# 2bitoperations/rtldavis

Hardware: AMD Instinct MI355X
Metric: complex MSamples/s demodulated (uint8 IQ -> packed bits -> preamble matches -> packets) (higher is better)
Workload: dtype f32 (FIR: f16 x f16 -> f32 on the matrix pipe, exact integer accumulation); 1 GPU; 4096 streams x 33 blocks x 8192 samples uint8 IQ per GPU (BASELINE configs[3]/[4]: 64 unique synthetic streams tiled, 2.21 GB resident in HBM), 14 samples/symbol, 19.2 kbit/s; streams_per_gpu=4096, parallelism=streams/1

## Files before the change

### include/rtldavis_hip.h

```cpp
#ifndef RTLDAVIS_HIP_H
#define RTLDAVIS_HIP_H

#include <stddef.h>
#include <stdint.h>

#ifdef __cplusplus
extern "C" {
#endif

#define RD_MAX_PREAMBLE 64
#define RD_MAX_PKT_BYTES 32

typedef enum rd_status {
    RD_OK = 0,
    RD_ERR_ARG = -1,
    RD_ERR_DEVICE = -2,
    RD_ERR_CAPACITY = -3,
    RD_ERR_STATE = -4
} rd_status;

typedef struct rd_config {
    int32_t bit_rate;
    int32_t symbol_length;
    int32_t preamble_symbols;
    int32_t packet_symbols;
    int32_t block_size;
    uint8_t preamble[RD_MAX_PREAMBLE];
} rd_config;

typedef struct rd_packet {
    int32_t stream;
    int32_t call;
    int32_t index;
    int32_t nbytes;
    uint8_t data[RD_MAX_PKT_BYTES];
    double rssi;
    double snr;
} rd_packet;

typedef struct rd_parsed {
    int32_t stream;
    int32_t call;
    int32_t index;
    int32_t freq_err;
    int32_t id;
    int32_t nbytes;
    uint8_t data[RD_MAX_PKT_BYTES];
    double rssi;
    double snr;
} rd_parsed;

typedef struct rd_timing {
    float demod_ms;
    float fixup_ms;
    float search_ms;
    float slice_ms;
    float total_ms;
    int32_t runs;
} rd_timing;

const char *rd_last_error(void);
int rd_device_count(void);
int rd_set_device(int device);
int rd_set_wait_timeout_ms(int ms);

typedef struct rd_demod rd_demod;

int rd_create(const rd_config *cfg, rd_demod **out);
void rd_destroy(rd_demod *h);
int rd_reset(rd_demod *h);
int rd_demod_block(rd_demod *h, const void *samples, size_t count, int is_complex, rd_packet *out, int cap, int *n);
int rd_create_multi(const rd_config *cfg, int n_streams, rd_demod **out);
int rd_demod_blocks(rd_demod *h, const uint8_t *iq, size_t nbytes, rd_packet *out, int cap, int *n);
int rd_demod_submit(rd_demod *h, const void *samples, size_t count, int is_complex);
int rd_set_input_push(int mode);
int rd_demod_input_mode(rd_demod *h);
int rd_demod_register_input(rd_demod *h, void *host, size_t nbytes);
int rd_demod_submit_from(rd_demod *h, size_t offset, size_t count, int is_complex);
int rd_demod_fetch(rd_demod *h, rd_packet *out, int cap, int *n);
int rd_demod_inflight(rd_demod *h);
int rd_demod_refetch(rd_demod *h, rd_packet *out, int cap, int *n);
int rd_copy_discriminated_stream(rd_demod *h, int stream, double *out, size_t n);
int rd_copy_discriminated(rd_demod *h, double *out, size_t n);
int rd_copy_filtered(rd_demod *h, double *out_interleaved, size_t n_complex);
int rd_copy_quantized(rd_demod *h, uint8_t *out, size_t n);

typedef struct rd_batch rd_batch;

int rd_batch_create(const rd_config *cfg, int n_streams, int n_blocks, rd_batch **out);
void rd_batch_destroy(rd_batch *b);
int rd_batch_input_ptr(rd_batch *b, void **dev_ptr, size_t *nbytes);
int rd_batch_upload(rd_batch *b, const uint8_t *iq_host, size_t nbytes);
int rd_batch_upload_async(rd_batch *b, const uint8_t *iq_host, size_t nbytes, void *hip_stream);
int rd_batch_run(rd_batch *b, void *hip_stream);
int rd_batch_results(rd_batch *b, rd_packet *out, int cap, int *n);
int rd_batch_copy_bits(rd_batch *b, int stream, uint8_t *out, size_t nbytes);
int rd_batch_copy_discriminated(rd_batch *b, int stream, size_t t0, double *out, size_t n);
int rd_batch_set_parse(rd_batch *b, int enabled);
int rd_batch_parsed(rd_batch *b, rd_parsed *out, int cap, int *n);
int rd_batch_set_timing(rd_batch *b, int enabled);
int rd_batch_get_timing(rd_batch *b, rd_timing *out);
int rd_batch_set_pipelined(rd_batch *b, int enabled);
#define RD_FORM_ORDERED_TAIL 1u
#define RD_FORM_SECOND_PASS 8u
#define RD_FORM_ONE_LAUNCH_TAIL 16u
int rd_batch_last_run_forms(rd_batch *b, uint32_t *forms);
int rd_batch_get_counters(rd_batch *b, uint64_t *fixup_runs, uint64_t *matches);

int rd_lut_execute(const uint8_t *in_bytes, size_t n_bytes, double *out_cplx, size_t n_cplx);
int rd_rotate_fs4(const double *in_cplx, double *out_cplx, size_t n_cplx);
int rd_fir9(const double *in_cplx, size_t n_in, double *out_cplx, size_t n_out);
int rd_discriminate(const double *in_cplx, size_t n_in, double *out, size_t n_out);
int rd_quantize(const double *in, uint8_t *out, size_t n);
int rd_search(const rd_config *cfg, const uint8_t *quantized, size_t n, int32_t *indices, int cap, int *count);

typedef struct rd_chan_config {
    int32_t out_rate;
    int32_t decim;
    int32_t n_taps;
    int32_t n_channels;
    double gain;
} rd_chan_config;
typedef struct rd_chan rd_chan;

#define RD_IQ_U8 0
#define RD_IQ_S8 1
#define RD_IQ_S16 2

int rd_chan_create(const rd_chan_config *cfg, const double *taps, const int64_t *shift_hz, rd_chan **out);
int rd_chan_create_fmt(const rd_chan_config *cfg, int sample_format, const double *taps, const int64_t *shift_hz,
                       rd_chan **out);
void rd_chan_destroy(rd_chan *h);
int rd_chan_upload(rd_chan *h, const void *wide_iq, size_t nbytes);
int rd_chan_input_ptr(rd_chan *h, size_t n_wide_samples, void **dev_ptr);
int rd_chan_run(rd_chan *h, size_t n_out, void *dst_dev, size_t dst_stream_stride, void *hip_stream);
int rd_chan_run_host(rd_chan *h, size_t n_out, uint8_t *out_host, size_t nbytes);

typedef struct rd_wideband rd_wideband;
int rd_wideband_create(const rd_config *cfg, const rd_chan_config *ccfg, const double *taps,
                       const int64_t *shift_hz, rd_wideband **out);
int rd_wb_create_fmt(const rd_config *cfg, const rd_chan_config *ccfg, int sample_format, const double *taps,
                     const int64_t *shift_hz, rd_wideband **out);
void rd_wideband_destroy(rd_wideband *w);
int rd_wideband_reset(rd_wideband *w);
int rd_wideband_submit(rd_wideband *w, const void *wide_iq, size_t nbytes);
int rd_wideband_fetch(rd_wideband *w, rd_packet *out, int cap, int *n);
int rd_wideband_refetch(rd_wideband *w, rd_packet *out, int cap, int *n);
int rd_wideband_inflight(rd_wideband *w);
int rd_wideband_copy_channelized(rd_wideband *w, uint8_t *out, size_t nbytes);
int rd_wideband_copy_discriminated(rd_wideband *w, int channel, double *out, size_t n);
int rd_wideband_debug_advance_clock(rd_wideband *w, uint64_t n_out);

void rd_debug_mfma_taps(uint16_t *out);
void rd_debug_mfma_taps8(uint16_t *out);
void rd_debug_mfma_taps8s(uint16_t *vals, uint32_t *idx);
int rd_debug_demod_mfma(const uint8_t *iq_host, int n_streams, uint32_t n_samples, int hist_mode,
                        uint32_t hist_bytes, float *g_out, uint32_t *bits_out, uint32_t *fix_out,
                        uint32_t fix_cap, uint32_t *n_fix);

#ifdef __cplusplus
}
#endif
#endif
```

### rtldavis_amd/_lib.py

```python
from __future__ import annotations

import ctypes as C
import os

import numpy as np

HERE = os.path.dirname(os.path.abspath(__file__))
LIB_PATH = os.environ.get("RTLDAVIS_HIP_LIB") or os.path.join(HERE, "librtldavis_hip.so")

RD_MAX_PREAMBLE = 64
RD_MAX_PKT_BYTES = 32
RD_OK, RD_ERR_ARG, RD_ERR_DEVICE, RD_ERR_CAPACITY, RD_ERR_STATE = 0, -1, -2, -3, -4


class HipError(RuntimeError):
    """A HIP/device failure reported by librtldavis_hip (never swallowed, never retried on CPU)."""


class RdConfig(C.Structure):
    _fields_ = [("bit_rate", C.c_int32), ("symbol_length", C.c_int32), ("preamble_symbols", C.c_int32),
                ("packet_symbols", C.c_int32), ("block_size", C.c_int32), ("preamble", C.c_uint8 * RD_MAX_PREAMBLE)]


class RdPacket(C.Structure):
    _fields_ = [("stream", C.c_int32), ("call", C.c_int32), ("index", C.c_int32), ("nbytes", C.c_int32),
                ("data", C.c_uint8 * RD_MAX_PKT_BYTES), ("rssi", C.c_double), ("snr", C.c_double)]


class RdParsed(C.Structure):
    _fields_ = [("stream", C.c_int32), ("call", C.c_int32), ("index", C.c_int32), ("freq_err", C.c_int32),
                ("id", C.c_int32), ("nbytes", C.c_int32), ("data", C.c_uint8 * RD_MAX_PKT_BYTES),
                ("rssi", C.c_double), ("snr", C.c_double)]


class RdTiming(C.Structure):
    _fields_ = [("demod_ms", C.c_float), ("fixup_ms", C.c_float), ("search_ms", C.c_float),
                ("slice_ms", C.c_float), ("total_ms", C.c_float), ("runs", C.c_int32)]


class RdChanConfig(C.Structure):
    _fields_ = [("out_rate", C.c_int32), ("decim", C.c_int32), ("n_taps", C.c_int32), ("n_channels", C.c_int32),
                ("gain", C.c_double)]


RD_IQ_U8, RD_IQ_S8, RD_IQ_S16 = 0, 1, 2
SAMPLE_FORMATS = {"u8": (RD_IQ_U8, np.uint8), "s8": (RD_IQ_S8, np.int8), "s16": (RD_IQ_S16, np.int16)}


def sample_format(name):
    try:
        return SAMPLE_FORMATS[name]
    except (KeyError, TypeError):
        raise ValueError(f"unknown sample format {name!r}: one of {sorted(SAMPLE_FORMATS)}") from None


def iq_array(a, dtype):
    if np.dtype(dtype) == np.uint8:
        return np.ascontiguousarray(a, dtype=np.uint8).reshape(-1)
    a = np.asarray(a)
    if a.dtype != dtype:
        info = np.iinfo(dtype)
        if a.dtype.kind not in "iu" or (a.size and (a.min() < info.min or a.max() > info.max)):
            raise ValueError(f"a {a.dtype} array is not a capture of {np.dtype(dtype).name} samples")
        a = a.astype(dtype)
    return np.ascontiguousarray(a).reshape(-1)


_P = C.c_void_p
SIGNATURES = {
    "rd_last_error": (C.c_char_p, []),
    "rd_device_count": (C.c_int, []),
    "rd_set_device": (C.c_int, [C.c_int]),
    "rd_set_wait_timeout_ms": (C.c_int, [C.c_int]),
    "rd_set_input_push": (C.c_int, [C.c_int]),
    "rd_demod_input_mode": (C.c_int, [C.c_void_p]),
    "rd_create": (C.c_int, [C.POINTER(RdConfig), C.POINTER(_P)]),
    "rd_create_multi": (C.c_int, [C.POINTER(RdConfig), C.c_int, C.POINTER(_P)]),
    "rd_demod_blocks": (C.c_int, [_P, _P, C.c_size_t, C.POINTER(RdPacket), C.c_int, C.POINTER(C.c_int)]),
    "rd_copy_discriminated_stream": (C.c_int, [_P, C.c_int, _P, C.c_size_t]),
    "rd_demod_submit": (C.c_int, [_P, _P, C.c_size_t, C.c_int]),
    "rd_demod_register_input": (C.c_int, [_P, _P, C.c_size_t]),
    "rd_demod_submit_from": (C.c_int, [_P, C.c_size_t, C.c_size_t, C.c_int]),
    "rd_demod_fetch": (C.c_int, [_P, C.POINTER(RdPacket), C.c_int, C.POINTER(C.c_int)]),
    "rd_demod_refetch": (C.c_int, [_P, C.POINTER(RdPacket), C.c_int, C.POINTER(C.c_int)]),
    "rd_demod_inflight": (C.c_int, [_P]),
    "rd_destroy": (None, [_P]),
    "rd_reset": (C.c_int, [_P]),
    "rd_demod_block": (C.c_int, [_P, _P, C.c_size_t, C.c_int, C.POINTER(RdPacket), C.c_int, C.POINTER(C.c_int)]),
    "rd_copy_discriminated": (C.c_int, [_P, _P, C.c_size_t]),
    "rd_copy_filtered": (C.c_int, [_P, _P, C.c_size_t]),
    "rd_copy_quantized": (C.c_int, [_P, _P, C.c_size_t]),
    "rd_batch_create": (C.c_int, [C.POINTER(RdConfig), C.c_int, C.c_int, C.POINTER(_P)]),
    "rd_batch_destroy": (None, [_P]),
    "rd_batch_input_ptr": (C.c_int, [_P, C.POINTER(_P), C.POINTER(C.c_size_t)]),
    "rd_batch_upload": (C.c_int, [_P, _P, C.c_size_t]),
    "rd_batch_upload_async": (C.c_int, [_P, _P, C.c_size_t, _P]),
    "rd_batch_run": (C.c_int, [_P, _P]),
    "rd_batch_results": (C.c_int, [_P, C.POINTER(RdPacket), C.c_int, C.POINTER(C.c_int)]),
    "rd_batch_copy_bits": (C.c_int, [_P, C.c_int, _P, C.c_size_t]),
    "rd_batch_copy_discriminated": (C.c_int, [_P, C.c_int, C.c_size_t, _P, C.c_size_t]),
    "rd_batch_set_parse": (C.c_int, [_P, C.c_int]),
    "rd_batch_parsed": (C.c_int, [_P, C.POINTER(RdParsed), C.c_int, C.POINTER(C.c_int)]),
    "rd_batch_set_timing": (C.c_int, [_P, C.c_int]),
    "rd_batch_set_pipelined": (C.c_int, [_P, C.c_int]),
    "rd_batch_last_run_forms": (C.c_int, [_P, C.POINTER(C.c_uint32)]),
    "rd_batch_get_timing": (C.c_int, [_P, C.POINTER(RdTiming)]),
    "rd_batch_get_counters": (C.c_int, [_P, C.POINTER(C.c_uint64), C.POINTER(C.c_uint64)]),
    "rd_lut_execute": (C.c_int, [_P, C.c_size_t, _P, C.c_size_t]),
    "rd_rotate_fs4": (C.c_int, [_P, _P, C.c_size_t]),
    "rd_fir9": (C.c_int, [_P, C.c_size_t, _P, C.c_size_t]),
    "rd_discriminate": (C.c_int, [_P, C.c_size_t, _P, C.c_size_t]),
    "rd_quantize": (C.c_int, [_P, _P, C.c_size_t]),
    "rd_search": (C.c_int, [C.POINTER(RdConfig), _P, C.c_size_t, _P, C.c_int, C.POINTER(C.c_int)]),
    "rd_chan_create": (C.c_int, [C.POINTER(RdChanConfig), _P, _P, C.POINTER(_P)]),
    "rd_chan_create_fmt": (C.c_int, [C.POINTER(RdChanConfig), C.c_int, _P, _P, C.POINTER(_P)]),
    "rd_chan_destroy": (None, [_P]),
    "rd_chan_upload": (C.c_int, [_P, _P, C.c_size_t]),
    "rd_chan_input_ptr": (C.c_int, [_P, C.c_size_t, C.POINTER(_P)]),
    "rd_chan_run": (C.c_int, [_P, C.c_size_t, _P, C.c_size_t, _P]),
    "rd_chan_run_host": (C.c_int, [_P, C.c_size_t, _P, C.c_size_t]),
    "rd_wideband_create": (C.c_int, [C.POINTER(RdConfig), C.POINTER(RdChanConfig), _P, _P, C.POINTER(_P)]),
    "rd_wb_create_fmt": (C.c_int, [C.POINTER(RdConfig), C.POINTER(RdChanConfig), C.c_int, _P, _P, C.POINTER(_P)]),
    "rd_wideband_destroy": (None, [_P]),
    "rd_wideband_reset": (C.c_int, [_P]),
    "rd_wideband_submit": (C.c_int, [_P, _P, C.c_size_t]),
    "rd_wideband_fetch": (C.c_int, [_P, C.POINTER(RdPacket), C.c_int, C.POINTER(C.c_int)]),
    "rd_wideband_refetch": (C.c_int, [_P, C.POINTER(RdPacket), C.c_int, C.POINTER(C.c_int)]),
    "rd_wideband_inflight": (C.c_int, [_P]),
    "rd_wideband_copy_channelized": (C.c_int, [_P, _P, C.c_size_t]),
    "rd_wideband_copy_discriminated": (C.c_int, [_P, C.c_int, _P, C.c_size_t]),
    "rd_wideband_debug_advance_clock": (C.c_int, [_P, C.c_uint64]),
    "rd_debug_mfma_taps": (None, [_P]),
    "rd_debug_mfma_taps8": (None, [_P]),
    "rd_debug_mfma_taps8s": (None, [_P, _P]),
    "rd_debug_demod_mfma": (C.c_int, [_P, C.c_int, C.c_uint32, C.c_int, C.c_uint32, _P, _P, _P, C.c_uint32,
                                      C.POINTER(C.c_uint32)]),
}

_lib = None


def lib():
    global _lib
    if _lib is None:
        if not os.path.exists(LIB_PATH):
            raise ImportError(
                f"{LIB_PATH} is missing: build it with `python -c 'import __graft_entry__ as g; g.build()'` "
                "or `make -C rtldavis_amd/csrc`.  rtldavis_amd has no CPU fallback.")
        L = C.CDLL(LIB_PATH)
        for name, (res, args) in SIGNATURES.items():
            fn = getattr(L, name)
            fn.restype = res
            fn.argtypes = args
        _lib = L
    return _lib


def last_error() -> str:
    return (lib().rd_last_error() or b"").decode("utf-8", "replace")


def check(rc: int) -> None:
    if rc == RD_OK:
        return
    msg = last_error()
    if rc == RD_ERR_ARG:
        raise ValueError(msg)
    if rc == RD_ERR_CAPACITY:
        raise BufferError(msg)
    if rc == RD_ERR_STATE:
        raise RuntimeError(msg)
    raise HipError(msg)


def make_config(bit_rate, symbol_length, preamble_symbols, packet_symbols, preamble, block_size) -> RdConfig:
    if len(preamble) > RD_MAX_PREAMBLE:
        raise ValueError("preamble longer than 64 symbols is not supported")
    c = RdConfig(int(bit_rate), int(symbol_length), int(preamble_symbols), int(packet_symbols), int(block_size))
    for i, ch in enumerate(preamble):
        c.preamble[i] = int(ch)
    return c
```

### rtldavis_amd/batch.py

```python
from __future__ import annotations

import ctypes as C
from typing import List, Optional

import numpy as np

from . import _lib
from .dsp import Packet, PacketConfig, _cfg_struct


RD_PACKET_DTYPE = np.dtype([("stream", "<i4"), ("call", "<i4"), ("index", "<i4"), ("nbytes", "<i4"),
                            ("data", "u1", (_lib.RD_MAX_PKT_BYTES,)), ("rssi", "<f8"), ("snr", "<f8")])
assert RD_PACKET_DTYPE.itemsize == C.sizeof(_lib.RdPacket)


RD_PARSED_DTYPE = np.dtype([("stream", "<i4"), ("call", "<i4"), ("index", "<i4"), ("freq_err", "<i4"),
                            ("id", "<i4"), ("nbytes", "<i4"), ("data", "u1", (_lib.RD_MAX_PKT_BYTES,)),
                            ("rssi", "<f8"), ("snr", "<f8")])
assert RD_PARSED_DTYPE.itemsize == C.sizeof(_lib.RdParsed)


class BatchDemodulator:
    def __init__(self, cfg: PacketConfig, n_streams: int, n_blocks: int, device: Optional[int] = None) -> None:
        self.cfg = cfg
        self.n_streams = int(n_streams)
        self.n_blocks = int(n_blocks)
        self.n_samples = self.n_blocks * cfg.block_size
        self._b = C.c_void_p()
        if device is not None:
            _lib.check(_lib.lib().rd_set_device(int(device)))
        _lib.check(_lib.lib().rd_batch_create(C.byref(_cfg_struct(cfg)), self.n_streams, self.n_blocks, C.byref(self._b)))
        self._cap = 0
        self._recs = None

    def close(self) -> None:
        if self._b:
            b, self._b = self._b, None
            _lib.lib().rd_batch_destroy(b)

    def __del__(self):
        try:
            self.close()
        except Exception:
            pass

    def input_ptr(self):
        p, n = C.c_void_p(), C.c_size_t()
        _lib.check(_lib.lib().rd_batch_input_ptr(self._b, C.byref(p), C.byref(n)))
        return p.value, n.value

    def upload(self, iq: np.ndarray) -> None:
        a = np.ascontiguousarray(iq, dtype=np.uint8)
        if a.size != self.n_streams * 2 * self.n_samples:
            raise ValueError("Incompatible array sizes")
        _lib.check(_lib.lib().rd_batch_upload(self._b, a.ctypes.data, a.size))

    def upload_async(self, iq: np.ndarray, hip_stream: int) -> None:
        if iq.dtype != np.uint8 or not iq.flags["C_CONTIGUOUS"] or iq.size != self.n_streams * 2 * self.n_samples:
            raise ValueError("Incompatible array sizes")
        _lib.check(_lib.lib().rd_batch_upload_async(self._b, iq.ctypes.data, iq.size, C.c_void_p(hip_stream or None)))

    def run(self, hip_stream: int = 0) -> None:
        _lib.check(_lib.lib().rd_batch_run(self._b, C.c_void_p(hip_stream or None)))

    def set_parse(self, enabled: bool) -> None:
        _lib.check(_lib.lib().rd_batch_set_parse(self._b, int(bool(enabled))))

    def parsed(self) -> np.ndarray:
        cap = max(1024, 4 * self.n_streams)
        while True:
            buf = (_lib.RdParsed * cap)()
            n = C.c_int(0)
            rc = _lib.lib().rd_batch_parsed(self._b, buf, cap, C.byref(n))
            if rc == _lib.RD_ERR_CAPACITY:
                cap = n.value + 1024
                continue
            _lib.check(rc)
            return np.frombuffer(buf, dtype=RD_PARSED_DTYPE, count=n.value).copy()

    def set_timing(self, level) -> None:
        _lib.check(_lib.lib().rd_batch_set_timing(self._b, int(level)))

    def set_pipelined(self, enabled=True) -> None:
        _lib.check(_lib.lib().rd_batch_set_pipelined(self._b, 1 if enabled else 0))

    def timing(self) -> dict:
        t = _lib.RdTiming()
        _lib.check(_lib.lib().rd_batch_get_timing(self._b, C.byref(t)))
        return {k: float(getattr(t, k)) for k, _ in t._fields_}

    def last_run_forms(self) -> dict:
        f = C.c_uint32()
        _lib.check(_lib.lib().rd_batch_last_run_forms(self._b, C.byref(f)))
        return {"ordered_tail": bool(f.value & 1), "second_pass": bool(f.value & 8), "one_launch_tail": bool(f.value & 16)}

    def counters(self) -> dict:
        f, m = C.c_uint64(), C.c_uint64()
        _lib.check(_lib.lib().rd_batch_get_counters(self._b, C.byref(f), C.byref(m)))
        return {"fixup_runs": f.value, "matches": m.value}

    def results(self) -> np.ndarray:
        L = _lib.lib()
        n = C.c_int(0)
        if self._recs is None:
            self._cap = max(1024, 16 * self.n_streams)
            self._recs = (_lib.RdPacket * self._cap)()
        rc = L.rd_batch_results(self._b, self._recs, self._cap, C.byref(n))
        if rc == _lib.RD_ERR_CAPACITY:
            self._cap = n.value + 1024
            self._recs = (_lib.RdPacket * self._cap)()
            rc = L.rd_batch_results(self._b, self._recs, self._cap, C.byref(n))
        _lib.check(rc)
        return np.frombuffer(self._recs, dtype=RD_PACKET_DTYPE, count=n.value)

    def records(self):
        out = []
        for r in self.results():
            data = np.frombuffer(r["data"][: int(r["nbytes"])].tobytes(), dtype=np.uint8)
            out.append((int(r["stream"]), int(r["call"]),
                        Packet(int(r["index"]), data, float(r["rssi"]), float(r["snr"]))))
        return out

    def packets(self) -> List[List[List[Packet]]]:
        res = [[[] for _ in range(self.n_blocks)] for _ in range(self.n_streams)]
        for s, c, p in self.records():
            res[s][c].append(p)
        return res

    def bits(self, stream: int) -> np.ndarray:
        out = np.empty((self.n_samples + 7) // 8, dtype=np.uint8)
        _lib.check(_lib.lib().rd_batch_copy_bits(self._b, int(stream), out.ctypes.data, out.size))
        return out

    def discriminated(self, stream: int, t0: int, n: int) -> np.ndarray:
        out = np.empty(int(n), dtype=np.float64)
        _lib.check(_lib.lib().rd_batch_copy_discriminated(self._b, int(stream), int(t0), out.ctypes.data, out.size))
        return out

    def demodulate(self, iq: np.ndarray) -> List[List[List[Packet]]]:
        self.upload(iq)
        self.run()
        return self.packets()
```

### rtldavis_amd/csrc/rd_api.hip

```cpp
#include <unistd.h>
#include <immintrin.h>
#include <hsa/hsa.h>
#include <hsa/hsa_ext_amd.h>

#include <algorithm>
#include <cstdarg>
#include <cstdio>
#include <cstring>
#include <string>
#include <vector>
#include <mutex>
#include <map>

#include <chrono>

#include "rd_host.h"
#include "rd_internal.h"
#include "rd_math.h"

static bool dbg_host() {
    static int v = -1;
    if (v < 0) v = getenv("RD_DEBUG_HOST") ? 1 : 0;
    return v == 1;
}
// ... 64 lines not shown
    return RD_OK;
}

static int wait_event(hipEvent_t ev, const char *what) {
    rd_waiter w(rd_wait_timeout_ms());
    for (;;) {
        const hipError_t e = hipEventQuery(ev);
        if (e == hipSuccess) return RD_OK;
        if (e != hipErrorNotReady) return fail(RD_ERR_DEVICE, "hipEventQuery: %s", hipGetErrorString(e));
        if (!w.relax()) return fail(RD_ERR_DEVICE, "timed out after %.0f ms waiting for %s", w.waited_ms(), what);
    }
}

static int wait_stream(hipStream_t st, const char *what) {
    rd_waiter w(rd_wait_timeout_ms());
    for (;;) {
        const hipError_t e = hipStreamQuery(st);
        if (e == hipSuccess) return RD_OK;
        if (e != hipErrorNotReady) return fail(RD_ERR_DEVICE, "hipStreamQuery: %s", hipGetErrorString(e));
        if (!w.relax()) return fail(RD_ERR_DEVICE, "timed out after %.0f ms waiting for %s", w.waited_ms(), what);
    }
}

extern "C" int rd_set_wait_timeout_ms(int ms) { return (int)rd_wait_timeout_set((double)ms); }

static int copy_d2h(void *dst, const void *src, size_t n, hipStream_t st) {
    if (n == 0) return RD_OK;
    HIPCHK(hipMemcpyAsync(dst, src, n, hipMemcpyDeviceToHost, st));
    return wait_stream(st, "a device-to-host copy");
}

static int make_devcfg(const rd_config *c, rd_devcfg *d) {
    const char *why = "";
    const int rc = rd_make_devcfg(c, d, &why);
    return rc ? fail(rc, "%s", why) : RD_OK;
}
static void order_and_dedupe(const rd_packet *recs, size_t n, int S, rd_order_scratch &sc) { rd_order_and_dedupe(recs, n, S, sc); }

struct rd_batch {
    rd_config cfg;
    rd_devcfg dc;
    int n_streams, n_blocks;
    long n_samples;
    size_t bits_stride;
    bool dev_ready = false, fast_ok = false, ran = false, timing = false, timing_detail = false;
    bool run_timing = false, run_detail = false;
    int device = -1;
    bool fetched = false;
    uint8_t *d_iq = nullptr;
    size_t iq_bytes = 0;
    uint32_t *d_bits = nullptr, *d_fix = nullptr, *d_cnt = nullptr;
    rd_match *d_matches = nullptr;
    void *d_tasks = nullptr;
    int dense = 0;
    rd_order_scratch order;
    rd_packet *d_recs = nullptr;
    int cnt_set = 0;
    bool parse = false;
    rd_parsed *d_parsed = nullptr;
    uint32_t fix_cap = 0, match_cap = 0, rec_cap = 0;
    hipStream_t stream = nullptr;
    std::vector<hipEvent_t> evs;
    size_t ev_runs = 0;
    hipEvent_t *ev = nullptr;
    hipEvent_t done = nullptr;
    hipEvent_t kdone = nullptr;
    hipEvent_t uploaded = nullptr;
    bool upload_pending = false;
    hipStream_t copy_stream = nullptr;
    uint32_t h_cnt[RD_CNT_SLOTS] = {};
    uint32_t *h_cnt_pin = nullptr;
    rd_packet *h_recs_pin = nullptr;
    uint32_t rec_pin_cap = 0;
    uint32_t spec_recs = 1024;
    uint64_t last_fix = 0, last_match = 0;
    rd_timing last_timing = {};
    bool dev_order = false, tail_off = false;
    size_t cnt_stride = RD_CNT_TOTAL;
    rd_ft_bufs ft;
    bool ft_ok = false, ft_run = false;
    uint32_t ft_seq = 0, ft_limit = 0;
    bool ft_sticky = false;
    size_t ft_cnt_off = 0;
    bool second_pass = false;
    uint32_t last_launch[2] = {0, 0};
    bool pipelined = false;
    bool deferred = false;
    hipEvent_t kfirst = nullptr;
    std::vector<uint8_t> ev_end;
};

static std::mutex g_tail_mx;
typedef std::pair<int, hipStream_t> rd_tail_key;
static std::map<rd_tail_key, rd_batch *> g_tail;

static rd_layout batch_layout(const rd_batch *b) {
    rd_layout l;
    l.iq = b->d_iq;
    l.stream_stride = (size_t)b->n_samples * 2;
    l.n_streams = b->n_streams;
    l.n_samples = (uint32_t)b->n_samples;
    l.hist_mode = 0;
    l.valid_from = 0;
    l.bits = b->d_bits;
    l.bits_stride = b->bits_stride;
    return l;
}

extern "C" int rd_batch_create(const rd_config *cfg, int n_streams, int n_blocks, rd_batch **out) {
    if (!out) return fail(RD_ERR_ARG, "null out");
    rd_devcfg dc;
    int rc = make_devcfg(cfg, &dc);
    if (rc) return rc;
    if (n_streams < 1 || n_blocks < 1) return fail(RD_ERR_ARG, "n_streams and n_blocks must be >= 1");
    const long n = (long)n_blocks * cfg->block_size;
    const uint64_t runs = (uint64_t)n_streams * ((n + RD_RUN - 1) / RD_RUN);
    if (n > 0x7FFFFFF0L || runs > 0x0FFFFFFFull)
        return fail(RD_ERR_ARG, "batch too large: at most 2^28 32-sample runs (8.6e9 samples) per batch");
    rd_batch *b = new rd_batch();
    b->cfg = *cfg;
    b->dc = dc;
    b->n_streams = n_streams;
    b->n_blocks = n_blocks;
    b->n_samples = n;
    b->bits_stride = (size_t)((n + 31) / 32);
    b->fast_ok = ((size_t)n * 2) % 16 == 0;
    *out = b;
    return RD_OK;
}

static uint32_t *batch_cnt(const rd_batch *b) { return b->d_cnt + (size_t)b->cnt_set * b->cnt_stride; }

static int use_device(int device) {
    if (device >= 0) HIPCHK(hipSetDevice(device));
    return RD_OK;
}

static int batch_alloc(rd_batch *b) {
    if (b->dev_ready) return use_device(b->device);
    int rc = ensure_device();
    if (rc) return rc;
    HIPCHK(hipGetDevice(&b->device));
    const uint64_t runs = (uint64_t)b->n_streams * b->bits_stride;
    b->iq_bytes = (size_t)b->n_streams * b->n_samples * 2;
    b->fix_cap = (uint32_t)std::min<uint64_t>(runs, std::max<uint64_t>(4096, runs / 8));
    b->match_cap = (uint32_t)std::min<uint64_t>((uint64_t)b->n_streams * (8 + 1ull * b->n_blocks) + 1024, 1u << 26);
    if (const char *e = getenv("RD_TEST_MATCH_CAP")) {
        const long v = atol(e);
        if (v >= 1 && v < (long)b->match_cap) b->match_cap = (uint32_t)v;
    }
    b->rec_cap = 2 * b->match_cap;
    HIPCHK(hipMalloc(&b->d_iq, b->iq_bytes + RD_INPUT_PAD));
    HIPCHK(hipMemset(b->d_iq + b->iq_bytes, 127, RD_INPUT_PAD));
    HIPCHK(hipMalloc(&b->d_bits, runs * sizeof(uint32_t)));
    HIPCHK(hipMalloc(&b->d_fix, (size_t)b->fix_cap * sizeof(uint32_t)));
    {
        const char *ti = getenv("RD_TAIL_IMPL");
        const bool legacy = ti && ti[0] == 'l';
        b->ft_ok = !legacy && b->fast_ok && b->dc.S == 14 && b->dc.P == 16 && b->dc.K == 80 && b->dc.pre_mask == 0x91D3ull &&
                   b->n_samples < (1l << 30) && b->dc.B < (1 << 24) && b->bits_stride % 4 == 0 && b->dc.L >= b->dc.B &&
                   (long)(b->n_blocks + 1) * b->dc.B - b->dc.L >= 0 &&
                   ((long)(b->n_blocks + 1) * b->dc.B - b->dc.L) / 32 + 16 <= (long)b->bits_stride;
        if (const char *e = getenv("RD_TEST_BUCKET_CAP")) {
            const long v = atol(e);
            if (v >= 1 && v < RD_BUCKET_MIN) b->ft_limit = (uint32_t)v;
        }
    }
    b->cnt_stride = RD_CNT_TOTAL;
    if (b->ft_ok) {
        const size_t groups = ((size_t)b->n_streams + RD_FT_STREAMS - 1) / RD_FT_STREAMS;
        b->ft_cnt_off = b->cnt_stride;
        b->cnt_stride += (groups + 3) & ~(size_t)3;
        const uint64_t tps = ((uint64_t)b->n_samples + RD_TILE_SAMPLES - 1) / RD_TILE_SAMPLES;
        b->ft.fix_bcap = (uint32_t)std::min<uint64_t>((2 * RD_FT_STREAMS * (tps / 4 + 8) + 63) & ~63ull, 1u << 20);
        if (const char *e = getenv("RD_TEST_FIX_BCAP")) {
            const long v = atol(e);
            if (v >= 1 && v < (long)b->ft.fix_bcap) b->ft.fix_bcap = (uint32_t)v;
        }
        b->ft.bcap = rd_ord_bucket_cap(b->n_samples);
        HIPCHK(hipMalloc(&b->ft.fixb, groups * b->ft.fix_bcap * sizeof(uint32_t)));
        HIPCHK(hipMalloc(&b->ft.gstate, 3 * groups * sizeof(uint32_t)));
        HIPCHK(hipMemset(b->ft.gstate, 0, 3 * groups * sizeof(uint32_t)));
    }
    HIPCHK(hipMalloc(&b->d_cnt, 2 * b->cnt_stride * sizeof(uint32_t)));
    HIPCHK(hipMemset(b->d_cnt, 0, 2 * b->cnt_stride * sizeof(uint32_t)));
    HIPCHK(hipMalloc(&b->d_matches, (size_t)b->match_cap * sizeof(rd_match)));
    HIPCHK(hipMalloc(&b->d_recs, (size_t)b->rec_cap * sizeof(rd_packet)));
    HIPCHK(hipMalloc(&b->d_tasks, (size_t)b->rec_cap * RD_TASK_BYTES));
    HIPCHK(hipHostMalloc((void **)&b->h_cnt_pin, RD_CNT_SLOTS * sizeof(uint32_t), hipHostMallocDefault));
    HIPCHK(hipHostMalloc((void **)&b->h_recs_pin, (size_t)b->rec_cap * sizeof(rd_packet), hipHostMallocDefault));
    b->rec_pin_cap = b->rec_cap;
    HIPCHK(hipEventCreateWithFlags(&b->done, hipEventDisableTiming));
    HIPCHK(hipEventCreateWithFlags(&b->kdone, hipEventDisableTiming));
    HIPCHK(hipEventCreateWithFlags(&b->kfirst, hipEventDisableTiming));
    HIPCHK(hipEventCreateWithFlags(&b->uploaded, hipEventDisableTiming));
    HIPCHK(hipStreamCreateWithFlags(&b->copy_stream, hipStreamNonBlocking));
    b->dev_ready = true;
    return RD_OK;
}

extern "C" void rd_batch_destroy(rd_batch *b) {
    if (!b) return;
    {
        std::lock_guard<std::mutex> g(g_tail_mx);
        auto it = g_tail.find(rd_tail_key(b->device, b->stream));
        if (it != g_tail.end() && it->second == b) g_tail.erase(it);
        b->deferred = false;
    }
    if (b->dev_ready && g_hip_pid == getpid()) {
        if (b->device >= 0) hipSetDevice(b->device);
        if (b->ran && !b->fetched) hipDeviceSynchronize();
        hipFree(b->d_iq); hipFree(b->d_bits); hipFree(b->d_fix); hipFree(b->d_cnt);
        hipFree(b->d_matches); hipFree(b->d_recs); hipFree(b->d_tasks);
        hipFree(b->d_parsed);
        hipFree(b->ft.fixb); hipFree(b->ft.gstate);
        hipHostFree(b->h_cnt_pin); hipHostFree(b->h_recs_pin);
        if (b->done) hipEventDestroy(b->done);
        if (b->kdone) hipEventDestroy(b->kdone);
        if (b->kfirst) hipEventDestroy(b->kfirst);
        if (b->uploaded) hipEventDestroy(b->uploaded);
        if (b->copy_stream) hipStreamDestroy(b->copy_stream);
        for (auto &e : b->evs) if (e) hipEventDestroy(e);
    }
    delete b;
}

extern "C" int rd_batch_input_ptr(rd_batch *b, void **dev_ptr, size_t *nbytes) {
    if (!b || !dev_ptr) return fail(RD_ERR_ARG, "null argument");
    int rc = batch_alloc(b);
    if (rc) return rc;
    *dev_ptr = b->d_iq;
    if (nbytes) *nbytes = b->iq_bytes;
    return RD_OK;
}

static int batch_flush(rd_batch *b);

extern "C" int rd_batch_upload(rd_batch *b, const uint8_t *iq_host, size_t nbytes) {
    if (!b || !iq_host) return fail(RD_ERR_ARG, "null argument");
    int rc = batch_alloc(b);
    if (rc) return rc;
    if (nbytes != b->iq_bytes) {
        return fail(RD_ERR_ARG, "Incompatible array sizes: got %zu bytes, expected %zu", nbytes, b->iq_bytes);
    }
    if (b->ran && !b->fetched) {
        rc = batch_flush(b);
        if (rc) return rc;
        rc = wait_event(b->done, "the previous run before an upload");
        if (rc) return rc;
    }
    HIPCHK(hipMemcpy(b->d_iq, iq_host, nbytes, hipMemcpyHostToDevice));
    if (!b->ft_sticky) b->tail_off = false;
    return RD_OK;
}

extern "C" int rd_batch_upload_async(rd_batch *b, const uint8_t *iq_host, size_t nbytes, void *hip_stream) {
    if (!b || !iq_host) return fail(RD_ERR_ARG, "null argument");
    int rc = batch_alloc(b);
    if (rc) return rc;
    if (nbytes != b->iq_bytes) return fail(RD_ERR_ARG, "Incompatible array sizes: got %zu bytes, expected %zu", nbytes, b->iq_bytes);
    hipStream_t cs = (hipStream_t)hip_stream;
    if (b->ran && !b->fetched) {
        rc = batch_flush(b);
        if (rc) return rc;
        HIPCHK(hipStreamWaitEvent(cs, b->done, 0));
    }
    HIPCHK(hipMemcpyAsync(b->d_iq, iq_host, nbytes, hipMemcpyHostToDevice, cs));
    HIPCHK(hipEventRecord(b->uploaded, cs));
    b->upload_pending = true;
    if (!b->ft_sticky) b->tail_off = false;
    return RD_OK;
}

static int batch_readback(rd_batch *b, hipEvent_t after) {
    HIPCHK(hipStreamWaitEvent(b->copy_stream, after, 0));
    HIPCHK(hipMemcpyAsync(b->h_cnt_pin, batch_cnt(b), RD_CNT_SLOTS * sizeof(uint32_t), hipMemcpyDeviceToHost,
                          b->copy_stream));
    const uint32_t spec = std::min(b->dev_order ? b->rec_cap : b->match_cap, b->spec_recs);
    if (spec)
        HIPCHK(hipMemcpyAsync(b->h_recs_pin, b->d_recs, (size_t)spec * sizeof(rd_packet), hipMemcpyDeviceToHost,
                              b->copy_stream));
    HIPCHK(hipEventRecord(b->done, b->copy_stream));
    return RD_OK;
}


static int batch_flush_locked(rd_batch *p) {
    if (!p->deferred) return RD_OK;
    auto it = g_tail.find(rd_tail_key(p->device, p->stream));
    if (it != g_tail.end() && it->second == p) g_tail.erase(it);
    p->deferred = false;
    int rc = use_device(p->device);
    if (rc) return rc;
    HIPCHK(hipEventRecord(p->kdone, p->stream));
    return batch_readback(p, p->kdone);
}
static int batch_flush(rd_batch *b) {
    std::lock_guard<std::mutex> g(g_tail_mx);
    return batch_flush_locked(b);
}
static bool batch_stream_has_tail(int device, hipStream_t st) {
    std::lock_guard<std::mutex> g(g_tail_mx);
    return g_tail.find(rd_tail_key(device, st)) != g_tail.end();
}
static int batch_adopt(int device, hipStream_t st, hipEvent_t carrier) {
    std::lock_guard<std::mutex> g(g_tail_mx);
    auto it = g_tail.find(rd_tail_key(device, st));
    if (it == g_tail.end()) return RD_OK;
    rd_batch *p = it->second;
    g_tail.erase(it);
    p->deferred = false;
    return batch_readback(p, carrier);
}

static int batch_search_slice(rd_batch *b, hipStream_t st, bool may_defer = false, uint32_t *zero_next = nullptr) {
    const rd_layout lay = batch_layout(b);
    const long B = b->dc.B, L = b->dc.L;
    const bool last_on_slice = !b->parse;
    const bool defer = may_defer && b->pipelined && last_on_slice && !(b->run_timing && b->run_detail);
    hipEvent_t last = defer ? nullptr : b->run_timing ? b->ev[4] : b->kdone;
    if (b->run_timing && may_defer) b->ev_end.push_back(defer ? 0 : 1);
    b->dev_order = false;
    if (b->ft_run && may_defer) {
        rd_ft_bufs fb = b->ft;
        fb.fixcnt = batch_cnt(b) + b->ft_cnt_off;
        b->ft_seq = b->ft_seq % 4095u + 1u;
        const int ok = rd_launch_tail_fused(lay, b->dc, b->n_blocks, B - L, (long)(b->n_blocks + 1) * B - L, fb,
                                            b->ft_limit ? b->ft_limit : fb.bcap, b->ft_seq, 0, b->d_recs, b->rec_cap, batch_cnt(b), st,
                                            last_on_slice ? last : nullptr, zero_next, (uint32_t)b->cnt_stride);
        if (!ok) return fail(RD_ERR_STATE, "the one-launch tail refused a shape its buffers were allocated for");
        b->dev_order = true;
        b->dense = 1;
    }
    if (!b->dev_order) {
        rd_launch_search(b->d_bits, b->bits_stride, b->n_streams, b->n_samples, B - L, (long)(b->n_blocks + 1) * B - L,
                         b->dc, b->d_matches, b->match_cap, batch_cnt(b), st);
        if (b->run_timing && b->run_detail) HIPCHK(hipEventRecord(b->ev[3], st));
        b->dense = rd_launch_slice(lay, b->d_bits, b->bits_stride, b->n_samples, b->dc, b->d_matches, b->match_cap, 1,
                                   b->n_blocks, 0, b->d_recs, nullptr, batch_cnt(b), st, last_on_slice ? last : nullptr,
                                   b->d_tasks);
    }
    if (b->parse) {
        if (!b->d_parsed) HIPCHK(hipMalloc(&b->d_parsed, (size_t)b->rec_cap * sizeof(rd_parsed)));
        rd_launch_parse(lay, b->dc, b->d_recs, b->match_cap, b->d_parsed, batch_cnt(b), st, b->dense);
    }
    if (defer) {
        std::lock_guard<std::mutex> g(g_tail_mx);
        auto it = g_tail.find(rd_tail_key(b->device, st));
        if (it != g_tail.end() && it->second != b) {
            int rc = batch_flush_locked(it->second);
            if (rc) return rc;
        }
        g_tail[rd_tail_key(b->device, st)] = b;
        b->deferred = true;
        HIPCHK(hipGetLastError());
        return RD_OK;
    }
    if (!last_on_slice) HIPCHK(hipEventRecord(last, st));
    int rc = batch_readback(b, last);
    if (rc) return rc;
    HIPCHK(hipGetLastError());
    return RD_OK;
}

extern "C" int rd_batch_run(rd_batch *b, void *hip_stream) {
    if (!b) return fail(RD_ERR_ARG, "null batch");
    int rc = batch_alloc(b);
    if (rc) return rc;
    hipStream_t st = (hipStream_t)hip_stream;
    const rd_layout lay = batch_layout(b);
    if (b->ran && !b->fetched) {
        rc = batch_flush(b);
        if (rc) return rc;
        HIPCHK(hipStreamWaitEvent(st, b->done, 0));
    }
    b->stream = st;
    if (b->upload_pending) {
        HIPCHK(hipStreamWaitEvent(st, b->uploaded, 0));
        b->upload_pending = false;
    }
    b->fetched = false;
    b->cnt_set ^= 1;
    uint32_t *cnt = batch_cnt(b), *cnt_next = b->d_cnt + (size_t)(b->cnt_set ^ 1) * b->cnt_stride;
    b->run_timing = b->timing;
    b->run_detail = b->timing_detail;
    if (b->timing) {
        if (b->evs.size() < 5 * (b->ev_runs + 1)) {
            const size_t old = b->evs.size();
            b->evs.resize(old + 5, nullptr);
            for (size_t i = old; i < b->evs.size(); i++) HIPCHK(hipEventCreate(&b->evs[i]));
        }
        b->ev = &b->evs[5 * b->ev_runs];
        b->ev_runs++;
    }
    const bool adopt = batch_stream_has_tail(b->device, st);
    const bool want_ft = b->ft_ok && b->fast_ok && !b->tail_off && !(b->timing && b->timing_detail);
    const uint32_t dflags = want_ft ? RD_DEMOD_FIX_BUCKETS : 0u;
    uint32_t *fixl = want_ft ? b->ft.fixb : b->d_fix, *bcnt = want_ft ? cnt + b->ft_cnt_off : nullptr;
    const uint32_t fixc = want_ft ? b->ft.fix_bcap : b->fix_cap;
    uint32_t honoured = 0;
    if (b->timing && b->fast_ok) {
        honoured = rd_launch_demod(lay, fixl, fixc, cnt, st, b->ev[0], b->ev[1], dflags, b->last_launch, bcnt);
        if (adopt && (rc = batch_adopt(b->device, st, b->ev[1]))) return rc;
    } else if (b->fast_ok && adopt) {
        honoured = rd_launch_demod(lay, fixl, fixc, cnt, st, nullptr, b->kfirst, dflags, b->last_launch, bcnt);
        if ((rc = batch_adopt(b->device, st, b->kfirst))) return rc;
    } else {
        if (b->timing) HIPCHK(hipEventRecord(b->ev[0], st));
        if (b->fast_ok) honoured = rd_launch_demod(lay, fixl, fixc, cnt, st, nullptr, nullptr, dflags, b->last_launch, bcnt);
        if (b->timing) HIPCHK(hipEventRecord(b->ev[1], st));
        if (adopt) {
            hipEvent_t carrier = b->timing ? b->ev[1] : b->kfirst;
            if (!b->timing) HIPCHK(hipEventRecord(carrier, st));
            if ((rc = batch_adopt(b->device, st, carrier))) return rc;
        }
    }
    b->second_pass = false;
    b->ft_run = b->fast_ok && (honoured & RD_DEMOD_FIX_BUCKETS);
    if (!b->ft_run)
        rd_launch_fixup(lay, fixl, fixc, cnt, b->fast_ok ? 0 : 1, cnt_next, st, (uint32_t)b->cnt_stride, b->last_fix);
    if (b->timing && b->timing_detail) HIPCHK(hipEventRecord(b->ev[2], st));
    rc = batch_search_slice(b, st, true, b->ft_run ? cnt_next : nullptr);
    if (rc) return rc;
    b->ran = true;
    return RD_OK;
}

static int batch_finish(rd_batch *b) {
    if (!b->ran) return fail(RD_ERR_STATE, "rd_batch_run has not been called");
    hipStream_t st = b->stream;
    {
        int frc = batch_flush(b);
        if (frc) return frc;
    }
    for (int attempt = 0; attempt < 8; attempt++) {
        const double ta = now_ms();
        int wrc = wait_event(b->done, "the batch run's results");
        if (wrc) return wrc;
        memcpy(b->h_cnt, b->h_cnt_pin, sizeof b->h_cnt);
        if (dbg_host()) fprintf(stderr, "[rd] finish: wait %.3f ms\n", now_ms() - ta);
        bool redo_search = false;
        if (b->ft_run && !b->second_pass && (b->h_cnt[RD_CNT_OVF] & (8u | 16u))) {
            const rd_layout lay = batch_layout(b);
            rd_launch_fixup(lay, b->d_fix, b->fix_cap, batch_cnt(b), 1, nullptr, st);
            b->last_fix = (uint64_t)b->n_streams * b->bits_stride;
            b->tail_off = true;
            b->h_cnt[RD_CNT_OVF] = 0;
            b->h_cnt[RD_CNT_FIX] = 0;
            redo_search = true;
        } else if (b->ft_run && !b->second_pass && (b->h_cnt[RD_CNT_OVF] & 1u)) {
            if (!b->ft_limit && b->ft.bcap < RD_BUCKET_MAX) b->ft.bcap = std::min<uint32_t>(2 * b->ft.bcap, RD_BUCKET_MAX);
            else if (!b->ft_limit) b->ft_sticky = true;
        }
        if (redo_search) {
        } else if (b->fast_ok && !b->ft_run && b->h_cnt[RD_CNT_FIX] > b->fix_cap) {
            const rd_layout lay = batch_layout(b);
            rd_launch_fixup(lay, b->d_fix, b->fix_cap, batch_cnt(b), 1, nullptr, st);
            uint32_t cap = b->fix_cap;
            HIPCHK(hipMemcpyAsync(batch_cnt(b) + RD_CNT_FIX, &cap, sizeof cap, hipMemcpyHostToDevice, st));
            b->last_fix = (uint64_t)b->n_streams * b->bits_stride;
            redo_search = true;
        } else if (attempt == 0) {
            b->last_fix = (uint64_t)b->h_cnt[RD_CNT_FIX];
        }
        if (redo_search && b->tail_off) b->dev_order = false;
        if (b->dev_order && b->h_cnt[RD_CNT_OVF]) {
            b->tail_off = true;
            if (dbg_host())
                fprintf(stderr, "[rd] one-launch tail overflow: flags %u (1 a stream's match list, 2 records), matches %u\n",
                        b->h_cnt[RD_CNT_OVF], b->h_cnt[RD_CNT_MATCH]);
            const uint32_t zero[5] = {0, 0, 0, 0, 0};
            HIPCHK(hipMemcpyAsync(batch_cnt(b) + RD_CNT_MATCH, zero, sizeof zero, hipMemcpyHostToDevice, st));
            b->second_pass = true;
            int rc2 = batch_search_slice(b, st);
            if (rc2) return rc2;
            continue;
        }
        if (!b->dev_order && b->h_cnt[RD_CNT_MATCH] > b->match_cap) {
            hipFree(b->d_matches); b->d_matches = nullptr;
            hipFree(b->d_recs); b->d_recs = nullptr;
            hipHostFree(b->h_recs_pin); b->h_recs_pin = nullptr;
            b->rec_pin_cap = 0;
            hipFree(b->d_tasks); b->d_tasks = nullptr;
            hipFree(b->d_parsed); b->d_parsed = nullptr;
            const uint32_t want = b->h_cnt[RD_CNT_MATCH] + b->h_cnt[RD_CNT_MATCH] / 4 + 1024;
            b->match_cap = 0;
            b->rec_cap = 0;
            b->ran = false;
            const uint32_t new_rec_cap = 2 * want;
            HIPCHK(hipMalloc(&b->d_matches, (size_t)want * sizeof(rd_match)));
            HIPCHK(hipMalloc(&b->d_recs, (size_t)new_rec_cap * sizeof(rd_packet)));
            HIPCHK(hipMalloc(&b->d_tasks, (size_t)new_rec_cap * RD_TASK_BYTES));
            HIPCHK(hipHostMalloc((void **)&b->h_recs_pin, (size_t)new_rec_cap * sizeof(rd_packet), hipHostMallocDefault));
            b->match_cap = want;
            b->rec_cap = new_rec_cap;
            b->rec_pin_cap = new_rec_cap;
            b->ran = true;
            redo_search = true;
        }
        if (!redo_search) {
            b->last_match = b->h_cnt[RD_CNT_MATCH];
            b->fetched = true;
            return RD_OK;
        }
        const uint32_t zero[5] = {0, 0, 0, 0, 0};
        HIPCHK(hipMemcpyAsync(batch_cnt(b) + RD_CNT_MATCH, zero, sizeof zero, hipMemcpyHostToDevice, st));
        b->second_pass = true;
        int rc2 = batch_search_slice(b, st);
        if (rc2) return rc2;
    }
    return fail(RD_ERR_DEVICE, "result lists kept overflowing");
}

extern "C" int rd_batch_results(rd_batch *b, rd_packet *out, int cap, int *n) {
    if (!b || !n) return fail(RD_ERR_ARG, "null argument");
    const double t0 = now_ms();
    int rc = batch_finish(b);
    if (rc) return rc;
    const double t1 = now_ms();
    const uint32_t nprim = b->dense ? std::min(b->h_cnt[RD_CNT_TASKS], b->rec_cap) : std::min(b->h_cnt[RD_CNT_MATCH], b->match_cap);
    const uint32_t nextra = b->dense ? 0u : std::min(b->h_cnt[RD_CNT_REC], b->match_cap);
    const uint32_t have = std::min(b->dev_order ? b->rec_cap : b->match_cap, b->spec_recs);
    if (nprim > have) {
        rc = copy_d2h(b->h_recs_pin + have, b->d_recs + have, (size_t)(nprim - have) * sizeof(rd_packet), b->copy_stream);
        if (rc) return rc;
    }
    if (nextra) {
        rc = copy_d2h(b->h_recs_pin + nprim, b->d_recs + b->match_cap, (size_t)nextra * sizeof(rd_packet), b->copy_stream);
        if (rc) return rc;
    }
    const uint32_t nrec = nprim + nextra;
    b->spec_recs = std::max<uint32_t>(1024, nprim + nprim / 4);
    const double t2 = now_ms();
    if (b->dev_order) {
        *n = (int)nrec;
        if ((int)nrec > cap) return fail(RD_ERR_CAPACITY, "need room for %u packets", nrec);
        if (nrec) {
            if (!out) return fail(RD_ERR_ARG, "null out");
            memcpy(out, b->h_recs_pin, (size_t)nrec * sizeof(rd_packet));
        }
        if (dbg_host())
            fprintf(stderr, "[rd] results (k_tail): finish %.3f ms, D2H %u recs %.3f ms, copy %.3f ms\n", t1 - t0, nrec,
                    t2 - t1, now_ms() - t2);
        return RD_OK;
    }
    order_and_dedupe(b->h_recs_pin, nrec, b->dc.S, b->order);
    const std::vector<uint32_t> &kept = b->order.kept;
    *n = (int)kept.size();
    if ((int)kept.size() > cap) return fail(RD_ERR_CAPACITY, "need room for %zu packets", kept.size());
    if (!kept.empty()) {
        if (!out) return fail(RD_ERR_ARG, "null out");
        for (size_t i = 0; i < kept.size(); i++) out[i] = b->h_recs_pin[kept[i]];
    }
    if (dbg_host())
        fprintf(stderr, "[rd] results: finish %.3f ms, D2H %u recs %.3f ms, order+dedupe+copy %.3f ms\n", t1 - t0, nrec,
                t2 - t1, now_ms() - t2);
    return RD_OK;
}

extern "C" int rd_batch_copy_bits(rd_batch *b, int stream, uint8_t *out, size_t nbytes) {
    if (!b || !out) return fail(RD_ERR_ARG, "null argument");
    if (stream < 0 || stream >= b->n_streams) return fail(RD_ERR_ARG, "stream out of range");
    const size_t need = (size_t)((b->n_samples + 7) / 8);
    if (nbytes < need) return fail(RD_ERR_ARG, "bit buffer too small: %zu < %zu", nbytes, need);
    int rc = batch_finish(b);
    if (rc) return rc;
    return copy_d2h(out, (const uint8_t *)(b->d_bits + (size_t)stream * b->bits_stride), need, b->stream);
}

extern "C" int rd_batch_copy_discriminated(rd_batch *b, int stream, size_t t0, double *out, size_t n) {
    if (!b || !out) return fail(RD_ERR_ARG, "null argument");
    if (stream < 0 || stream >= b->n_streams || t0 + n > (size_t)b->n_samples)
        return fail(RD_ERR_ARG, "range out of bounds");
    int rc = batch_alloc(b);
    if (rc) return rc;
    if (n == 0) return RD_OK;
    double *d = nullptr;
    HIPCHK(hipMalloc(&d, n * sizeof(double)));
    rd_launch_disc(batch_layout(b), stream, (long)t0, (long)n, d, b->stream);
    rc = copy_d2h(out, d, n * sizeof(double), b->stream);
    hipFree(d);
    return rc;
}

// ... 30 lines not shown
        for (size_t k = group; k < kept && !dup; k++)
            dup = recs[k].nbytes == r.nbytes && memcmp(recs[k].data, r.data, sizeof r.data) == 0;
        if (!dup) recs[kept++] = r;
    }
    *n = (int)kept;
    if ((int)kept > cap) return fail(RD_ERR_CAPACITY, "need room for %zu messages", kept);
    if (kept) {
        if (!out) return fail(RD_ERR_ARG, "null out");
        memcpy(out, recs.data(), kept * sizeof(rd_parsed));
    }
    return RD_OK;
}

extern "C" int rd_batch_set_pipelined(rd_batch *b, int enabled) {
    if (!b) return fail(RD_ERR_ARG, "null batch");
    b->pipelined = enabled != 0;
    return RD_OK;
}

extern "C" int rd_batch_set_timing(rd_batch *b, int enabled) {
    if (!b) return fail(RD_ERR_ARG, "null batch");
    b->timing = enabled != 0;
    b->timing_detail = enabled >= 2;
    b->ev_runs = 0;
    b->ev_end.clear();
    if (b->timing && b->dev_ready && use_device(b->device) == RD_OK) {
        const size_t want = 5 * 64;
        const size_t old = b->evs.size();
        if (old < want) {
            b->evs.resize(want, nullptr);
            for (size_t i = old; i < want; i++) HIPCHK(hipEventCreate(&b->evs[i]));
        }
    }
    return RD_OK;
}

extern "C" int rd_batch_get_timing(rd_batch *b, rd_timing *out) {
    if (!b || !out) return fail(RD_ERR_ARG, "null argument");
    if (!b->timing) return fail(RD_ERR_STATE, "timing not enabled");
    int rc = batch_finish(b);
    if (rc) return rc;
    rd_timing t = {};
    size_t n_end = 0;
    for (size_t r = 0; r < b->ev_runs; r++) {
        hipEvent_t *e = &b->evs[5 * r];
        float v[5] = {0, 0, 0, 0, 0};
        HIPCHK(hipEventElapsedTime(&v[0], e[0], e[1]));
        if (b->timing_detail) {
            HIPCHK(hipEventElapsedTime(&v[1], e[1], e[2]));
            HIPCHK(hipEventElapsedTime(&v[2], e[2], e[3]));
            HIPCHK(hipEventElapsedTime(&v[3], e[3], e[4]));
        }
        const bool has_end = r >= b->ev_end.size() || b->ev_end[r];
        if (has_end) { HIPCHK(hipEventElapsedTime(&v[4], e[0], e[4])); n_end++; }
        t.demod_ms += v[0]; t.fixup_ms += v[1]; t.search_ms += v[2]; t.slice_ms += v[3]; t.total_ms += v[4];
    }
    if (b->ev_runs) {
        const float k = 1.0f / (float)b->ev_runs;
        t.demod_ms *= k; t.fixup_ms *= k; t.search_ms *= k; t.slice_ms *= k;
        t.total_ms = n_end ? t.total_ms / (float)n_end : 0.0f;
    }
    t.runs = (int32_t)b->ev_runs;
    b->ev_runs = 0;
    b->ev_end.clear();
    b->last_timing = t;
    *out = t;
    return RD_OK;
}

extern "C" int rd_batch_last_run_forms(rd_batch *b, uint32_t *forms) {
    if (!b || !forms) return fail(RD_ERR_ARG, "null argument");
    int rc = batch_finish(b);
    if (rc) return rc;
    *forms = (b->dev_order ? RD_FORM_ORDERED_TAIL | RD_FORM_ONE_LAUNCH_TAIL : 0u) | (b->second_pass ? RD_FORM_SECOND_PASS : 0u);
    return RD_OK;
}

extern "C" int rd_batch_get_counters(rd_batch *b, uint64_t *fixup_runs, uint64_t *matches) {
    if (!b) return fail(RD_ERR_ARG, "null batch");
    int rc = batch_finish(b);
    if (rc) return rc;
    if (fixup_runs) *fixup_runs = b->last_fix;
    if (matches) *matches = b->last_match;
    return RD_OK;
}

#define RD_MAX_DEVICES 64
struct rd_push_info {
    int state = 0;
    volatile uint32_t *hdp_flush = nullptr;
};
static rd_push_info g_push[RD_MAX_DEVICES];

struct rd_hdp_find { uint32_t bdf, domain; volatile uint32_t *reg; bool found; };
static hsa_status_t rd_hdp_cb(hsa_agent_t agent, void *data) {
    rd_hdp_find *f = (rd_hdp_find *)data;
    hsa_device_type_t t;
    if (hsa_agent_get_info(agent, HSA_AGENT_INFO_DEVICE, &t) != HSA_STATUS_SUCCESS || t != HSA_DEVICE_TYPE_GPU) return HSA_STATUS_SUCCESS;
    uint32_t bdf = 0, dom = 0;
    if (hsa_agent_get_info(agent, (hsa_agent_info_t)HSA_AMD_AGENT_INFO_BDFID, &bdf) != HSA_STATUS_SUCCESS) return HSA_STATUS_SUCCESS;
    if (hsa_agent_get_info(agent, (hsa_agent_info_t)HSA_AMD_AGENT_INFO_DOMAIN, &dom) != HSA_STATUS_SUCCESS) return HSA_STATUS_SUCCESS;
    if (bdf != f->bdf || dom != f->domain) return HSA_STATUS_SUCCESS;
    hsa_amd_hdp_flush_t h = {nullptr, nullptr};
    if (hsa_agent_get_info(agent, (hsa_agent_info_t)HSA_AMD_AGENT_INFO_HDP_FLUSH, &h) == HSA_STATUS_SUCCESS) f->reg = h.HDP_MEM_FLUSH_CNTL;
    f->found = true;
    return HSA_STATUS_INFO_BREAK;
}

static int g_push_mode = -1;
static bool push_available(int dev) {
    if (dev < 0 || dev >= RD_MAX_DEVICES || g_push_mode == 0) return false;
    static std::mutex mu;
    std::lock_guard<std::mutex> lock(mu);
    rd_push_info &p = g_push[dev];
    if (p.state) return p.state > 0;
    p.state = -1;
    const char *e = getenv("RD_PUSH_INPUT");
    if (e && atoi(e) == 0) return false;
    int large = 0;
    if (hipDeviceGetAttribute(&large, hipDeviceAttributeIsLargeBar, dev) != hipSuccess || !large) return false;
    char id[64] = {0};
    unsigned dom = 0, bus = 0, d = 0, fn = 0;
    if (hipDeviceGetPCIBusId(id, sizeof id, dev) != hipSuccess || sscanf(id, "%x:%x:%x.%x", &dom, &bus, &d, &fn) != 4) return false;
    if (hsa_init() != HSA_STATUS_SUCCESS) return false;
    rd_hdp_find f = {(bus << 8) | (d << 3) | fn, dom, nullptr, false};
    hsa_iterate_agents(rd_hdp_cb, &f);
    if (!f.found || !f.reg) return false;
    p.hdp_flush = f.reg;
    p.state = 1;
    return true;
}

extern "C" int rd_set_input_push(int mode) {
    int rc = ensure_device();
    if (rc) return rc;
    g_push_mode = mode == 0 ? 0 : -1;
    int dev = -1;
    if (hipGetDevice(&dev) != hipSuccess) return fail(RD_ERR_DEVICE, "hipGetDevice failed");
    return push_available(dev) ? 1 : 0;
}

struct rd_slot {
    uint8_t *h_in = nullptr;
    uint8_t *d_in_map = nullptr;
    uint8_t *d_in = nullptr;
    uint8_t *d_push = nullptr;
    uint32_t *h_cnt = nullptr;
    rd_packet *h_recs = nullptr;
    rd_packet *d_recs_map = nullptr;
    uint32_t *h_sb = nullptr;
    uint32_t *d_sb_map = nullptr;
    uint32_t seq = 0;
    bool one = false;
    hipEvent_t e_in = nullptr, e_done = nullptr;
};

struct rd_demod {
    rd_config cfg;
    rd_devcfg dc;
    bool dev_ready = false;
    bool cplx_mode = false;
    long seen = 0;
    int NS = 1;
    int device = -1;
    size_t ring_stride = 0;
    uint8_t *d_ring = nullptr;
// ... 749 lines not shown
```

### rtldavis_amd/csrc/rd_demod_mfma.hip

```cpp
#include <cstdio>
#include <cstdlib>
#include <cstring>

#include <hip/hip_ext.h>

#include "rd_internal.h"
#include "rd_math.h"
#include "rd_mfma.h"

#define RD_MF_WG 256
#define RD_MF_WAVES (RD_MF_WG / 64)
#ifndef RD_MF_MINWAVES
#define RD_MF_MINWAVES 4
#endif
#define RD_MF_GROUP_BYTES 1152
#define RD_MF_IMG_BYTES (16 + 4 * RD_MF_GROUP_BYTES)
#define RD_MF_IMG_PAD 4624
#define RD_MF_XB_BYTES (3 * 1024 + 32 + 32)
#define RD_MF_PEND 32
#ifndef RD_MF_STAGE_TILES
#define RD_MF_STAGE_TILES 4
#endif

typedef _Float16 rd_h8 __attribute__((ext_vector_type(8)));
typedef _Float16 rd_h16 __attribute__((ext_vector_type(16)));
typedef _Float16 rd_h2 __attribute__((ext_vector_type(2)));
typedef float rd_f16v __attribute__((ext_vector_type(16)));
typedef uint32_t rd_u4v __attribute__((ext_vector_type(4)));
typedef float rd_f4v __attribute__((ext_vector_type(4)));
typedef uint32_t rd_u2v __attribute__((ext_vector_type(2)));

static const rd_mf_taps h_mf_taps = rd_mf_make_taps();
__device__ const rd_mf_taps8 g_mf_taps8 = rd_mf_make_taps8();
static const rd_mf_taps8 h_mf_taps8 = rd_mf_make_taps8();
extern "C" void rd_debug_mfma_taps8(uint16_t *out) { memcpy(out, &h_mf_taps8, sizeof h_mf_taps8); }
#ifndef RD_MF_SPARSE
#define RD_MF_SPARSE 1
#endif
constexpr bool rd_mf_taps8s_ok() { bool ok = true; (void)rd_mf_make_taps8s(&ok); return ok; }
static_assert(rd_mf_taps8s_ok(), "a row of the tap matrix has more than two non-zero elements in a group of four");
constexpr rd_mf_taps8s rd_mf_taps8s_value() { bool ok = true; return rd_mf_make_taps8s(&ok); }
__device__ const rd_mf_taps8s g_mf_taps8s = rd_mf_taps8s_value();
static const rd_mf_taps8s h_mf_taps8s = rd_mf_taps8s_value();
extern "C" void rd_debug_mfma_taps8s(uint16_t *vals, uint32_t *idx) {
    memcpy(vals, h_mf_taps8s.v, sizeof h_mf_taps8s.v);
    memcpy(idx, h_mf_taps8s.idx, sizeof h_mf_taps8s.idx);
}

extern "C" void rd_debug_mfma_taps(uint16_t *out) { memcpy(out, &h_mf_taps, sizeof h_mf_taps); }

__device__ __forceinline__ rd_h8 rd_mf_frag(rd_u2v d) {
    rd_u4v v;
    v.x = d.x & 0x00FF00FFu;
    v.y = __builtin_amdgcn_perm(0u, d.x, 0x0c030c01u);
    v.z = d.y & 0x00FF00FFu;
    v.w = __builtin_amdgcn_perm(0u, d.y, 0x0c030c01u);
    return __builtin_bit_cast(rd_h8, v);
}

__device__ __forceinline__ float rd_mf_num(float ar, float ai, float cr, float ci, float &t1) {
    t1 = ai * ci;
    return __builtin_fmaf(-ar, cr, -t1);
}
__device__ __forceinline__ float rd_mf_guard(float nmin, float tmax) { return __builtin_fmaf(-4.76837158e-7f, tmax, nmin); }


template <int OFF>
__device__ __forceinline__ void rd_lds_write16(uint32_t addr, rd_f4v v) {
    asm volatile("ds_write_b128 %0, %1 offset:%2" : : "v"(addr), "v"(v), "i"(OFF) : "memory");
}
template <int OFF>
__device__ __forceinline__ rd_f4v rd_lds_read16(uint32_t addr) {
    rd_f4v r;
    asm volatile("ds_read_b128 %0, %1 offset:%2" : "=v"(r) : "v"(addr), "i"(OFF) : "memory");
    return r;
}
__device__ __forceinline__ void rd_lds_wait(rd_f4v &r) { asm volatile("s_waitcnt lgkmcnt(0)" : "+v"(r) : : "memory"); }
__device__ __forceinline__ void rd_lds_write4(uint32_t addr, uint32_t v) {
    asm volatile("ds_write_b32 %0, %1" : : "v"(addr), "v"(v) : "memory");
}
__device__ __forceinline__ rd_u4v rd_lds_read16u(uint32_t addr) {
    rd_u4v r;
    asm volatile("ds_read_b128 %0, %1\n\ts_waitcnt lgkmcnt(0)" : "=&v"(r) : "v"(addr) : "memory");
    return r;
}
__device__ __forceinline__ uint32_t rd_lds_read4(uint32_t addr) {
    uint32_t r;
    asm volatile("ds_read_b32 %0, %1\n\ts_waitcnt lgkmcnt(0)" : "=&v"(r) : "v"(addr) : "memory");
    return r;
}
__device__ __forceinline__ uint32_t rd_lds_addr(const void *p) {
    return (uint32_t)(uintptr_t)(const __attribute__((address_space(3))) void *)p;
}

__device__ __forceinline__ bool rd_mf_any(bool c) { return __ballot(c) != 0; }


struct rd_mf8_addr {
    uint32_t xw;
    uint32_t xw7;
    uint32_t rd1, rdE, rdO;
    uint32_t rd0;
// ... 112 lines not shown
    rd_mf8_block<3, DBG>(A, dcC, sidx, sidx2, D, bfA, bb, ad, k0, kp, p, Wlo, Whi, fblo, fbhi, slow, dg, dleft);
    rd_mf8_block<4, DBG>(A, dcC, sidx, sidx2, D, bfA, bb, ad, k0, kp, p, Wlo, Whi, fblo, fbhi, slow, dg, dleft);
    rd_mf8_block<5, DBG>(A, dcC, sidx, sidx2, D, bfA, bb, ad, k0, kp, p, Wlo, Whi, fblo, fbhi, slow, dg, dleft);
    rd_mf8_block<6, DBG>(A, dcC, sidx, sidx2, D, bfA, bb, ad, k0, kp, p, Wlo, Whi, fblo, fbhi, slow, dg, dleft);
    rd_mf8_block<7, DBG>(A, dcC, sidx, sidx2, D, bfA, bb, ad, k0, kp, p, Wlo, Whi, fblo, fbhi, slow, dg, dleft);
    rd_f4v p0 = rd_lds_read16<0>(ad.rd0);
    rd_mf8_finish<7, DBG>(kp, p, Whi, fbhi, slow);
    {
        rd_lds_wait(p0);
        float t0, t1;
        const float n0 = rd_mf_num(p0.x, p0.y, p0.z, p0.w, t0);
        const float n1 = rd_mf_num(p0.z, p0.w, k0.g0r, k0.g0i, t1);
        if (DBG == 0 || DBG == 3) {
            const float nm = rd_mf_guard(rd_min3abs(k0.nmin, n0, n1), rd_max3abs(k0.tmax, t0, t1));
            if (rd_mf_any(!(nm > RD_MF_C0_MAX))) {
                slow = true;
                float F = rd_max3abs(0.0f, p0.x, p0.y);
                F = rd_max3abs(F, p0.z, p0.w);
                F = rd_max3abs(F, k0.g0r, k0.g0i);
                F = rd_max3abs(F, k0.g1r, k0.g1i);
                F = rd_max3abs(F, k0.g2r, k0.g2i);
                if (!(nm > rd_mf_c0(F))) fblo |= 1u;
            }
        }
        uint32_t b0 = rd_shift_in_sign(0u, n0);
        b0 = rd_shift_in_sign(b0, n1);
        b0 = rd_shift_in_sign(b0, k0.n2);
        b0 = __builtin_amdgcn_alignbit(b0, __builtin_bit_cast(uint32_t, k0.n3), 27);
        Wlo = (b0 << 24) | Wlo;
    }
    const uint32_t Vlo = __builtin_bitreverse32(Wlo & 0xF0F0F0F0u), Vhi = __builtin_bitreverse32(Whi & 0xF0F0F0F0u);
    const auto r = __builtin_amdgcn_permlane32_swap(Vlo, Vhi, false, false);
    word = (r[1] << 4) | r[0];
    fbw = 0;
    if (slow && rd_mf_any((fblo | fbhi) != 0)) {
        const auto f = __builtin_amdgcn_permlane32_swap(fblo, fbhi, false, false);
        fbw = f[0] | f[1];
    }
}

#ifndef RD_MF_LOAD_AUX
#define RD_MF_LOAD_AUX 2
#endif

__device__ __forceinline__ void rd_mf_issue(const rd_layout &lay, uint32_t s, uint32_t ti, uint8_t *img, int lane,
                                            bool halo_dma = true) {
    const uint8_t *src = lay.iq + (size_t)s * lay.stream_stride + (size_t)ti * RD_TILE_BYTES;
    const int perm = 8 * (lane & 7) + (lane >> 3);
    const __attribute__((address_space(1))) void *g0 = (const __attribute__((address_space(1))) void *)(src + perm * 16);
    __builtin_amdgcn_global_load_lds(g0, (__attribute__((address_space(3))) void *)(img + 16), 16, 0, RD_MF_LOAD_AUX);
    __builtin_amdgcn_global_load_lds(g0, (__attribute__((address_space(3))) void *)(img + 16 + 128), 16, 1024, RD_MF_LOAD_AUX);
    __builtin_amdgcn_global_load_lds(g0, (__attribute__((address_space(3))) void *)(img + 16 + 256), 16, 2048, RD_MF_LOAD_AUX);
    __builtin_amdgcn_global_load_lds(g0, (__attribute__((address_space(3))) void *)(img + 16 + 384), 16, 3072, RD_MF_LOAD_AUX);
    const bool has_halo = (ti > 0) || lay.hist_mode;
    if (lane == 0 && halo_dma)
        __builtin_amdgcn_global_load_lds((const __attribute__((address_space(1))) void *)(src + (has_halo ? -16 : 0)),
                                         (__attribute__((address_space(3))) void *)(img), 16, 0, 0);
}

__device__ __forceinline__ int rd_lane_now() {
    return (int)__builtin_amdgcn_mbcnt_hi(~0u, __builtin_amdgcn_mbcnt_lo(~0u, 0u));
}

__device__ __forceinline__ void rd_mf_flush(const uint32_t *pend, uint32_t count, uint32_t *fix_list, uint32_t fix_cap,
                                            uint32_t *counters, uint32_t bits_stride, uint32_t *bucket_cnt) {
    const int lane = rd_lane_now();
    asm volatile("s_waitcnt lgkmcnt(0)" ::: "memory");
    if (bucket_cnt) {
        for (uint32_t i = lane; i < count; i += 64) {
            const uint32_t e = pend[i];
            const uint32_t grp = ((e >> 4) / bits_stride) >> RD_FT_GSH;
            const uint32_t slot = atomicAdd(&bucket_cnt[grp], 1u);
            if (slot < fix_cap) fix_list[(size_t)grp * fix_cap + slot] = e;
        }
        return;
    }
    uint32_t base = 0;
    if (lane == 0) base = atomicAdd(&counters[RD_CNT_FIX], count);
    base = __builtin_amdgcn_readfirstlane(base);
    for (uint32_t i = lane; i < count; i += 64)
        if (base + i < fix_cap) fix_list[base + i] = pend[i];
}


__device__ __forceinline__ void rd_mf_store_staged(uint32_t stage_addr, uint32_t nst, uint32_t *base, uint32_t stflags) {
    const int lane = rd_lane_now();
    if (nst == RD_MF_STAGE_TILES) {
#pragma unroll
        for (int j = 0; j < RD_MF_STAGE_TILES / 4; j++) {
            const rd_u4v v = rd_lds_read16u(stage_addr + 16 * (lane + 64 * j));
            if (!(stflags & 1)) __builtin_nontemporal_store(v, (rd_u4v *)(base + 4 * (lane + 64 * j)));
            else *(rd_u4v *)(base + 4 * (lane + 64 * j)) = v;
        }
    } else {
        for (uint32_t q = 0; q < nst; q++) base[64 * q + lane] = rd_lds_read4(stage_addr + 256 * q + 4 * lane);
    }
}

struct rd_mf_pos {
    uint32_t tile, s, ti, inchunk;
};
struct rd_mf_nextchunk {
    uint32_t tile, s, ti;
};
__device__ __forceinline__ rd_mf_nextchunk rd_mf_chunk_at(uint64_t chunk_id, uint32_t chunk, uint32_t tps, uint32_t total) {
    rd_mf_nextchunk c;
    const uint32_t n_chunks = (total + chunk - 1) / chunk;
    const bool have = chunk_id < n_chunks;
    const uint32_t nt = have ? (uint32_t)chunk_id * chunk : 0u;
    c.tile = have ? nt : 0xFFFFFFFFu;
    c.s = 0; c.ti = 0;
    if (have) {
        c.s = __builtin_amdgcn_readfirstlane(c.tile / tps);
        c.ti = c.tile - c.s * tps;
    }
    return c;
}
__device__ __forceinline__ rd_mf_pos rd_mf_next(rd_mf_pos p, uint32_t chunk, uint32_t tps, const rd_mf_nextchunk &nc) {
    rd_mf_pos q;
    if (p.inchunk + 1 < chunk) {
        q.tile = p.tile + 1; q.inchunk = p.inchunk + 1;
        q.s = p.s; q.ti = p.ti + 1;
        if (q.ti >= tps) { q.ti = 0; q.s++; }
    } else {
        q.tile = nc.tile; q.inchunk = 0;
        q.s = nc.s; q.ti = nc.ti;
    }
    return q;
}

__device__ __forceinline__ void rd_mf_read_window(uint32_t a_prv, uint32_t a_own, rd_u2v (&D)[9]) {
    asm volatile("ds_read_b64 %0, %9\n\t"
                 "ds_read_b64 %1, %10\n\t"
                 "ds_read_b64 %2, %10 offset:128\n\t"
                 "ds_read_b64 %3, %10 offset:256\n\t"
                 "ds_read_b64 %4, %10 offset:384\n\t"
                 "ds_read_b64 %5, %10 offset:512\n\t"
                 "ds_read_b64 %6, %10 offset:640\n\t"
                 "ds_read_b64 %7, %10 offset:768\n\t"
                 "ds_read_b64 %8, %10 offset:896\n\t"
                 "s_waitcnt lgkmcnt(0)"
                 : "=&v"(D[0]), "=&v"(D[1]), "=&v"(D[2]), "=&v"(D[3]), "=&v"(D[4]), "=&v"(D[5]), "=&v"(D[6]),
                   "=&v"(D[7]), "=&v"(D[8])
                 : "v"(a_prv), "v"(a_own)
                 : "memory");
}

__device__ __forceinline__ uint64_t rd_stamp() {
    uint64_t t;
    __builtin_amdgcn_sched_barrier(0);
    asm volatile("s_memtime %0\n\ts_waitcnt lgkmcnt(0)" : "=s"(t) : : "memory");
    __builtin_amdgcn_sched_barrier(0);
    return t;
}
__device__ __forceinline__ uint64_t rd_stamp_real() {
    uint64_t t;
    __builtin_amdgcn_sched_barrier(0);
    asm volatile("s_memrealtime %0\n\ts_waitcnt lgkmcnt(0)" : "=s"(t) : : "memory");
    __builtin_amdgcn_sched_barrier(0);
    return t;
}


#define RD_STAMP_WORDS 12
#define RD_STF_BUCKETS 8192u
template <int DBG, bool STAMP>
__global__ __launch_bounds__(RD_MF_WG, RD_MF_MINWAVES) void k_demod_mfma(rd_layout lay, uint32_t tiles_per_stream, uint32_t total_tiles,
                                                         uint32_t chunk, uint32_t *fix_list, uint32_t fix_cap,
                                                         uint32_t *counters, float *dbg_g, uint32_t stflags) {
    __shared__ __attribute__((aligned(16))) uint8_t s_img[RD_MF_WAVES][RD_MF_IMG_PAD];
    __shared__ __attribute__((aligned(32))) uint8_t s_xb[RD_MF_WAVES][RD_MF_XB_BYTES];
    __shared__ uint32_t s_pend[RD_MF_WAVES][RD_MF_PEND];
    __shared__ __attribute__((aligned(16))) uint32_t s_stage[RD_MF_WAVES][RD_MF_STAGE_TILES][64];
    constexpr bool LOADS = DBG != 1;
    const int lane = threadIdx.x & 63;
    const int wave = __builtin_amdgcn_readfirstlane(threadIdx.x >> 6);
    uint8_t *img0 = s_img[wave];
    uint8_t *xb = s_xb[wave];
    uint32_t *mypend = s_pend[wave];
    uint32_t npend = 0;
    constexpr bool CAN_BUCKET = DBG == 0 && !STAMP;
    uint32_t *bucket_cnt = (CAN_BUCKET && (stflags & RD_STF_BUCKETS)) ? (uint32_t *)dbg_g : nullptr;

    const int n = lane & 31, h = lane >> 5;
    rd_h8 A8[2];
    rd_f16v dcC;
    int sidx = 0, sidx2 = 0;
    if (RD_MF_SPARSE && DBG != 8 && DBG != 9) {
        A8[0] = *(const rd_h8 *)g_mf_taps8s.v[lane];
        A8[1] = *(const rd_h8 *)g_mf_taps8s.v[lane ^ 32];
        sidx = (int)g_mf_taps8s.idx[lane];
        sidx2 = (int)g_mf_taps8s.idx[lane ^ 32];
    } else {
        A8[0] = *(const rd_h8 *)g_mf_taps8.v[0][lane];
        A8[1] = *(const rd_h8 *)g_mf_taps8.v[1][lane];
    }
    const float dchi = -(float)RD_MF_DHI / 16777216.0f;
#pragma unroll
    for (int i = 0; i < 16; i++) dcC[i] = i < 8 ? dchi : 0.0f;
    if (RD_MF_SPARSE && DBG != 8 && DBG != 9) asm volatile("" : "+v"(A8[0]), "+v"(A8[1]), "+v"(sidx), "+v"(sidx2));
    else asm volatile("" : "+v"(A8[0]), "+v"(A8[1]), "+v"(dcC));
    const uint32_t img_addr = rd_lds_addr(img0);
    const uint32_t own = 16 + RD_MF_GROUP_BYTES * (n >> 3) + 16 * (n & 7) + 8 * h;
    const uint32_t prv = n == 0 ? 8 * h
                       : (n & 7) ? own + 16 * 55
                                 : 16 + RD_MF_GROUP_BYTES * ((n >> 3) - 1) + 16 * 63 + 8 * h;
    const uint32_t xb_addr = rd_lds_addr(xb), pend_addr = rd_lds_addr(mypend);
    const uint32_t stage_addr = rd_lds_addr(s_stage[wave]);
    const uint32_t rtoggle = lane == 0 ? 16u : 0u, wtoggle = lane == 63 ? 16u : 0u;
    rd_mf8_addr ad8;
    ad8.xw = xb_addr + 16 * lane;
    ad8.xw7 = xb_addr + (lane == 63 ? 3072 : 1024 + 16 * lane);
    ad8.rd1 = xb_addr + (h ? 1024 + 16 * (lane - 32) : 16 * (lane + 32));
    ad8.rdE = xb_addr + (h ? 2048 + 16 * (lane - 32) : 1024 + 16 * (lane + 32));
    ad8.rdO = xb_addr + (h ? 1024 + 16 * (lane - 32) : 2048 + 16 * (lane + 32));
    ad8.rd0 = xb_addr + (h ? 16 * (lane - 32) : lane ? 1024 + 16 * (lane + 31) : 3072 + 16);
    if (lane < 8) ((uint32_t *)(xb + 3072))[lane] = 0;

    const uint32_t nwaves = gridDim.x * RD_MF_WAVES;
    const uint32_t wave_id = blockIdx.x * RD_MF_WAVES + wave;
    const bool dynamic = !(stflags & 4096) && chunk >= 4;
    uint32_t cur_chunk = wave_id;
    rd_mf_nextchunk nextc = {0xFFFFFFFFu, 0, 0};
    if (!dynamic) nextc = rd_mf_chunk_at((uint64_t)cur_chunk + nwaves, chunk, tiles_per_stream, total_tiles);
    uint32_t grab = 0;
    bool grab_pending = false;
    const uint32_t my_queue = wave_id % RD_NQUEUE;
    uint32_t *queue = &counters[RD_CNT_QUEUE0 + RD_QUEUE_STRIDE * my_queue];
    rd_mf_pos cur;
    cur.tile = wave_id * chunk;
    cur.s = cur.tile / tiles_per_stream;
    cur.ti = cur.tile % tiles_per_stream;
    cur.inchunk = 0;
    rd_mf_pos nx1 = rd_mf_next(cur, chunk, tiles_per_stream, nextc);

    uint32_t nst = 0;
    uint32_t *st_base = nullptr;
    bool st_flush = false;
    uint64_t sm_wait = 0, sm_gap = 0, sm_comp = 0, sm_wait_st = 0, sm_t0 = 0, sm_r0 = 0, sm_mark = 0, sm_wmax = 0;
    uint32_t sm_iters = 0, sm_iters_st = 0;
    bool sm_stored = false;
    if (STAMP) { sm_t0 = rd_stamp(); sm_r0 = rd_stamp_real(); }
    if (LOADS && cur.tile < total_tiles) rd_mf_issue(lay, cur.s, cur.ti, img0, lane);
    if (STAMP) sm_mark = rd_stamp();
    while (cur.tile < total_tiles) {
        const uint32_t tile = cur.tile, s = cur.s, ti = cur.ti, inchunk = cur.inchunk;
        uint64_t sm_a = 0;
        if (STAMP) { sm_a = rd_stamp(); sm_comp += sm_a - sm_mark; }
        asm volatile("s_waitcnt vmcnt(0)" : "+v"(grab) : : "memory");
        uint64_t sm_b = 0;
        if (STAMP) {
            sm_b = rd_stamp();
            const uint64_t w = sm_b - sm_a;
            sm_wait += w;
            if (w > sm_wmax) sm_wmax = w;
            if (sm_stored) { sm_wait_st += w; sm_iters_st++; }
            sm_iters++;
            sm_stored = false;
        }
        if (dynamic) {
            if (grab_pending) {
                nextc = rd_mf_chunk_at((uint64_t)nwaves + my_queue + (uint64_t)RD_NQUEUE * __builtin_amdgcn_readfirstlane(grab),
                                       chunk, tiles_per_stream, total_tiles);
                grab_pending = false;
            }
            if (inchunk == 0) {
                const uint32_t one = 1, zoff = 0;
                uint64_t saved_exec;
                asm volatile("s_mov_b64 %1, exec\n\ts_mov_b64 exec, 1\n\tglobal_atomic_add %0, %2, %3, %4 sc0\n\ts_mov_b64 exec, %1"
                             : "+v"(grab), "=&s"(saved_exec) : "v"(zoff), "v"(one), "s"(queue) : "memory");
                grab_pending = true;
            }
        } else if (inchunk == 0 && tile != wave_id * chunk) {
            cur_chunk += nwaves;
            nextc = rd_mf_chunk_at((uint64_t)cur_chunk + nwaves, chunk, tiles_per_stream, total_tiles);
        }
        if (!(stflags & 4)) __builtin_amdgcn_s_setprio(3);
        rd_u2v D[9];
        rd_mf_read_window(img_addr + prv, img_addr + own, D);
        if (nst == RD_MF_STAGE_TILES || (nst && st_flush)) {
            rd_mf_store_staged(stage_addr, nst, st_base, stflags);
            nst = 0;
            if (STAMP) sm_stored = true;
        }
        const rd_mf_pos nx2 = rd_mf_next(nx1, chunk, tiles_per_stream, nextc);
        bool halo_dma = true;
        {
            const bool follows = nx1.tile < total_tiles && nx1.s == s && nx1.ti == ti + 1;
            if (follows) {
                halo_dma = false;
                if (n == 31) asm volatile("ds_write_b64 %0, %1" : : "v"(img_addr + 8 * h), "v"(D[8]) : "memory");
            }
        }
        if (LOADS && nx1.tile < total_tiles) rd_mf_issue(lay, nx1.s, nx1.ti, img0, lane, halo_dma);
        if (!(stflags & 4)) __builtin_amdgcn_s_setprio(0);
        if (STAMP) { sm_mark = rd_stamp(); sm_gap += sm_mark - sm_b; }

        uint32_t word = 0;
        bool slow_taken = false;
        uint32_t fbw8 = 0;
        if (DBG == 2 || DBG == 6) {
#pragma unroll
            for (int j = 0; j < 9; j++) word ^= D[j].x ^ D[j].y;
        } else {
            float *dg = DBG == 3 ? dbg_g + ((size_t)tile * RD_TILE_SAMPLES + 64 * n + 4 * h + 1) * 2 : nullptr;
            const int dleft = RD_TILE_SAMPLES - (64 * n + 4 * h + 1);
            rd_mf8_tile<DBG>(A8, dcC, sidx, sidx2, D, ad8, word, fbw8, slow_taken, dg, dleft);
            ad8.rd0 ^= rtoggle;
            ad8.xw7 ^= wtoggle;
        }
        uint32_t gmask = 0;
        const bool carry = inchunk > 0 && ti > 0;
        const uint32_t run = ti * 64 + 2 * n + h;
        const uint32_t t0 = run * RD_RUN;
        const bool any_flag = slow_taken && rd_mf_any(fbw8 != 0);
        if (any_flag) gmask = ((fbw8 * 0x00204081u) >> 21) & 0xFu;
        if (!carry && lane == 0) {
            if (ti == 0 && !lay.hist_mode) gmask = 0xFu;
            else gmask |= 1u;
        }
        const bool ragged = (ti + 1 == tiles_per_stream) && (lay.n_samples % RD_TILE_SAMPLES) != 0;
        if (DBG == 6) {
            if (word == 0x12345678u) lay.bits[0] = word;
        } else if (!ragged) {
            if (nst == 0) {
                st_base = &lay.bits[(size_t)s * lay.bits_stride + ti * 64];
                if (stflags & 2) st_base = &lay.bits[(((size_t)s * lay.bits_stride + ti * 64) & 0x3FFFFu) & ~255u];
            }
            rd_lds_write4(stage_addr + 256 * nst + 4 * (2 * n + h), word);
            nst++;
            const bool next_ragged = (nx1.ti + 1 == tiles_per_stream) && (lay.n_samples % RD_TILE_SAMPLES) != 0;
            st_flush = !(nx1.tile < total_tiles && nx1.s == s && nx1.ti == ti + 1 && !next_ragged);
        } else if (t0 < lay.n_samples) {
            const uint32_t left = lay.n_samples - t0;
            if (left < RD_RUN) {
                word &= (1u << left) - 1u;
                gmask &= (1u << ((left + RD_GROUP - 1) / RD_GROUP)) - 1u;
            }
            lay.bits[(size_t)s * lay.bits_stride + run] = word;
        } else {
            gmask = 0;
        }
        if (DBG == 1 || DBG == 2 || DBG == 6) gmask = 0;
        const uint64_t fm = (any_flag || !carry) ? __ballot(gmask != 0) : 0;
        if (fm) {
            const uint32_t nf = (uint32_t)__popcll(fm);
            if (npend + nf > RD_MF_PEND) {
                rd_mf_flush(mypend, npend, fix_list, fix_cap, counters, (uint32_t)lay.bits_stride, bucket_cnt);
                npend = 0;
            }
            if (gmask)
                rd_lds_write4(pend_addr + 4 * (npend + __builtin_amdgcn_mbcnt_hi((uint32_t)(fm >> 32),
                                                                                  __builtin_amdgcn_mbcnt_lo((uint32_t)fm, 0))),
                              ((uint32_t)((size_t)s * lay.bits_stride + run) << 4) | gmask);
            npend += nf;
        }
        cur = nx1;
        nx1 = nx2;
    }
    if (nst) rd_mf_store_staged(stage_addr, nst, st_base, stflags);
    if (npend) rd_mf_flush(mypend, npend, fix_list, fix_cap, counters, (uint32_t)lay.bits_stride, bucket_cnt);
    if (STAMP && dbg_g) {
        const uint64_t t1 = rd_stamp(), r1 = rd_stamp_real();
        sm_comp += t1 - sm_mark;
        if (lane == 0) {
            uint64_t *o = (uint64_t *)dbg_g + (size_t)wave_id * RD_STAMP_WORDS;
            o[0] = sm_wait; o[1] = sm_gap; o[2] = sm_comp; o[3] = sm_wait_st;
            o[4] = sm_iters; o[5] = sm_iters_st; o[6] = t1 - sm_t0; o[7] = r1 - sm_r0;
            o[8] = sm_wmax; o[9] = sm_r0; o[10] = r1;
            uint32_t xcc;
            asm volatile("s_getreg_b32 %0, hwreg(HW_REG_XCC_ID)" : "=s"(xcc));
            o[11] = xcc;
        }
    }
}

static int rd_mf_env(const char *name, int dflt) {
    const char *e = getenv(name);
    return e ? atoi(e) : dflt;
}

struct rd_mf_params {
    int dbg = 0, stamp = 0, chunk_env = 0, per_cu_env = 0, n_cu = 256;
    uint32_t stflags = 0;
    rd_mf_params() {
        chunk_env = rd_mf_env("RD_K1_CHUNK", 0);
        per_cu_env = rd_mf_env("RD_K1_WGS_PER_CU", 0);
#ifdef RD_DIAG
        dbg = rd_mf_env("RD_K1_DEBUG", 0);
        stamp = rd_mf_env("RD_K1_STAMPS", 0) ? 1 : 0;
        stflags = (uint32_t)rd_mf_env("RD_K1_STFLAGS", 0) & (1u | 2u | 4u | 4096u);
#endif
        int dev = 0;
        hipDeviceProp_t prop;
        if (hipGetDevice(&dev) == hipSuccess && hipGetDeviceProperties(&prop, dev) == hipSuccess && prop.multiProcessorCount > 0)
            n_cu = prop.multiProcessorCount;
    }
};
static const rd_mf_params &rd_mf_get_params() {
    static const rd_mf_params p;
    return p;
}

#ifdef RD_DIAG
static uint64_t *g_stamp_buf = nullptr;
static uint32_t g_stamp_waves = 0;
extern "C" int rd_diag_read_stamps(uint64_t *out, uint32_t cap_waves, uint32_t *n_waves) {
    if (!g_stamp_buf || !n_waves) return RD_ERR_STATE;
    if (hipDeviceSynchronize() != hipSuccess) return RD_ERR_DEVICE;
    *n_waves = g_stamp_waves;
    const uint32_t n = g_stamp_waves < cap_waves ? g_stamp_waves : cap_waves;
    if (n && hipMemcpy(out, g_stamp_buf, (size_t)n * RD_STAMP_WORDS * 8, hipMemcpyDeviceToHost) != hipSuccess) return RD_ERR_DEVICE;
    return RD_OK;
}
extern "C" int rd_diag_variant(int *dbg, int *stamp, uint32_t *stflags) {
    const rd_mf_params &P = rd_mf_get_params();
    if (dbg) *dbg = P.dbg;
    if (stamp) *stamp = P.stamp;
    if (stflags) *stflags = P.stflags;
    return RD_OK;
}
#endif

struct rd_mf_launch_args {
    rd_layout lay;
    uint32_t tps, total;
    uint64_t total64;
    uint32_t *fix_list, fix_cap, *counters;
    hipStream_t st;
    hipEvent_t ev_start, ev_stop;
    uint32_t *bucket_cnt = nullptr;
    uint32_t *chunk_out = nullptr;
    float *dbg_g;
};

template <int D, bool STAMP>
static void rd_mf_launch_variant(const rd_mf_launch_args &a) {
    const rd_mf_params &P = rd_mf_get_params();
    static const int per_cu_occ = [] {
        int occ = 0;
        const hipError_t e = hipOccupancyMaxActiveBlocksPerMultiprocessor(&occ, k_demod_mfma<D, STAMP>, RD_MF_WG, 0);
        return (e == hipSuccess && occ >= 1) ? (occ > 8 ? 8 : occ) : 2;
    }();
    const int per_cu = (P.per_cu_env >= 1 && P.per_cu_env <= 8) ? P.per_cu_env : per_cu_occ;
    uint32_t chunk = P.chunk_env > 0 ? (uint32_t)P.chunk_env : ((P.stflags & 4096) ? 28 : 8);
    if (P.chunk_env <= 0) {
        const uint64_t waves = (uint64_t)P.n_cu * per_cu * RD_MF_WAVES;
        while (chunk > RD_MF_STAGE_TILES && a.total64 / chunk < waves) chunk -= RD_MF_STAGE_TILES;
    }
    if (chunk > a.total) chunk = a.total;
    const uint64_t chunks = (a.total64 + chunk - 1) / chunk;
    uint64_t wgs = (chunks + RD_MF_WAVES - 1) / RD_MF_WAVES;
    const uint64_t max_wgs = (uint64_t)P.n_cu * per_cu;
    if (wgs > max_wgs) wgs = max_wgs;
    float *dbg = a.dbg_g;
    uint32_t stf = P.stflags;
    if (a.bucket_cnt && D == 0 && !STAMP) { dbg = (float *)a.bucket_cnt; stf |= RD_STF_BUCKETS; }
    if (a.chunk_out) { a.chunk_out[0] = chunk; a.chunk_out[1] = (uint32_t)wgs * RD_MF_WAVES; }
#ifdef RD_DIAG
    if (STAMP) {
        const uint32_t nw = (uint32_t)wgs * RD_MF_WAVES;
        if (nw > g_stamp_waves || !g_stamp_buf) {
            if (g_stamp_buf) hipFree(g_stamp_buf);
            g_stamp_buf = nullptr;
            if (hipMalloc(&g_stamp_buf, (size_t)nw * RD_STAMP_WORDS * 8) != hipSuccess) g_stamp_buf = nullptr;
        }
        g_stamp_waves = g_stamp_buf ? nw : 0;
        dbg = (float *)g_stamp_buf;
    }
#endif
    if (a.ev_start || a.ev_stop)
        hipExtLaunchKernelGGL((k_demod_mfma<D, STAMP>), dim3((unsigned)wgs), dim3(RD_MF_WG), 0, a.st, a.ev_start,
                              a.ev_stop, 0, a.lay, a.tps, a.total, chunk, a.fix_list, a.fix_cap, a.counters, dbg, stf);
    else
        hipLaunchKernelGGL((k_demod_mfma<D, STAMP>), dim3((unsigned)wgs), dim3(RD_MF_WG), 0, a.st, a.lay, a.tps, a.total,
                           chunk, a.fix_list, a.fix_cap, a.counters, dbg, stf);
}

bool rd_launch_demod_mfma(const rd_layout &lay, uint32_t *fix_list, uint32_t fix_cap, uint32_t *counters, hipStream_t st,
                          hipEvent_t ev_start, hipEvent_t ev_stop, float *dbg_g, uint32_t flags, uint32_t *chunk_out,
                          uint32_t *bucket_cnt) {
    rd_mf_launch_args a;
    a.chunk_out = chunk_out;
    a.bucket_cnt = (flags & RD_DEMOD_FIX_BUCKETS) && !dbg_g ? bucket_cnt : nullptr;
    a.lay = lay;
    a.tps = (lay.n_samples + RD_TILE_SAMPLES - 1) / RD_TILE_SAMPLES;
    a.total64 = (uint64_t)lay.n_streams * a.tps;
    if (a.total64 == 0) return a.bucket_cnt != nullptr;
    a.total = (uint32_t)a.total64;
    a.fix_list = fix_list; a.fix_cap = fix_cap; a.counters = counters;
    a.st = st; a.ev_start = ev_start; a.ev_stop = ev_stop; a.dbg_g = dbg_g;
    if (dbg_g) {
        rd_mf_launch_variant<3, false>(a);
        return false;
    }
#ifdef RD_DIAG
    const rd_mf_params &P = rd_mf_get_params();
    if (P.stamp || P.dbg) {
        a.bucket_cnt = nullptr;
        if (P.stamp && P.dbg == 0) { rd_mf_launch_variant<0, true>(a); return false; }
        switch (P.dbg) {
            case 1: rd_mf_launch_variant<1, false>(a); return false;
            case 2: rd_mf_launch_variant<2, false>(a); return false;
            case 6: rd_mf_launch_variant<6, false>(a); return false;
            case 7: rd_mf_launch_variant<7, false>(a); return false;
            case 8: rd_mf_launch_variant<8, false>(a); return false;
            case 9: rd_mf_launch_variant<9, false>(a); return false;
            case 10: rd_mf_launch_variant<10, false>(a); return false;
            case 11: rd_mf_launch_variant<11, false>(a); return false;
            default:
                fprintf(stderr, "[rd diag] no kernel variant RD_K1_DEBUG=%d RD_K1_STAMPS=%d is compiled in\n", P.dbg, P.stamp);
                abort();
        }
    }
#endif
    rd_mf_launch_variant<0, false>(a);
    return a.bucket_cnt != nullptr;
}

extern "C" int rd_debug_demod_mfma(const uint8_t *iq_host, int n_streams, uint32_t n_samples, int hist_mode,
                                   uint32_t hist_bytes, float *g_out, uint32_t *bits_out, uint32_t *fix_out,
                                   uint32_t fix_cap, uint32_t *n_fix) {
    int rc = rd_ensure_device_public();
    if (rc) return rc;
    const size_t stride = (size_t)n_samples * 2 + (hist_mode ? hist_bytes : 0);
    if (stride % 16 || (hist_mode && hist_bytes % 16)) return RD_ERR_ARG;
    const uint32_t tps = (n_samples + RD_TILE_SAMPLES - 1) / RD_TILE_SAMPLES;
    const size_t words = (n_samples + 31) / 32;
    const size_t iq_bytes = stride * n_streams;
    uint8_t *d_iq = nullptr;
    uint32_t *d_bits = nullptr, *d_fix = nullptr, *d_cnt = nullptr;
    float *d_g = nullptr;
    const size_t g_floats = (size_t)n_streams * tps * RD_TILE_SAMPLES * 2;
#define RD_DBG_CHK(x) do { if ((x) != hipSuccess) { rc = RD_ERR_DEVICE; goto out; } } while (0)
    RD_DBG_CHK(hipMalloc(&d_iq, iq_bytes + RD_INPUT_PAD));
    RD_DBG_CHK(hipMemset(d_iq + iq_bytes, 127, RD_INPUT_PAD));
    RD_DBG_CHK(hipMemcpy(d_iq, iq_host, iq_bytes, hipMemcpyHostToDevice));
    RD_DBG_CHK(hipMalloc(&d_bits, words * n_streams * 4));
    RD_DBG_CHK(hipMemset(d_bits, 0, words * n_streams * 4));
    RD_DBG_CHK(hipMalloc(&d_fix, (size_t)fix_cap * 4 + 4));
    RD_DBG_CHK(hipMalloc(&d_cnt, RD_CNT_TOTAL * 4));
    RD_DBG_CHK(hipMemset(d_cnt, 0, RD_CNT_TOTAL * 4));
    RD_DBG_CHK(hipMalloc(&d_g, g_floats * 4));
    RD_DBG_CHK(hipMemset(d_g, 0, g_floats * 4));
    {
        rd_layout lay;
        lay.iq = d_iq + (hist_mode ? hist_bytes : 0);
        lay.stream_stride = stride;
        lay.n_streams = n_streams;
        lay.n_samples = n_samples;
        lay.hist_mode = hist_mode;
        lay.valid_from = hist_mode ? -(long)(hist_bytes / 2) : 0;
        lay.bits = d_bits;
        lay.bits_stride = words;
        rd_launch_demod_mfma(lay, d_fix, fix_cap, d_cnt, nullptr, nullptr, nullptr, d_g);
    }
    RD_DBG_CHK(hipDeviceSynchronize());
    RD_DBG_CHK(hipMemcpy(g_out, d_g, g_floats * 4, hipMemcpyDeviceToHost));
    RD_DBG_CHK(hipMemcpy(bits_out, d_bits, words * n_streams * 4, hipMemcpyDeviceToHost));
    {
        uint32_t cnt[RD_CNT_SLOTS];
        RD_DBG_CHK(hipMemcpy(cnt, d_cnt, sizeof cnt, hipMemcpyDeviceToHost));
        *n_fix = cnt[RD_CNT_FIX];
        const uint32_t have = cnt[RD_CNT_FIX] < fix_cap ? cnt[RD_CNT_FIX] : fix_cap;
        if (have) RD_DBG_CHK(hipMemcpy(fix_out, d_fix, (size_t)have * 4, hipMemcpyDeviceToHost));
    }
out:
#undef RD_DBG_CHK
    hipFree(d_iq); hipFree(d_bits); hipFree(d_fix); hipFree(d_cnt); hipFree(d_g);
    return rc;
}
```

### rtldavis_amd/csrc/rd_internal.h

```cpp
#pragma once
#include <hip/hip_runtime.h>
#include <stdint.h>

#include "../../include/rtldavis_hip.h"
#include "rd_host.h"

enum { RD_CNT_FIX = 0, RD_CNT_MATCH = 1, RD_CNT_REC = 2, RD_CNT_TASKS = 3, RD_CNT_PARSED = 4, RD_CNT_OVF = 5, RD_CNT_SLOTS = 8 };
#define RD_DEMOD_FIX_BUCKETS 4u
#define RD_FT_GSH 2
#define RD_FT_STREAMS (1 << RD_FT_GSH)
struct rd_ft_bufs {
    uint32_t *fixb = nullptr;
    uint32_t *fixcnt = nullptr;
    uint32_t fix_bcap = 0;
    uint32_t bcap = 0;
    uint32_t *gstate = nullptr;
};
#define RD_NQUEUE 32
#define RD_QUEUE_STRIDE 64
#define RD_CNT_QUEUE0 RD_QUEUE_STRIDE
#define RD_CNT_TOTAL (RD_CNT_QUEUE0 + RD_NQUEUE * RD_QUEUE_STRIDE)

#define RD_TILE_SAMPLES 2048
#define RD_TILE_BYTES 4096
#define RD_INPUT_PAD 8192

struct rd_layout {
    const uint8_t *iq;
    size_t stream_stride;
    int n_streams;
    uint32_t n_samples;
    int hist_mode;
    long valid_from;
    uint32_t *bits;
    size_t bits_stride;
};


struct rd_match {
    int32_t stream;
    int32_t pos;
};

int rd_ensure_device_public(void);

uint32_t rd_launch_demod(const rd_layout &lay, uint32_t *fix_list, uint32_t fix_cap, uint32_t *counters, hipStream_t st,
                         hipEvent_t ev_start = nullptr, hipEvent_t ev_stop = nullptr, uint32_t flags = 0,
                         uint32_t *chunk_out = nullptr, uint32_t *bucket_cnt = nullptr);
bool rd_launch_demod_mfma(const rd_layout &lay, uint32_t *fix_list, uint32_t fix_cap, uint32_t *counters, hipStream_t st,
                          hipEvent_t ev_start = nullptr, hipEvent_t ev_stop = nullptr, float *dbg_g = nullptr,
                          uint32_t flags = 0, uint32_t *chunk_out = nullptr, uint32_t *bucket_cnt = nullptr);
void rd_launch_fixup(const rd_layout &lay, const uint32_t *fix_list, uint32_t fix_cap, uint32_t *counters, int all,
                     uint32_t *zero_next, hipStream_t st, uint32_t zero_words = RD_CNT_TOTAL, uint64_t expect = 0);
void rd_launch_search(const uint32_t *bits, size_t bits_stride, int n_streams, long n_bits, long p_lo, long p_hi,
                      const rd_devcfg &cfg, rd_match *matches, uint32_t match_cap, uint32_t *counters,
                      hipStream_t st);
int rd_launch_tail_fused(const rd_layout &lay, const rd_devcfg &cfg, int n_calls, long p_lo, long p_hi, const rd_ft_bufs &fb,
                         uint32_t bucket_limit, uint32_t seq, int skip_fix, rd_packet *recs, uint32_t rec_cap, uint32_t *counters,
                         hipStream_t st, hipEvent_t ev_stop = nullptr, uint32_t *zero_next = nullptr, uint32_t zero_words = 0);
int rd_launch_slice(const rd_layout &lay, const uint32_t *bits, size_t bits_stride, long n_bits, const rd_devcfg &cfg,
                     const rd_match *matches, uint32_t match_cap, int batch_mode, int n_calls, int call,
                     rd_packet *recs, rd_packet *recs_host, uint32_t *counters, hipStream_t st,
                     hipEvent_t ev_stop = nullptr, void *tasks = nullptr);
#define RD_TASK_BYTES 16
void rd_launch_parse(const rd_layout &lay, const rd_devcfg &cfg, const rd_packet *recs, uint32_t match_cap,
                     rd_parsed *parsed, uint32_t *counters, hipStream_t st, int dense = 0);
void rd_launch_disc(const rd_layout &lay, int stream, long t0, long n, double *out, hipStream_t st);
void rd_launch_filtered(const rd_layout &lay, int stream, long t0, long n, double *out, hipStream_t st);
void rd_launch_window_update(uint32_t *win_out, const uint32_t *win_in, long n_win_bits, const uint32_t *block,
                             long n_block_bits, int n_streams, size_t win_stride, size_t block_stride,
                             hipStream_t st);

#define RD_SB_THREADS 1024
#ifndef RD_SBC_THREADS
#define RD_SBC_THREADS 256
#endif
struct rd_sb_args {
    rd_devcfg cfg;
    uint8_t *ring;
    size_t ring_stride;
    const uint8_t *in;
    const uint32_t *win_in;
    uint32_t *win_out;
    rd_packet *recs_host;
    uint32_t *cnt_host;
    uint32_t *flag_host;
    uint32_t seq;
    long seen_before;
    uint64_t *stamps;
};
int rd_launch_stream_block(const rd_sb_args &a, int n_streams, hipStream_t st);

struct rd_sbc_args {
    rd_devcfg cfg;
    double *ring;
    const void *in;
    int in_is_u8;
    const uint32_t *win_in;
    uint32_t *win_out;
    rd_packet *recs_host;
    uint32_t *cnt_host, *flag_host;
    uint32_t seq;
    long seen_before;
    uint32_t *sync;
    uint64_t *stamps;
};
int rd_launch_stream_block_cplx(const rd_sbc_args &a, hipStream_t st);

struct rd_cplx_layout {
    const double *x;
    long valid_from;
    long n;
};
void rd_launch_cplx_bits(const rd_cplx_layout &lay, uint32_t *bits, hipStream_t st);
void rd_launch_cplx_disc(const rd_cplx_layout &lay, long t0, long n, double *out, hipStream_t st);
void rd_launch_cplx_filtered(const rd_cplx_layout &lay, long t0, long n, double *out, hipStream_t st);
void rd_launch_cplx_slice(const rd_cplx_layout &lay, const uint32_t *bits, long n_bits, const rd_devcfg &cfg,
                          const rd_match *matches, uint32_t match_cap, int call, rd_packet *recs, rd_packet *recs_host,
                          uint32_t *counters, hipStream_t st);
void rd_launch_lut(const uint8_t *in, double *out, size_t n_cplx, hipStream_t st);

void rd_launch_rotate(const double *in, double *out, size_t n, hipStream_t st);
void rd_launch_fir9(const double *in, double *out, size_t n_out, hipStream_t st);
void rd_launch_discriminate(const double *in, double *out, size_t n_out, hipStream_t st);
void rd_launch_quantize(const double *in, uint8_t *out, size_t n, hipStream_t st);
void rd_launch_pack_bytes(const uint8_t *in01, uint32_t *words, size_t n, hipStream_t st);

int rd_chan_stream_prepare(rd_chan *h);
int rd_chan_stream_launch(rd_chan *h, const uint8_t *wide, const uint8_t *prev, size_t n_out, uint64_t t_base, void *dst,
                          size_t dst_stride, hipStream_t st);
int rd_chan_n_channels(const rd_chan *h);
int rd_chan_bytes_per_sample(const rd_chan *h);
int rd_demod_prepare(rd_demod *h, hipStream_t *st, hipStream_t *st_copy);
int rd_demod_check_room(rd_demod *h);
int rd_demod_submit_device(rd_demod *h, const uint8_t *dev_block);
int rd_demod_pending(const rd_demod *h);
```

### rtldavis_amd/csrc/rd_kernels.hip

```cpp
#include <algorithm>
#include <cstdlib>

#include <hip/hip_ext.h>

#include "rd_internal.h"
#include "rd_math.h"
#include "rd_mfma.h"

uint32_t rd_launch_demod(const rd_layout &lay, uint32_t *fix_list, uint32_t fix_cap, uint32_t *counters, hipStream_t st,
                         hipEvent_t ev_start, hipEvent_t ev_stop, uint32_t flags, uint32_t *chunk_out, uint32_t *bucket_cnt) {
    if (!bucket_cnt) flags &= ~RD_DEMOD_FIX_BUCKETS;
    const bool bucketed = rd_launch_demod_mfma(lay, fix_list, fix_cap, counters, st, ev_start, ev_stop, nullptr, flags, chunk_out, bucket_cnt);
    return bucketed ? RD_DEMOD_FIX_BUCKETS : 0u;
}

__global__ __launch_bounds__(256) void k_fixup(rd_layout lay, uint32_t runs_per_stream, const uint32_t *fix_list,
                                               uint32_t fix_cap, const uint32_t *counters, int all,
                                               uint32_t *zero_next, uint32_t zero_words) {
    if (zero_next && blockIdx.x == 0)
        for (uint32_t i = threadIdx.x; i < zero_words; i += blockDim.x) zero_next[i] = 0;
    uint64_t count;
    if (all) {
        count = (uint64_t)lay.n_streams * runs_per_stream;
    } else {
        count = counters[RD_CNT_FIX];
        if (count > fix_cap) count = fix_cap;
    }
    const uint64_t stride = (uint64_t)gridDim.x * blockDim.x;
    for (uint64_t i = (uint64_t)blockIdx.x * blockDim.x + threadIdx.x; i < count; i += stride) {
        rd_stream_view v;
        v.valid_from = lay.valid_from;
        v.n = lay.n_samples;
        if (all) {
            const uint32_t s = (uint32_t)(i / runs_per_stream);
            const uint32_t run = (uint32_t)(i - (uint64_t)s * runs_per_stream);
            const long t0 = (long)run * RD_RUN;
            v.base = lay.iq + (size_t)s * lay.stream_stride;
            const long left = (long)lay.n_samples - t0;
            lay.bits[(size_t)s * lay.bits_stride + run] = rd_exact_run(v, t0, left < RD_RUN ? (int)left : RD_RUN);
        } else {
            const uint32_t e = fix_list[i];
            const uint32_t widx = e >> 4;
            const uint32_t s = widx / (uint32_t)lay.bits_stride;
            const uint32_t run = widx - s * (uint32_t)lay.bits_stride;
            v.base = lay.iq + (size_t)s * lay.stream_stride;
            for (int g = 0; g < RD_GROUPS; g++) {
                if (!((e >> g) & 1)) continue;
                const long t0 = (long)run * RD_RUN + g * RD_GROUP;
                const long left = (long)lay.n_samples - t0;
                if (left <= 0) break;
                const int count = left < RD_GROUP ? (int)left : RD_GROUP;
                const uint8_t *p = v.base + 2 * (t0 - 10);
                uint32_t dw[10];
                const long x = v.valid_from - (t0 - 10), z = (long)lay.n_samples + 8 - (t0 - 10);
                const int d_lo = x <= 0 ? 0 : x >= 20 ? 10 : (int)(x / 2);
                const int d_hi = z <= 0 ? 0 : z >= 20 ? 10 : (int)((z + 1) / 2);
#pragma unroll
                for (int d = 0; d < 10; d++) dw[d] = (d >= d_lo && d < d_hi) ? *(const uint32_t *)(p + 4 * d) : 0u;
                ((uint8_t *)lay.bits)[(size_t)widx * 4 + g] = (uint8_t)rd_exact_group_dw(dw, t0, count, v.valid_from);
            }
        }
    }
}

void rd_launch_fixup(const rd_layout &lay, const uint32_t *fix_list, uint32_t fix_cap, uint32_t *counters, int all,
                     uint32_t *zero_next, hipStream_t st, uint32_t zero_words, uint64_t expect) {
    const uint32_t rps = (lay.n_samples + RD_RUN - 1) / RD_RUN;
    if (rps == 0 || lay.n_streams == 0) return;
    uint64_t want = all ? (uint64_t)lay.n_streams * rps : fix_cap;
    if (!all && expect > 0) want = std::min<uint64_t>(want, std::max<uint64_t>(expect + expect / 4, 256 * 256));
    uint64_t wgs = (want + 255) / 256;
    if (wgs > 256ull * 16) wgs = 256ull * 16;
    if (wgs == 0) wgs = 1;
    hipLaunchKernelGGL(k_fixup, dim3((unsigned)wgs), dim3(256), 0, st, lay, rps, fix_list, fix_cap, counters, all,
                       zero_next, zero_words);
}

__device__ __forceinline__ uint32_t rd_word_at(const uint32_t *w, long nwords, long i) {
    return (i >= 0 && i < nwords) ? w[i] : 0u;
}

__device__ __forceinline__ uint32_t rd_bits32_at(const uint32_t *w, long nwords, long o) {
    const long wi = o >> 5;
    const uint32_t sh = (uint32_t)(o & 31);
    const uint32_t lo = rd_word_at(w, nwords, wi);
    const uint32_t hi = rd_word_at(w, nwords, wi + 1);
    return __builtin_amdgcn_alignbit(hi, lo, sh);
}

__device__ __forceinline__ uint32_t rd_bits32_at_i(const uint32_t *w, int nwords, int o) {
    const int wi = o >> 5;
    const uint32_t lo = (wi >= 0 && wi < nwords) ? w[wi] : 0u;
    const uint32_t hi = (wi + 1 >= 0 && wi + 1 < nwords) ? w[wi + 1] : 0u;
    return __builtin_amdgcn_alignbit(hi, lo, (uint32_t)(o & 31));
}

// ... 635 lines not shown
                tasks[t++] = tk;
            };
            put(t, pb, pq);
            if (use0 && use1) put(t, b1, q1);
        }
    }
}

__global__ __launch_bounds__(256) void k_rssi_u8(rd_layout lay, rd_devcfg cfg, const rd_task *tasks, uint32_t task_cap,
                                                 rd_packet *recs, const uint32_t *counters) {
    const int lane = threadIdx.x & 63;
    const uint32_t nw = gridDim.x * (blockDim.x >> 6);
    const uint32_t i0 = blockIdx.x * (blockDim.x >> 6) + (threadIdx.x >> 6);
    rd_k_h8 Ahi[3], Alo[3];
#pragma unroll
    for (int d = 0; d < 3; d++) {
        Ahi[d] = *(const rd_k_h8 *)g_rssi_taps.v[0][d][lane];
        Alo[d] = *(const rd_k_h8 *)g_rssi_taps.v[1][d][lane];
    }
    rd_task t_cur = {0, 0, 0, 0}, t_nxt = {0, 0, 0, 0};
    if (i0 < task_cap) t_cur = tasks[i0];
    if (i0 + nw < task_cap) t_nxt = tasks[i0 + nw];
    uint32_t count = counters[RD_CNT_TASKS];
    if (count > task_cap) count = task_cap;
    auto view = [&](int stream) {
        rd_stream_view v;
        v.base = lay.iq + (size_t)stream * lay.stream_stride;
        v.valid_from = lay.valid_from;
        v.n = lay.n_samples;
        return v;
    };
    auto job_of = [&](const rd_task &t) {
        const int stream = __builtin_amdgcn_readfirstlane(t.stream), call = __builtin_amdgcn_readfirstlane(t.call),
                  q = __builtin_amdgcn_readfirstlane(t.q);
        return rd_rssi_prepare(view(stream), call * cfg.B, cfg, q, lane);
    };
    rd_rssi_job j_cur = {};
    rd_rssi_data d_cur = {};
    if (i0 < count) {
        j_cur = job_of(t_cur);
        if (j_cur.ok) d_cur = rd_rssi_fetch(j_cur);
    }
    for (uint32_t i = i0; i < count; i += nw) {
        const rd_task t_now = t_cur;
        const rd_rssi_job j_now = j_cur;
        const rd_rssi_data d_now = d_cur;
        if (i + nw < count) {
            j_cur = job_of(t_nxt);
            if (j_cur.ok) d_cur = rd_rssi_fetch(j_cur);
        }
        t_cur = t_nxt;
        if (i + 2 * nw < task_cap) t_nxt = tasks[i + 2 * nw];
        const uint32_t rec = __builtin_amdgcn_readfirstlane(t_now.rec);
        double rssi = 0.0, snr = 0.0;
        if (j_now.ok) {
            float noise, sig;
            rd_rssi_block(j_now, d_now, Ahi, Alo, lane, noise, sig);
            rd_rssi_finish(noise, sig, j_now.ns, j_now.pe, j_now.q, lane, rssi, snr);
        } else {
            const int stream = __builtin_amdgcn_readfirstlane(t_now.stream);
            rd_rssi_u8(view(stream), (long)__builtin_amdgcn_readfirstlane(t_now.call) * cfg.B, cfg,
                       (long)__builtin_amdgcn_readfirstlane(t_now.q), lane, rssi, snr);
        }
        if (lane == 0) { recs[rec].rssi = rssi; recs[rec].snr = snr; }
    }
}

#define RD_FT_WG 256
#ifndef RD_FT_DEPTH
#define RD_FT_DEPTH 5
#endif
struct rd_ft_args {
    rd_layout lay;
    rd_devcfg cfg;
    int n_calls;
    int p_hi;
    int skip_fix;
    const uint32_t *fixb;
    const uint32_t *fixcnt;
    uint32_t fix_bcap;
    uint32_t bcap;
    uint32_t bucket_limit;
    uint32_t *gstate;
    uint32_t seq;
    rd_packet *recs;
    uint32_t rec_cap;
    uint32_t *counters;
    uint32_t *zero_next;
    uint32_t zero_words;
    uint64_t *stamps;
    int abl;
};
#ifdef RD_DIAG
#define RD_FT_STAMP(k) do { if (a.stamps && (tid & 63) == 0) { uint64_t t_; asm volatile("s_memrealtime %0\n\ts_waitcnt lgkmcnt(0)" : "=s"(t_) : : "memory"); \
                                                               a.stamps[(size_t)grp * 8 + (k)] = t_; } } while (0)
#else
#define RD_FT_STAMP(k) do { } while (0)
#endif

template <int S_, int T>
__device__ __forceinline__ uint32_t rd_tap(const uint32_t *r, int o) {
    constexpr int wj = (T * S_) >> 5, sh = (T * S_) & 31;
    return sh ? __builtin_amdgcn_alignbit(r[o + wj + 1], r[o + wj], sh) : r[o + wj];
}
constexpr int rd_tt3(bool pa, bool pb, bool pc) { return (pa ? 0xF0 : 0x0F) & (pb ? 0xCC : 0x33) & (pc ? 0xAA : 0x55); }
template <int S_, int P_, uint64_t PRE_, int T>
__device__ __forceinline__ uint32_t rd_match_from(uint32_t m, const uint32_t *r, int o) {
    if constexpr (T >= P_) {
        return m;
    } else if constexpr (T + 1 == P_) {
        const uint32_t v = rd_tap<S_, T>(r, o);
        return __builtin_amdgcn_bitop3_b32(m, v, v, rd_tt3(true, (PRE_ >> T) & 1, (PRE_ >> T) & 1));
    } else {
        const uint32_t n = __builtin_amdgcn_bitop3_b32(m, rd_tap<S_, T>(r, o), rd_tap<S_, T + 1>(r, o),
                                                       rd_tt3(true, (PRE_ >> T) & 1, (PRE_ >> (T + 1)) & 1));
        return rd_match_from<S_, P_, PRE_, T + 2>(n, r, o);
    }
}
template <int S_, int P_, uint64_t PRE_>
__device__ __forceinline__ uint32_t rd_match_word(const uint32_t *r, int o) {
    static_assert(P_ >= 3, "three taps in the first instruction");
    const uint32_t m = __builtin_amdgcn_bitop3_b32(rd_tap<S_, 0>(r, o), rd_tap<S_, 1>(r, o), rd_tap<S_, 2>(r, o),
                                                   rd_tt3(PRE_ & 1, (PRE_ >> 1) & 1, (PRE_ >> 2) & 1));
    return rd_match_from<S_, P_, PRE_, 3>(m, r, o);
}

__device__ __forceinline__ void rd_barrier_lds() { asm volatile("s_waitcnt lgkmcnt(0)\n\ts_barrier" ::: "memory"); }

template <int S_, int P_, uint64_t PRE_, int K_>
__global__ __launch_bounds__(RD_FT_WG, 4) void k_tail(rd_ft_args a) {
    constexpr int G = RD_FT_STREAMS;
    static_assert(PRE_ & 1, "positions below 0 are skipped because the preamble starts with a one");
    static_assert(RD_FT_WG == 64 * G, "one wave per stream in the classify strips");
    extern __shared__ __attribute__((aligned(16))) uint32_t s_dyn[];
    uint32_t *s_t = s_dyn;
    int32_t *s_pos = (int32_t *)(s_dyn + (size_t)G * a.bcap * 8);
    uint32_t *s_ord = s_dyn + (size_t)G * a.bcap * 9;
    __shared__ uint32_t s_cnt[G], s_kept[G];
    __shared__ uint32_t s_ready;
    const int tid = threadIdx.x, lane = tid & 63, wave = __builtin_amdgcn_readfirstlane(tid >> 6);
    const int grp = blockIdx.x, n_groups = gridDim.x;
    const int stream0 = grp * G;
    const int n_here = a.lay.n_streams - stream0 < G ? a.lay.n_streams - stream0 : G;
    const int nwords = (int)((a.lay.n_samples + 31) / 32);
    if (grp == 0 && a.zero_next)
        for (uint32_t i = tid; i < a.zero_words; i += RD_FT_WG) a.zero_next[i] = 0;
    if (tid < G) { s_cnt[tid] = 0; s_kept[tid] = 0; }
    if (tid == 0) s_ready = 0;
    const int prio_q = (int)(((unsigned)grp * 4u) / (unsigned)n_groups);
    if (wave == 0) RD_FT_STAMP(0);

    uint32_t n_fix_raw = 0;
    if (!a.skip_fix) {
        const uint32_t *bk = a.fixb + (size_t)grp * a.fix_bcap;
        const uint32_t e_first = (uint32_t)tid < a.fix_bcap ? bk[tid] : 0u;
        n_fix_raw = a.fixcnt[grp];
        const uint32_t n_fix = n_fix_raw < a.fix_bcap ? n_fix_raw : a.fix_bcap;
        uint32_t *s_items = s_t;
        __shared__ uint32_t s_nitems;
        static_assert(RD_GROUPS == 4, "an entry lists up to four groups");
        for (uint32_t i0 = 0; i0 < n_fix; i0 += RD_FT_WG) {
            if (tid == 0) s_nitems = 0;
            __syncthreads();
            const uint32_t i = i0 + (uint32_t)tid;
            const uint32_t e = i < n_fix ? (i0 == 0 ? e_first : bk[i]) : 0u;
            const uint32_t k = (uint32_t)__popc(e & 0xFu);
            if (k) {
                uint32_t at = atomicAdd(&s_nitems, k);
                for (int g = 0; g < RD_GROUPS; g++)
                    if ((e >> g) & 1) s_items[at++] = ((uint32_t)tid << 2) | (uint32_t)g;
                s_items[4 * RD_FT_WG + tid] = e;
            }
            __syncthreads();
            const uint32_t n_items = s_nitems;
            for (uint32_t it = (uint32_t)tid; it < n_items; it += RD_FT_WG) {
                const uint32_t item = s_items[it];
                const uint32_t ee = s_items[4 * RD_FT_WG + (item >> 2)];
                const int g = (int)(item & 3u);
                const uint32_t widx = ee >> 4;
                const uint32_t s = widx / (uint32_t)a.lay.bits_stride;
                const uint32_t run = widx - s * (uint32_t)a.lay.bits_stride;
                const uint8_t *base = a.lay.iq + (size_t)s * a.lay.stream_stride;
                const long t0 = (long)run * RD_RUN + g * RD_GROUP;
                const long left = (long)a.lay.n_samples - t0;
                if (left <= 0) continue;
                const int count = left < RD_GROUP ? (int)left : RD_GROUP;
                const uint8_t *p = base + 2 * (t0 - 10);
                uint32_t dw[10];
                const long x = a.lay.valid_from - (t0 - 10), z = (long)a.lay.n_samples + 8 - (t0 - 10);
                const int d_lo = x <= 0 ? 0 : x >= 20 ? 10 : (int)(x / 2);
                const int d_hi = z <= 0 ? 0 : z >= 20 ? 10 : (int)((z + 1) / 2);
#pragma unroll
                for (int d = 0; d < 10; d++) dw[d] = (d >= d_lo && d < d_hi) ? *(const uint32_t *)(p + 4 * d) : 0u;
                ((uint8_t *)a.lay.bits)[(size_t)widx * 4 + g] = (uint8_t)rd_exact_group_dw(dw, t0, count, a.lay.valid_from);
            }
            if (i0 + RD_FT_WG < n_fix) __syncthreads();
        }
    }
    __syncthreads();
    if (wave == 0) RD_FT_STAMP(1);

    {
        constexpr int NW = ((RD_SEARCH_OUT + ((P_ - 1) * S_ + 31) / 32 + 1 + 3) / 4) * 4;
        const int gps = a.p_hi / (32 * RD_SEARCH_OUT) + 1;
        const int wgps = (gps + 63) / 64;
        const int units = n_here * wgps;
        auto fetch = [&](int g, int rem, uint32_t (&r)[NW]) {
            const int gi = rem * 64 + lane;
            const uint32_t *w = a.lay.bits + (size_t)(stream0 + g) * a.lay.bits_stride;
            int w0 = RD_SEARCH_OUT * gi;
            w0 = w0 + NW <= nwords ? w0 : nwords - NW;
#pragma unroll
            for (int j = 0; j < NW / 4; j++) {
                const uint4 v4 = *(const uint4 *)(w + w0 + 4 * j);
                r[4 * j] = v4.x; r[4 * j + 1] = v4.y; r[4 * j + 2] = v4.z; r[4 * j + 3] = v4.w;
            }
        };
        auto test = [&](int g, int rem, const uint32_t (&r)[NW]) {
            const int gi = rem * 64 + lane;
            uint32_t m[RD_SEARCH_OUT] = {};
            const int p0 = 32 * RD_SEARCH_OUT * gi;
            if (gi < gps) {
#pragma unroll
                for (int o = 0; o < RD_SEARCH_OUT; o++) m[o] = rd_match_word<S_, P_, PRE_>(r, o);
                if (p0 + 32 * RD_SEARCH_OUT - 1 > a.p_hi) {
#pragma unroll
                    for (int o = 0; o < RD_SEARCH_OUT; o++) {
                        const int q0 = p0 + 32 * o;
                        if (q0 + 31 > a.p_hi) m[o] &= (a.p_hi < q0) ? 0u : (0xFFFFFFFFu >> (31 - (a.p_hi - q0)));
                    }
                }
            }
            uint32_t anym = 0;
#pragma unroll
            for (int o = 0; o < RD_SEARCH_OUT; o++) anym |= m[o];
            if (__ballot(anym != 0)) {
                uint32_t mine = 0;
#pragma unroll
                for (int o = 0; o < RD_SEARCH_OUT; o++) mine += (uint32_t)__popc(m[o]);
                uint32_t incl = mine;
#pragma unroll
                for (int sh = 1; sh < 64; sh <<= 1) {
                    const uint32_t up = (uint32_t)__shfl_up((int)incl, sh, 64);
                    if (lane >= sh) incl += up;
                }
                const uint32_t tot = (uint32_t)__shfl((int)incl, 63, 64);
                uint32_t slot0 = 0;
                if (lane == 0) slot0 = atomicAdd(&s_cnt[g], tot);
                uint32_t slot = (uint32_t)__builtin_amdgcn_readfirstlane((int)slot0) + incl - mine;
#pragma unroll
                for (int o = 0; o < RD_SEARCH_OUT; o++) {
                    uint32_t mm = m[o];
                    while (mm) {
                        const int bpos = __builtin_ctz(mm);
                        mm &= mm - 1;
                        if (slot < a.bcap) s_pos[(size_t)g * a.bcap + slot] = p0 + 32 * o + bpos;
                        slot++;
                    }
                }
            }
        };
        constexpr int DEPTH = RD_FT_DEPTH;
        uint32_t rb[DEPTH][NW];
        const int dq = G / wgps, dr = G % wgps;
        int fg = wave / wgps, fr = wave % wgps, fu = wave;
        int tg = fg, tr = fr, prio_k = 0;
        auto step = [&](int &gg, int &rr) { gg += dq; rr += dr; if (rr >= wgps) { rr -= wgps; gg++; } };
        auto fetch_next = [&](uint32_t (&r)[NW]) {
#ifdef RD_DIAG
            if (a.abl & 2) return;
#endif
            fetch(fg, fr, r);
            if (fu + G < units) { fu += G; step(fg, fr); }
        };
        auto test_next = [&](const uint32_t (&r)[NW]) {
#ifdef RD_DIAG
            if (a.abl & 1) { if (r[0] == 0x12345678u) s_cnt[0] = 1; step(tg, tr); return; }
#endif
            switch ((prio_q + prio_k++) & 3) {
                case 0: __builtin_amdgcn_s_setprio(0); break;
                case 1: __builtin_amdgcn_s_setprio(1); break;
                case 2: __builtin_amdgcn_s_setprio(2); break;
                default: __builtin_amdgcn_s_setprio(3); break;
            }
            test(tg, tr, r);
// ... 60 lines not shown
    }
    if (wave == 0) RD_FT_STAMP(7);
    for (uint32_t j = lane; j < ((count + 63) & ~63u); j += 64) {
        const bool live = j < count;
        const uint4 me = live ? *(const uint4 *)(tg + 8 * j) : uint4{0, 0, 0, 0};
        const uint4 md = live ? *(const uint4 *)(tg + 8 * j + 4) : uint4{0, 0, 0, 0};
        const int b0 = (int)me.y, b1 = b0 - 1;
        const uint32_t k0 = me.z, k1 = me.w;
        bool dup0 = false, dup1 = false;
        for (uint32_t i0 = 0; i0 < count; i0 += 4) {
            uint4 xa[4], da[4];
#pragma unroll
            for (int u = 0; u < 4; u++) {
                const uint32_t i = (i0 + u) < a.bcap ? i0 + u : i0;
                xa[u] = *(const uint4 *)(tg + 8 * i);
                da[u] = *(const uint4 *)(tg + 8 * i + 4);
            }
#pragma unroll
            for (int u = 0; u < 4; u++) {
                const uint32_t i = i0 + u;
                const uint4 x = xa[u], d = da[u];
                const int ob0 = (int)x.y;
                const bool lower = i < j;
                if (i < count && d.x == md.x && d.y == md.y && d.z == md.z) {
                    if ((x.x & 1u) && ob0 == b0 && (x.z < k0 || (x.z == k0 && lower))) dup0 = true;
                    if ((x.x & 2u) && ob0 - 1 == b0 && (x.w < k0 || (x.w == k0 && lower))) dup0 = true;
                    if ((x.x & 1u) && ob0 == b1 && (x.z < k1 || (x.z == k1 && lower))) dup1 = true;
                    if ((x.x & 2u) && ob0 - 1 == b1 && (x.w < k1 || (x.w == k1 && lower))) dup1 = true;
                }
            }
        }
        if (live) tg[8 * j + 7] = (((me.x & 1u) && !dup0) ? 1u : 0u) | (((me.x & 2u) && !dup1) ? 2u : 0u);
    }
    uint32_t kept_here = 0;
    for (uint32_t j = lane; j < ((count + 63) & ~63u); j += 64) {
        const bool live = j < count;
        const uint4 me = live ? *(const uint4 *)(tg + 8 * j) : uint4{0, 0, 0, 0};
        const uint32_t mk = live ? tg[8 * j + 7] : 0u;
        const int b0 = (int)me.y, b1 = b0 - 1;
        const uint32_t k0 = me.z, k1 = me.w;
        uint32_t r0 = 0, r1 = 0;
        for (uint32_t i0 = 0; i0 < count; i0 += 4) {
            uint4 xa[4];
            uint32_t ka[4];
#pragma unroll
            for (int u = 0; u < 4; u++) {
                const uint32_t i = (i0 + u) < a.bcap ? i0 + u : i0;
                xa[u] = *(const uint4 *)(tg + 8 * i);
                ka[u] = tg[8 * i + 7];
            }
#pragma unroll
            for (int u = 0; u < 4; u++) {
                const uint4 x = xa[u];
                const uint32_t xk = (i0 + u) < count ? ka[u] & 3u : 0u;
                const int ob0 = (int)x.y;
                auto before = [](int ca, uint32_t ka_, int cb, uint32_t kb) { return ca < cb || (ca == cb && ka_ < kb); };
                if (xk & 1u) { r0 += before(ob0, x.z, b0, k0) ? 1u : 0u; r1 += before(ob0, x.z, b1, k1) ? 1u : 0u; }
                if (xk & 2u) { r0 += before(ob0 - 1, x.w, b0, k0) ? 1u : 0u; r1 += before(ob0 - 1, x.w, b1, k1) ? 1u : 0u; }
            }
        }
        kept_here += (uint32_t)__popcll(__ballot((mk & 1u) != 0)) + (uint32_t)__popcll(__ballot((mk & 2u) != 0));
        if (live) tg[8 * j + 7] = mk | (r0 << 2) | (r1 << 17);
    }
    if (lane == 0) s_kept[g] = kept_here;
    if (ovf && lane == 0) atomicOr(&a.counters[RD_CNT_OVF], 1u);
    rd_barrier_lds();
    uint32_t off = 0, total = 0, mtotal = 0;
#pragma unroll
    for (int i = 0; i < G; i++) {
        off += i < g ? s_kept[i] : 0u;
        total += s_kept[i];
        mtotal += i < n_here ? s_cnt[i] : 0u;
    }
    for (uint32_t j = lane; j < count; j += 64) {
        const uint32_t res = tg[8 * j + 7];
        if (res & 1u) s_ord[off + ((res >> 2) & 0x7FFFu)] = ((uint32_t)g << 16) | (j << 1);
        if (res & 2u) s_ord[off + (res >> 17)] = ((uint32_t)g << 16) | (j << 1) | 1u;
    }
    const uint32_t tag = (a.seq & 0xFFFu) << 20;
    if (tid == 0) {
        __hip_atomic_store(&a.gstate[n_groups + grp], tag | (mtotal < 0xFFFFFu ? mtotal : 0xFFFFFu), __ATOMIC_RELAXED, __HIP_MEMORY_SCOPE_AGENT);
        __hip_atomic_store(&a.gstate[2 * n_groups + grp], tag | (n_fix_raw < 0xFFFFFu ? n_fix_raw : 0xFFFFFu), __ATOMIC_RELAXED,
                           __HIP_MEMORY_SCOPE_AGENT);
        __hip_atomic_store(&a.gstate[grp], tag | total, __ATOMIC_RELAXED, __HIP_MEMORY_SCOPE_AGENT);
        if (n_fix_raw > a.fix_bcap) atomicOr(&a.counters[RD_CNT_OVF], 8u);
    }
    rd_barrier_lds();
    if (wave == 0) RD_FT_STAMP(3);

    if (wave == G - 1) {
        uint32_t polls = 0;
        bool gave_up = false;
        auto tagged = [&](const uint32_t *p) -> uint32_t {
            for (;;) {
                const uint32_t v = __hip_atomic_load(p, __ATOMIC_RELAXED, __HIP_MEMORY_SCOPE_AGENT);
                if ((v & 0xFFF00000u) == tag) return v & 0xFFFFFu;
                if (++polls > (1u << 22)) { gave_up = true; return 0u; }
                __builtin_amdgcn_s_sleep(8);
            }
        };
        uint32_t sum = 0;
        for (int j0 = 0; j0 < grp; j0 += 1024) {
            uint32_t v[16];
#pragma unroll
            for (int k = 0; k < 16; k++) {
                const int j = j0 + lane + 64 * k;
                v[k] = j < grp ? __hip_atomic_load(&a.gstate[j], __ATOMIC_RELAXED, __HIP_MEMORY_SCOPE_AGENT) : tag;
            }
#pragma unroll
            for (int k = 0; k < 16; k++) {
                if ((v[k] & 0xFFF00000u) != tag) v[k] = tag | tagged(&a.gstate[j0 + lane + 64 * k]);
                sum += v[k] & 0xFFFFFu;
            }
        }
#pragma unroll
        for (int o = 32; o > 0; o >>= 1) sum += (uint32_t)__shfl_xor((int)sum, o, 64);
        if (lane == 0) __hip_atomic_store(&s_ready, sum + 1u, __ATOMIC_RELAXED, __HIP_MEMORY_SCOPE_WORKGROUP);
        if (grp == n_groups - 1) {
            uint32_t mt = 0, ft = 0;
            for (int i0 = 0; i0 < n_groups; i0 += 512) {
                uint32_t vm[8], vf[8];
#pragma unroll
                for (int k = 0; k < 8; k++) {
                    const int i = i0 + lane + 64 * k;
                    vm[k] = i < n_groups ? __hip_atomic_load(&a.gstate[n_groups + i], __ATOMIC_RELAXED, __HIP_MEMORY_SCOPE_AGENT) : tag;
                    vf[k] = i < n_groups ? __hip_atomic_load(&a.gstate[2 * n_groups + i], __ATOMIC_RELAXED, __HIP_MEMORY_SCOPE_AGENT) : tag;
                }
#pragma unroll
                for (int k = 0; k < 8; k++) {
                    const int i = i0 + lane + 64 * k;
                    if ((vm[k] & 0xFFF00000u) != tag) vm[k] = tagged(&a.gstate[n_groups + i]);
                    if ((vf[k] & 0xFFF00000u) != tag) vf[k] = tagged(&a.gstate[2 * n_groups + i]);
                    mt += vm[k] & 0xFFFFFu;
                    ft += vf[k] & 0xFFFFFu;
                }
            }
#pragma unroll
            for (int o = 32; o > 0; o >>= 1) {
                mt += (uint32_t)__shfl_xor((int)mt, o, 64);
                ft += (uint32_t)__shfl_xor((int)ft, o, 64);
            }
            if (lane == 0) {
                a.counters[RD_CNT_TASKS] = sum + total;
                a.counters[RD_CNT_MATCH] = mt;
                a.counters[RD_CNT_FIX] = ft;
                if (sum + total > a.rec_cap) atomicOr(&a.counters[RD_CNT_OVF], 2u);
            }
        }
        if (__ballot(gave_up) && lane == 0) atomicOr(&a.counters[RD_CNT_OVF], 16u);
        RD_FT_STAMP(4);
    }
    float *s_res = (float *)(s_dyn + (size_t)G * a.bcap * 11);
    if ((uint32_t)wave < total) {
        rd_k_h8 Ahi[3], Alo[3];
#pragma unroll
        for (int d = 0; d < 3; d++) {
            Ahi[d] = *(const rd_k_h8 *)g_rssi_taps.v[0][d][lane];
            Alo[d] = *(const rd_k_h8 *)g_rssi_taps.v[1][d][lane];
        }
        struct task { int stream, call, q; };
        auto task_at = [&](uint32_t r) {
            const uint32_t o = s_ord[r];
            const uint32_t *e = s_t + ((size_t)(o >> 16) * a.bcap + ((o >> 1) & 0x7FFFu)) * 8;
            task t;
            t.stream = stream0 + (int)(o >> 16);
            t.call = (int)e[1] - (int)(o & 1u);
            t.q = (int)(e[2] & 0xFFFFFFu) + ((o & 1u) ? B : 0);
            return t;
        };
        auto view = [&](int s) {
            rd_stream_view v;
            v.base = a.lay.iq + (size_t)s * a.lay.stream_stride;
            v.valid_from = a.lay.valid_from;
            v.n = a.lay.n_samples;
            return v;
        };
        auto job_of = [&](const task &t) {
            return rd_rssi_prepare(view(__builtin_amdgcn_readfirstlane(t.stream)), __builtin_amdgcn_readfirstlane(t.call) * B, a.cfg,
                                   __builtin_amdgcn_readfirstlane(t.q), lane);
        };
        task t_cur = task_at((uint32_t)wave);
        rd_rssi_job j_cur = job_of(t_cur);
        rd_rssi_data d_cur = {};
        if (j_cur.ok) d_cur = rd_rssi_fetch(j_cur);
        for (uint32_t r = (uint32_t)wave; r < total; r += G) {
            const task t_now = t_cur;
            const rd_rssi_job j_now = j_cur;
            const rd_rssi_data d_now = d_cur;
            if (r + G < total) {
                t_cur = task_at(r + G);
                j_cur = job_of(t_cur);
                if (j_cur.ok) d_cur = rd_rssi_fetch(j_cur);
            }
            double rssi = 0.0, snr = 0.0;
            if (j_now.ok) {
                float noise, sig;
                rd_rssi_block(j_now, d_now, Ahi, Alo, lane, noise, sig);
                rd_rssi_finish(noise, sig, j_now.ns, j_now.pe, j_now.q, lane, rssi, snr);
            } else {
                rd_rssi_u8(view(__builtin_amdgcn_readfirstlane(t_now.stream)), (long)__builtin_amdgcn_readfirstlane(t_now.call) * B, a.cfg,
                           (long)__builtin_amdgcn_readfirstlane(t_now.q), lane, rssi, snr);
            }
            if (lane == 0) { s_res[2 * r] = (float)rssi; s_res[2 * r + 1] = (float)snr; }
        }
    }
    rd_barrier_lds();
    if ((uint32_t)tid < total) {
        uint32_t spins = 0, v = 0;
        while (!(v = __hip_atomic_load(&s_ready, __ATOMIC_RELAXED, __HIP_MEMORY_SCOPE_WORKGROUP)) && ++spins < (1u << 24))
            __builtin_amdgcn_s_sleep(2);
        const uint32_t first = v - 1u;
        for (uint32_t r = (uint32_t)tid; r < total; r += RD_FT_WG) {
            const uint32_t o = s_ord[r];
            const uint32_t *e = s_t + ((size_t)(o >> 16) * a.bcap + ((o >> 1) & 0x7FFFu)) * 8;
            const uint4 x = *(const uint4 *)e, d = *(const uint4 *)(e + 4);
            const uint32_t at = first + r;
            if (at < a.rec_cap) {
                const double rssi = (double)s_res[2 * r], snr = (double)s_res[2 * r + 1];
                uint4 *out = (uint4 *)&a.recs[at];
                out[0] = uint4{(uint32_t)(stream0 + (int)(o >> 16)), (uint32_t)((int)x.y - (int)(o & 1u)),
                               (uint32_t)((int)(x.z & 0xFFFFFFu) + ((o & 1u) ? B : 0)), (uint32_t)a.cfg.nbytes};
                out[1] = uint4{d.x, d.y, d.z, 0u};
                out[2] = uint4{0u, 0u, 0u, 0u};
                const uint2 rb = __builtin_bit_cast(uint2, rssi), sb = __builtin_bit_cast(uint2, snr);
                out[3] = uint4{rb.x, rb.y, sb.x, sb.y};
            }
        }
    }
    if (wave == 0) RD_FT_STAMP(5);
}

#ifdef RD_DIAG
static uint64_t *g_ft_stamps = nullptr;
static uint32_t g_ft_groups = 0;
extern "C" int rd_diag_read_tail_stamps(uint64_t *out, uint32_t cap_groups, uint32_t *n_groups) {
    if (!g_ft_stamps || !n_groups) return RD_ERR_STATE;
    if (hipDeviceSynchronize() != hipSuccess) return RD_ERR_DEVICE;
    *n_groups = g_ft_groups;
    const uint32_t n = g_ft_groups < cap_groups ? g_ft_groups : cap_groups;
    if (n && hipMemcpy(out, g_ft_stamps, (size_t)n * 64, hipMemcpyDeviceToHost) != hipSuccess) return RD_ERR_DEVICE;
    return RD_OK;
}
#endif

size_t rd_tail_fused_lds(uint32_t bcap) { return (size_t)RD_FT_STREAMS * bcap * (8 + 1 + 2 + 4) * sizeof(uint32_t); }

int rd_launch_tail_fused(const rd_layout &lay, const rd_devcfg &cfg, int n_calls, long p_lo, long p_hi, const rd_ft_bufs &fb,
                         uint32_t bucket_limit, uint32_t seq, int skip_fix, rd_packet *recs, uint32_t rec_cap, uint32_t *counters,
                         hipStream_t st, hipEvent_t ev_stop, uint32_t *zero_next, uint32_t zero_words) {
    const long n_bits = lay.n_samples;
    if (!(cfg.S == 14 && cfg.P == 16 && cfg.K == 80 && cfg.pre_mask == 0x91D3ull) || n_bits >= (1l << 30) || cfg.B >= (1 << 24) ||
        lay.n_streams <= 0 || p_lo > 0 || p_hi < 0 || p_hi >= (1l << 30) || !fb.gstate || !fb.fixb || fb.bcap == 0 || fb.bcap % 32 ||
        fb.bcap > RD_BUCKET_MAX || lay.bits_stride % 4 || ((size_t)lay.bits % 16) || lay.hist_mode ||
        p_hi / 32 + 16 > (n_bits + 31) / 32)
        return 0;
    rd_ft_args a;
    a.lay = lay; a.cfg = cfg; a.n_calls = n_calls; a.p_hi = (int)p_hi; a.skip_fix = skip_fix;
    a.fixb = fb.fixb; a.fixcnt = fb.fixcnt; a.fix_bcap = fb.fix_bcap;
    a.bcap = fb.bcap; a.bucket_limit = bucket_limit < fb.bcap ? bucket_limit : fb.bcap;
    a.gstate = fb.gstate; a.seq = seq;
    a.recs = recs; a.rec_cap = rec_cap; a.counters = counters; a.zero_next = zero_next; a.zero_words = zero_words;
    a.stamps = nullptr;
    a.abl = 0;
    const uint32_t groups = (uint32_t)(lay.n_streams + RD_FT_STREAMS - 1) / RD_FT_STREAMS;
#ifdef RD_DIAG
    if (const char *e = getenv("RD_FT_ABL")) a.abl = atoi(e);
    if (getenv("RD_FT_STAMPS")) {
        if (groups > g_ft_groups) { if (g_ft_stamps) hipFree(g_ft_stamps); g_ft_stamps = nullptr; if (hipMalloc(&g_ft_stamps, (size_t)groups * 64) != hipSuccess) g_ft_stamps = nullptr; }
        g_ft_groups = g_ft_stamps ? groups : 0;
        a.stamps = g_ft_stamps;
    }
#endif
    const size_t lds = std::max<size_t>(rd_tail_fused_lds(fb.bcap), 33 * 1024);
    static bool attr_set = false;
    if (lds > 48 * 1024 && !attr_set) {
        hipFuncSetAttribute((const void *)k_tail<14, 16, 0x91D3ull, 80>, hipFuncAttributeMaxDynamicSharedMemorySize, 150 * 1024);
        attr_set = true;
    }
    if (ev_stop)
        hipExtLaunchKernelGGL((k_tail<14, 16, 0x91D3ull, 80>), dim3(groups), dim3(RD_FT_WG), (unsigned)lds, st, nullptr, ev_stop, 0, a);
    else
        hipLaunchKernelGGL((k_tail<14, 16, 0x91D3ull, 80>), dim3(groups), dim3(RD_FT_WG), (unsigned)lds, st, a);
    return 1;
}

static uint32_t rd_slice_grid(uint32_t match_cap) {
    uint32_t wgs = (match_cap + 3) / 4;
    if (wgs > 4096) wgs = 4096;
    return wgs ? wgs : 1;
}

int rd_launch_slice(const rd_layout &lay, const uint32_t *bits, size_t bits_stride, long n_bits, const rd_devcfg &cfg,
                    const rd_match *matches, uint32_t match_cap, int batch_mode, int n_calls, int call,
                    rd_packet *recs, rd_packet *recs_host, uint32_t *counters, hipStream_t st, hipEvent_t ev_stop,
                    void *tasks) {
    rd_u8_src src;
    src.lay = lay;
    if (tasks && batch_mode && recs && !recs_host && cfg.S == 14 && cfg.K == 80 && n_bits < (1l << 30)) {
        const uint32_t cg = std::min<uint32_t>((match_cap + 255) / 256, 1024);
        hipLaunchKernelGGL((k_classify<14, 80>), dim3(cg ? cg : 1), dim3(256), 0, st, bits, bits_stride,
                           (int)((n_bits + 31) / 32), cfg, matches, match_cap, n_calls, recs, (rd_task *)tasks, counters);
        const uint32_t rg = std::min<uint32_t>(rd_slice_grid(match_cap), 1024);
        if (ev_stop)
            hipExtLaunchKernelGGL(k_rssi_u8, dim3(rg), dim3(256), 0, st, nullptr, ev_stop, 0, lay, cfg,
                                  (const rd_task *)tasks, 2 * match_cap, recs, counters);
        else
            hipLaunchKernelGGL(k_rssi_u8, dim3(rg), dim3(256), 0, st, lay, cfg, (const rd_task *)tasks,
                               2 * match_cap, recs, counters);
        return 1;
    }
    if (ev_stop)
        hipExtLaunchKernelGGL(k_slice_rssi<rd_u8_src>, dim3(rd_slice_grid(match_cap)), dim3(256), 0, st, nullptr,
                              ev_stop, 0, src, bits, bits_stride, (n_bits + 31) / 32, cfg, matches, match_cap,
                              batch_mode, n_calls, call, recs, recs_host, counters);
    else
        hipLaunchKernelGGL(k_slice_rssi<rd_u8_src>, dim3(rd_slice_grid(match_cap)), dim3(256), 0, st, src, bits,
                           bits_stride, (n_bits + 31) / 32, cfg, matches, match_cap, batch_mode, n_calls, call, recs,
                           recs_host, counters);
    return 0;
}

__device__ __forceinline__ uint32_t rd_swap_bits8(uint32_t b) {
    b = ((b & 0xF0) >> 4) | ((b & 0x0F) << 4);
    b = ((b & 0xCC) >> 2) | ((b & 0x33) << 2);
    b = ((b & 0xAA) >> 1) | ((b & 0x55) << 1);
    return b;
}

__global__ __launch_bounds__(256) void k_parse_select(const rd_packet *recs, uint32_t match_cap, rd_parsed *parsed,
                                                      uint32_t *counters, int dense) {
    uint32_t nprim = counters[RD_CNT_MATCH], nextra = counters[RD_CNT_REC];
    if (nprim > match_cap) nprim = match_cap;
    if (nextra > match_cap) nextra = match_cap;
    if (dense) {
        nprim = counters[RD_CNT_TASKS];
        if (nprim > 2 * match_cap) nprim = 2 * match_cap;
        nextra = 0;
    }
    const uint32_t rec_cap = 2 * match_cap;
    const uint32_t i = blockIdx.x * blockDim.x + threadIdx.x;
    const int lane = threadIdx.x & 63;
    bool ok = false;
    uint8_t sw[RD_MAX_PKT_BYTES];
    int nb = 0;
    if ((i < nprim || (!dense && i >= match_cap && i - match_cap < nextra)) && recs[i].stream >= 0) {
        const rd_packet *r = &recs[i];
        nb = r->nbytes;
        uint32_t crc = 0;
#pragma unroll
        for (int k = 0; k < RD_MAX_PKT_BYTES; k++) {
            const uint32_t b = k < nb ? rd_swap_bits8(r->data[k]) : 0u;
            sw[k] = (uint8_t)b;
            if (k >= 2 && k < nb) {
                crc ^= b << 8;
#pragma unroll
                for (int j = 0; j < 8; j++) crc = (crc & 0x8000) ? ((crc << 1) ^ 0x1021) & 0xFFFF : (crc << 1) & 0xFFFF;
// ... 656 lines not shown
```

Measured before the change: 2.063 million MS/s.

## Fuse preamble search into demod kernel with tail handling boundary candidates

The demod MFMA kernel now keeps a per-wave LDS ring of recent bit words and tests each produced word against the preamble. Matches go into a per-group list. The tail kernel then only searches the words the demod did not own (flagged or tile-boundary words) and merges in the demod's matches. The goal is to avoid a separate pass that re-reads the whole packed bit stream to search for preambles. In exchange it adds LDS use and instructions to the demod kernel, which may lower occupancy, plus atomics for emitting matches and more tail-kernel LDS for a bitmap.

```diff
diff --git a/include/rtldavis_hip.h b/include/rtldavis_hip.h
--- a/include/rtldavis_hip.h
+++ b/include/rtldavis_hip.h
@@ -106,6 +106,7 @@
 #define RD_FORM_ONE_LAUNCH_TAIL 16u
 int rd_batch_last_run_forms(rd_batch *b, uint32_t *forms);
 int rd_batch_get_counters(rd_batch *b, uint64_t *fixup_runs, uint64_t *matches);
+int rd_batch_get_search_counters(rd_batch *b, uint64_t *demod_found, uint64_t *tail_found);
 
 int rd_lut_execute(const uint8_t *in_bytes, size_t n_bytes, double *out_cplx, size_t n_cplx);
 int rd_rotate_fs4(const double *in_cplx, double *out_cplx, size_t n_cplx);
diff --git a/rtldavis_amd/_lib.py b/rtldavis_amd/_lib.py
--- a/rtldavis_amd/_lib.py
+++ b/rtldavis_amd/_lib.py
@@ -106,6 +106,7 @@
     "rd_batch_last_run_forms": (C.c_int, [_P, C.POINTER(C.c_uint32)]),
     "rd_batch_get_timing": (C.c_int, [_P, C.POINTER(RdTiming)]),
     "rd_batch_get_counters": (C.c_int, [_P, C.POINTER(C.c_uint64), C.POINTER(C.c_uint64)]),
+    "rd_batch_get_search_counters": (C.c_int, [_P, C.POINTER(C.c_uint64), C.POINTER(C.c_uint64)]),
     "rd_lut_execute": (C.c_int, [_P, C.c_size_t, _P, C.c_size_t]),
     "rd_rotate_fs4": (C.c_int, [_P, _P, C.c_size_t]),
     "rd_fir9": (C.c_int, [_P, C.c_size_t, _P, C.c_size_t]),
diff --git a/rtldavis_amd/batch.py b/rtldavis_amd/batch.py
--- a/rtldavis_amd/batch.py
+++ b/rtldavis_amd/batch.py
@@ -99,6 +99,11 @@
         _lib.check(_lib.lib().rd_batch_get_counters(self._b, C.byref(f), C.byref(m)))
         return {"fixup_runs": f.value, "matches": m.value}
 
+    def search_counters(self) -> dict:
+        d, t = C.c_uint64(), C.c_uint64()
+        _lib.check(_lib.lib().rd_batch_get_search_counters(self._b, C.byref(d), C.byref(t)))
+        return {"demod_found": d.value, "tail_found": t.value}
+
     def results(self) -> np.ndarray:
         L = _lib.lib()
         n = C.c_int(0)
diff --git a/rtldavis_amd/csrc/rd_api.hip b/rtldavis_amd/csrc/rd_api.hip
--- a/rtldavis_amd/csrc/rd_api.hip
+++ b/rtldavis_amd/csrc/rd_api.hip
@@ -170,6 +170,11 @@
     uint32_t ft_seq = 0, ft_limit = 0;
     bool ft_sticky = false;
     size_t ft_cnt_off = 0;
+    uint32_t *d_fsl = nullptr;
+    uint32_t fs_cap = 0;
+    size_t fs_cnt_off = 0;
+    bool fs_run = false;
+    uint64_t last_dmatch = 0;
     bool second_pass = false;
     uint32_t last_launch[2] = {0, 0};
     bool pipelined = false;
@@ -267,8 +272,15 @@
         }
         b->ft.bcap = rd_ord_bucket_cap(b->n_samples);
         HIPCHK(hipMalloc(&b->ft.fixb, groups * b->ft.fix_bcap * sizeof(uint32_t)));
-        HIPCHK(hipMalloc(&b->ft.gstate, 3 * groups * sizeof(uint32_t)));
-        HIPCHK(hipMemset(b->ft.gstate, 0, 3 * groups * sizeof(uint32_t)));
+        HIPCHK(hipMalloc(&b->ft.gstate, RD_FT_GSTATE_ROWS * groups * sizeof(uint32_t)));
+        HIPCHK(hipMemset(b->ft.gstate, 0, RD_FT_GSTATE_ROWS * groups * sizeof(uint32_t)));
+        const char *fse = getenv("RD_FUSED_SEARCH");
+        if (!(fse && fse[0] == '0')) {
+            b->fs_cap = 4 * RD_FT_STREAMS * b->ft.bcap;
+            b->fs_cnt_off = b->cnt_stride;
+            b->cnt_stride += (groups + 3) & ~(size_t)3;
+            HIPCHK(hipMalloc(&b->d_fsl, groups * b->fs_cap * sizeof(uint32_t)));
+        }
     }
     HIPCHK(hipMalloc(&b->d_cnt, 2 * b->cnt_stride * sizeof(uint32_t)));
     HIPCHK(hipMemset(b->d_cnt, 0, 2 * b->cnt_stride * sizeof(uint32_t)));
@@ -301,7 +313,7 @@
         hipFree(b->d_iq); hipFree(b->d_bits); hipFree(b->d_fix); hipFree(b->d_cnt);
         hipFree(b->d_matches); hipFree(b->d_recs); hipFree(b->d_tasks);
         hipFree(b->d_parsed);
-        hipFree(b->ft.fixb); hipFree(b->ft.gstate);
+        hipFree(b->ft.fixb); hipFree(b->ft.gstate); hipFree(b->d_fsl);
         hipHostFree(b->h_cnt_pin); hipHostFree(b->h_recs_pin);
         if (b->done) hipEventDestroy(b->done);
         if (b->kdone) hipEventDestroy(b->kdone);
@@ -412,6 +424,7 @@
     if (b->ft_run && may_defer) {
         rd_ft_bufs fb = b->ft;
         fb.fixcnt = batch_cnt(b) + b->ft_cnt_off;
+        if (b->fs_run) { fb.fsl = b->d_fsl; fb.fscnt = batch_cnt(b) + b->fs_cnt_off; fb.fs_cap = b->fs_cap; }
         b->ft_seq = b->ft_seq % 4095u + 1u;
         const int ok = rd_launch_tail_fused(lay, b->dc, b->n_blocks, B - L, (long)(b->n_blocks + 1) * B - L, fb,
                                             b->ft_limit ? b->ft_limit : fb.bcap, b->ft_seq, 0, b->d_recs, b->rec_cap, batch_cnt(b), st,
@@ -483,19 +496,26 @@
     }
     const bool adopt = batch_stream_has_tail(b->device, st);
     const bool want_ft = b->ft_ok && b->fast_ok && !b->tail_off && !(b->timing && b->timing_detail);
-    const uint32_t dflags = want_ft ? RD_DEMOD_FIX_BUCKETS : 0u;
+    const bool want_fs = want_ft && b->d_fsl && rd_tail_fused_search_fits(b->ft.bcap, (uint32_t)b->n_samples);
+    const uint32_t dflags = want_ft ? (RD_DEMOD_FIX_BUCKETS | (want_fs ? RD_DEMOD_FUSED_SEARCH : 0u)) : 0u;
+    rd_fs_out fso;
+    if (want_fs) {
+        fso.list = b->d_fsl; fso.cnt = cnt + b->fs_cnt_off; fso.cap = b->fs_cap;
+        fso.p_hi = (int)((long)(b->n_blocks + 1) * b->dc.B - b->dc.L);
+    }
+    const rd_fs_out *fsp = want_fs ? &fso : nullptr;
     uint32_t *fixl = want_ft ? b->ft.fixb : b->d_fix, *bcnt = want_ft ? cnt + b->ft_cnt_off : nullptr;
     const uint32_t fixc = want_ft ? b->ft.fix_bcap : b->fix_cap;
     uint32_t honoured = 0;
     if (b->timing && b->fast_ok) {
-        honoured = rd_launch_demod(lay, fixl, fixc, cnt, st, b->ev[0], b->ev[1], dflags, b->last_launch, bcnt);
+        honoured = rd_launch_demod(lay, fixl, fixc, cnt, st, b->ev[0], b->ev[1], dflags, b->last_launch, bcnt, fsp);
         if (adopt && (rc = batch_adopt(b->device, st, b->ev[1]))) return rc;
     } else if (b->fast_ok && adopt) {
-        honoured = rd_launch_demod(lay, fixl, fixc, cnt, st, nullptr, b->kfirst, dflags, b->last_launch, bcnt);
+        honoured = rd_launch_demod(lay, fixl, fixc, cnt, st, nullptr, b->kfirst, dflags, b->last_launch, bcnt, fsp);
         if ((rc = batch_adopt(b->device, st, b->kfirst))) return rc;
     } else {
         if (b->timing) HIPCHK(hipEventRecord(b->ev[0], st));
-        if (b->fast_ok) honoured = rd_launch_demod(lay, fixl, fixc, cnt, st, nullptr, nullptr, dflags, b->last_launch, bcnt);
+        if (b->fast_ok) honoured = rd_launch_demod(lay, fixl, fixc, cnt, st, nullptr, nullptr, dflags, b->last_launch, bcnt, fsp);
         if (b->timing) HIPCHK(hipEventRecord(b->ev[1], st));
         if (adopt) {
             hipEvent_t carrier = b->timing ? b->ev[1] : b->kfirst;
@@ -505,6 +525,7 @@
     }
     b->second_pass = false;
     b->ft_run = b->fast_ok && (honoured & RD_DEMOD_FIX_BUCKETS);
+    b->fs_run = b->ft_run && (honoured & RD_DEMOD_FUSED_SEARCH);
     if (!b->ft_run)
         rd_launch_fixup(lay, fixl, fixc, cnt, b->fast_ok ? 0 : 1, cnt_next, st, (uint32_t)b->cnt_stride, b->last_fix);
     if (b->timing && b->timing_detail) HIPCHK(hipEventRecord(b->ev[2], st));
@@ -588,6 +609,7 @@
         }
         if (!redo_search) {
             b->last_match = b->h_cnt[RD_CNT_MATCH];
+            b->last_dmatch = (b->fs_run && b->dev_order && !b->second_pass) ? b->h_cnt[RD_CNT_DMATCH] : 0;
             b->fetched = true;
             return RD_OK;
         }
@@ -784,6 +806,15 @@
     if (rc) return rc;
     if (fixup_runs) *fixup_runs = b->last_fix;
     if (matches) *matches = b->last_match;
+    return RD_OK;
+}
+
+extern "C" int rd_batch_get_search_counters(rd_batch *b, uint64_t *demod_found, uint64_t *tail_found) {
+    if (!b) return fail(RD_ERR_ARG, "null batch");
+    int rc = batch_finish(b);
+    if (rc) return rc;
+    if (demod_found) *demod_found = b->last_dmatch;
+    if (tail_found) *tail_found = b->last_match - b->last_dmatch;
     return RD_OK;
 }
 
diff --git a/rtldavis_amd/csrc/rd_demod_mfma.hip b/rtldavis_amd/csrc/rd_demod_mfma.hip
--- a/rtldavis_amd/csrc/rd_demod_mfma.hip
+++ b/rtldavis_amd/csrc/rd_demod_mfma.hip
@@ -7,6 +7,7 @@
 #include "rd_internal.h"
 #include "rd_math.h"
 #include "rd_mfma.h"
+#include "rd_search.h"
 
 #define RD_MF_WG 256
 #define RD_MF_WAVES (RD_MF_WG / 64)
@@ -18,6 +19,8 @@
 #define RD_MF_IMG_PAD 4624
 #define RD_MF_XB_BYTES (3 * 1024 + 32 + 32)
 #define RD_MF_PEND 32
+#define RD_MF_MPEND 64
+#define RD_MF_RING 72
 #ifndef RD_MF_STAGE_TILES
 #define RD_MF_STAGE_TILES 4
 #endif
@@ -296,6 +299,60 @@
         if (base + i < fix_cap) fix_list[base + i] = pend[i];
 }
 
+template <int S_, int P_, uint64_t PRE_>
+__device__ __forceinline__ uint32_t rd_fs_test_tile(uint32_t ring_addr, uint32_t wi, uint32_t word, uint32_t flagged) {
+    static_assert(((P_ - 1) * S_ + 31) / 32 + 1 == RD_FS_SPAN, "the ring's history covers a position's taps");
+    asm volatile("ds_write_b64 %0, %1" : : "v"(ring_addr + 8 * (8 + wi)), "v"(rd_u2v{word, flagged}) : "memory");
+    uint32_t r[8];
+    asm volatile("ds_read2_b32 %0, %4 offset0:2 offset1:4\n\tds_read2_b32 %1, %4 offset0:6 offset1:8\n\t"
+                 "ds_read2_b32 %2, %4 offset0:10 offset1:12\n\tds_read2_b32 %3, %4 offset0:14 offset1:16\n\t"
+                 "s_waitcnt lgkmcnt(0)"
+                 : "=&v"(*(rd_u2v *)&r[0]), "=&v"(*(rd_u2v *)&r[2]), "=&v"(*(rd_u2v *)&r[4]), "=&v"(*(rd_u2v *)&r[6])
+                 : "v"(ring_addr + 8 * wi) : "memory");
+    return rd_match_word<S_, P_, PRE_>(r, 0);
+}
+__device__ __forceinline__ void rd_fs_flush(const uint32_t *mpend, uint32_t count, const rd_fs_out &fs) {
+    const int lane = rd_lane_now();
+    asm volatile("s_waitcnt lgkmcnt(0)" ::: "memory");
+    for (uint32_t i = lane; i < count; i += 64) {
+        const uint32_t s = mpend[2 * i], pos = mpend[2 * i + 1];
+        const uint32_t grp = s >> RD_FT_GSH;
+        const uint32_t slot = atomicAdd(&fs.cnt[grp], 1u);
+        if (slot < fs.cap) fs.list[(size_t)grp * fs.cap + slot] = ((s & (RD_FT_STREAMS - 1)) << 30) | pos;
+    }
+}
+__device__ __forceinline__ void rd_fs_emit(uint32_t ring_addr, uint32_t wi, uint32_t m, uint32_t s, uint32_t ti, const rd_fs_out &fs,
+                                           uint32_t *mpend, uint32_t &npm) {
+    const long v = rd_fs_demod_word(ti, wi);
+    uint32_t keep = 0;
+    if (m) {
+        uint32_t f[8];
+        asm volatile("ds_read2_b32 %0, %4 offset0:3 offset1:5\n\tds_read2_b32 %1, %4 offset0:7 offset1:9\n\t"
+                     "ds_read2_b32 %2, %4 offset0:11 offset1:13\n\tds_read2_b32 %3, %4 offset0:15 offset1:17\n\t"
+                     "s_waitcnt lgkmcnt(0)"
+                     : "=&v"(*(rd_u2v *)&f[0]), "=&v"(*(rd_u2v *)&f[2]), "=&v"(*(rd_u2v *)&f[4]), "=&v"(*(rd_u2v *)&f[6])
+                     : "v"(ring_addr + 8 * wi) : "memory");
+        uint32_t dirty8 = 0;
+#pragma unroll
+        for (int k = 0; k < 8; k++) dirty8 |= f[k] ? 1u << k : 0u;
+        if (rd_fs_demod_owns(dirty8, true)) keep = m & rd_fs_range_mask(v, fs.p_hi);
+    }
+    const uint32_t mp_addr = rd_lds_addr(mpend);
+    for (;;) {
+        const uint64_t bm = __ballot(keep != 0);
+        if (!bm) break;
+        const uint32_t nf = (uint32_t)__popcll(bm);
+        if (npm + nf > RD_MF_MPEND) { rd_fs_flush(mpend, npm, fs); npm = 0; }
+        if (keep) {
+            const uint32_t b = (uint32_t)__builtin_ctz(keep);
+            keep &= keep - 1;
+            const uint32_t at = npm + __builtin_amdgcn_mbcnt_hi((uint32_t)(bm >> 32), __builtin_amdgcn_mbcnt_lo((uint32_t)bm, 0));
+            asm volatile("ds_write_b64 %0, %1" : : "v"(mp_addr + 8 * at), "v"(rd_u2v{s, (uint32_t)(32 * v) + b}) : "memory");
+        }
+        npm += nf;
+    }
+}
+
 
 __device__ __forceinline__ void rd_mf_store_staged(uint32_t stage_addr, uint32_t nst, uint32_t *base, uint32_t stflags) {
     const int lane = rd_lane_now();
@@ -378,14 +435,17 @@
 
 #define RD_STAMP_WORDS 12
 #define RD_STF_BUCKETS 8192u
-template <int DBG, bool STAMP>
+template <int DBG, bool STAMP, bool FS>
 __global__ __launch_bounds__(RD_MF_WG, RD_MF_MINWAVES) void k_demod_mfma(rd_layout lay, uint32_t tiles_per_stream, uint32_t total_tiles,
                                                          uint32_t chunk, uint32_t *fix_list, uint32_t fix_cap,
-                                                         uint32_t *counters, float *dbg_g, uint32_t stflags) {
+                                                         uint32_t *counters, float *dbg_g, uint32_t stflags, rd_fs_out fs) {
+    static_assert(!FS || (DBG == 0 && !STAMP), "the fused search belongs to the product kernel");
     __shared__ __attribute__((aligned(16))) uint8_t s_img[RD_MF_WAVES][RD_MF_IMG_PAD];
     __shared__ __attribute__((aligned(32))) uint8_t s_xb[RD_MF_WAVES][RD_MF_XB_BYTES];
     __shared__ uint32_t s_pend[RD_MF_WAVES][RD_MF_PEND];
     __shared__ __attribute__((aligned(16))) uint32_t s_stage[RD_MF_WAVES][RD_MF_STAGE_TILES][64];
+    __shared__ __attribute__((aligned(8))) uint32_t s_ring[RD_MF_WAVES][2 * RD_MF_RING];
+    __shared__ __attribute__((aligned(8))) uint32_t s_mpend[RD_MF_WAVES][2 * RD_MF_MPEND];
     constexpr bool LOADS = DBG != 1;
     const int lane = threadIdx.x & 63;
     const int wave = __builtin_amdgcn_readfirstlane(threadIdx.x >> 6);
@@ -448,6 +508,7 @@
     cur.inchunk = 0;
     rd_mf_pos nx1 = rd_mf_next(cur, chunk, tiles_per_stream, nextc);
 
+    uint32_t npm = 0;
     uint32_t nst = 0;
     uint32_t *st_base = nullptr;
     bool st_flush = false;
@@ -556,6 +617,16 @@
             gmask = 0;
         }
         if (DBG == 1 || DBG == 2 || DBG == 6) gmask = 0;
+        if constexpr (FS) {
+            const uint32_t ring_addr = rd_lds_addr(s_ring[wave]);
+            const uint32_t wi = (uint32_t)(2 * n + h);
+            const uint32_t flagged = gmask != 0 ? 1u : 0u;
+            uint32_t m = rd_fs_test_tile<14, 16, 0x91D3ull>(ring_addr, wi, word, flagged);
+            if (!rd_fs_demod_one_wave(wi, carry)) m = 0;
+            if (rd_mf_any(m != 0)) rd_fs_emit(ring_addr, wi, m, s, ti, fs, s_mpend[wave], npm);
+            if (wi >= RD_FS_TILE_WORDS - 8)
+                asm volatile("ds_write_b64 %0, %1" : : "v"(ring_addr + 8 * (wi - (RD_FS_TILE_WORDS - 8))), "v"(rd_u2v{word, flagged}) : "memory");
+        }
         const uint64_t fm = (any_flag || !carry) ? __ballot(gmask != 0) : 0;
         if (fm) {
             const uint32_t nf = (uint32_t)__popcll(fm);
@@ -574,6 +645,9 @@
     }
     if (nst) rd_mf_store_staged(stage_addr, nst, st_base, stflags);
     if (npend) rd_mf_flush(mypend, npend, fix_list, fix_cap, counters, (uint32_t)lay.bits_stride, bucket_cnt);
+    if constexpr (FS) {
+        if (npm) rd_fs_flush(s_mpend[wave], npm, fs);
+    }
     if (STAMP && dbg_g) {
         const uint64_t t1 = rd_stamp(), r1 = rd_stamp_real();
         sm_comp += t1 - sm_mark;
@@ -644,16 +718,17 @@
     hipStream_t st;
     hipEvent_t ev_start, ev_stop;
     uint32_t *bucket_cnt = nullptr;
+    rd_fs_out fs;
     uint32_t *chunk_out = nullptr;
     float *dbg_g;
 };
 
-template <int D, bool STAMP>
+template <int D, bool STAMP, bool FS = false>
 static void rd_mf_launch_variant(const rd_mf_launch_args &a) {
     const rd_mf_params &P = rd_mf_get_params();
     static const int per_cu_occ = [] {
         int occ = 0;
-        const hipError_t e = hipOccupancyMaxActiveBlocksPerMultiprocessor(&occ, k_demod_mfma<D, STAMP>, RD_MF_WG, 0);
+        const hipError_t e = hipOccupancyMaxActiveBlocksPerMultiprocessor(&occ, k_demod_mfma<D, STAMP, FS>, RD_MF_WG, 0);
         return (e == hipSuccess && occ >= 1) ? (occ > 8 ? 8 : occ) : 2;
     }();
     const int per_cu = (P.per_cu_env >= 1 && P.per_cu_env <= 8) ? P.per_cu_env : per_cu_occ;
@@ -684,52 +759,60 @@
     }
 #endif
     if (a.ev_start || a.ev_stop)
-        hipExtLaunchKernelGGL((k_demod_mfma<D, STAMP>), dim3((unsigned)wgs), dim3(RD_MF_WG), 0, a.st, a.ev_start,
-                              a.ev_stop, 0, a.lay, a.tps, a.total, chunk, a.fix_list, a.fix_cap, a.counters, dbg, stf);
+        hipExtLaunchKernelGGL((k_demod_mfma<D, STAMP, FS>), dim3((unsigned)wgs), dim3(RD_MF_WG), 0, a.st, a.ev_start,
+                              a.ev_stop, 0, a.lay, a.tps, a.total, chunk, a.fix_list, a.fix_cap, a.counters, dbg, stf, a.fs);
     else
-        hipLaunchKernelGGL((k_demod_mfma<D, STAMP>), dim3((unsigned)wgs), dim3(RD_MF_WG), 0, a.st, a.lay, a.tps, a.total,
-                           chunk, a.fix_list, a.fix_cap, a.counters, dbg, stf);
-}
-
-bool rd_launch_demod_mfma(const rd_layout &lay, uint32_t *fix_list, uint32_t fix_cap, uint32_t *counters, hipStream_t st,
-                          hipEvent_t ev_start, hipEvent_t ev_stop, float *dbg_g, uint32_t flags, uint32_t *chunk_out,
-                          uint32_t *bucket_cnt) {
+        hipLaunchKernelGGL((k_demod_mfma<D, STAMP, FS>), dim3((unsigned)wgs), dim3(RD_MF_WG), 0, a.st, a.lay, a.tps, a.total,
+                           chunk, a.fix_list, a.fix_cap, a.counters, dbg, stf, a.fs);
+}
+
+uint32_t rd_launch_demod_mfma(const rd_layout &lay, uint32_t *fix_list, uint32_t fix_cap, uint32_t *counters, hipStream_t st,
+                              hipEvent_t ev_start, hipEvent_t ev_stop, float *dbg_g, uint32_t flags, uint32_t *chunk_out,
+                              uint32_t *bucket_cnt, const rd_fs_out *fs) {
     rd_mf_launch_args a;
     a.chunk_out = chunk_out;
     a.bucket_cnt = (flags & RD_DEMOD_FIX_BUCKETS) && !dbg_g ? bucket_cnt : nullptr;
+    const bool want_fs = (flags & RD_DEMOD_FUSED_SEARCH) && a.bucket_cnt && fs && fs->list && fs->cnt && fs->cap && fs->p_hi >= 0 &&
+                         lay.n_samples < (1u << 30);
+    const uint32_t all_flags = RD_DEMOD_FIX_BUCKETS | (want_fs ? RD_DEMOD_FUSED_SEARCH : 0u);
     a.lay = lay;
     a.tps = (lay.n_samples + RD_TILE_SAMPLES - 1) / RD_TILE_SAMPLES;
     a.total64 = (uint64_t)lay.n_streams * a.tps;
-    if (a.total64 == 0) return a.bucket_cnt != nullptr;
+    if (a.total64 == 0) return a.bucket_cnt ? all_flags : 0u;
     a.total = (uint32_t)a.total64;
     a.fix_list = fix_list; a.fix_cap = fix_cap; a.counters = counters;
     a.st = st; a.ev_start = ev_start; a.ev_stop = ev_stop; a.dbg_g = dbg_g;
     if (dbg_g) {
         rd_mf_launch_variant<3, false>(a);
-        return false;
+        return 0u;
     }
 #ifdef RD_DIAG
     const rd_mf_params &P = rd_mf_get_params();
     if (P.stamp || P.dbg) {
         a.bucket_cnt = nullptr;
-        if (P.stamp && P.dbg == 0) { rd_mf_launch_variant<0, true>(a); return false; }
+        if (P.stamp && P.dbg == 0) { rd_mf_launch_variant<0, true>(a); return 0u; }
         switch (P.dbg) {
-            case 1: rd_mf_launch_variant<1, false>(a); return false;
-            case 2: rd_mf_launch_variant<2, false>(a); return false;
-            case 6: rd_mf_launch_variant<6, false>(a); return false;
-            case 7: rd_mf_launch_variant<7, false>(a); return false;
-            case 8: rd_mf_launch_variant<8, false>(a); return false;
-            case 9: rd_mf_launch_variant<9, false>(a); return false;
-            case 10: rd_mf_launch_variant<10, false>(a); return false;
-            case 11: rd_mf_launch_variant<11, false>(a); return false;
+            case 1: rd_mf_launch_variant<1, false>(a); return 0u;
+            case 2: rd_mf_launch_variant<2, false>(a); return 0u;
+            case 6: rd_mf_launch_variant<6, false>(a); return 0u;
+            case 7: rd_mf_launch_variant<7, false>(a); return 0u;
+            case 8: rd_mf_launch_variant<8, false>(a); return 0u;
+            case 9: rd_mf_launch_variant<9, false>(a); return 0u;
+            case 10: rd_mf_launch_variant<10, false>(a); return 0u;
+            case 11: rd_mf_launch_variant<11, false>(a); return 0u;
             default:
                 fprintf(stderr, "[rd diag] no kernel variant RD_K1_DEBUG=%d RD_K1_STAMPS=%d is compiled in\n", P.dbg, P.stamp);
                 abort();
         }
     }
 #endif
-    rd_mf_launch_variant<0, false>(a);
-    return a.bucket_cnt != nullptr;
+    if (want_fs) {
+        a.fs = *fs;
+        rd_mf_launch_variant<0, false, true>(a);
+    } else {
+        rd_mf_launch_variant<0, false>(a);
+    }
+    return a.bucket_cnt ? all_flags : 0u;
 }
 
 extern "C" int rd_debug_demod_mfma(const uint8_t *iq_host, int n_streams, uint32_t n_samples, int hist_mode,
diff --git a/rtldavis_amd/csrc/rd_internal.h b/rtldavis_amd/csrc/rd_internal.h
--- a/rtldavis_amd/csrc/rd_internal.h
+++ b/rtldavis_amd/csrc/rd_internal.h
@@ -5,8 +5,15 @@
 #include "../../include/rtldavis_hip.h"
 #include "rd_host.h"
 
-enum { RD_CNT_FIX = 0, RD_CNT_MATCH = 1, RD_CNT_REC = 2, RD_CNT_TASKS = 3, RD_CNT_PARSED = 4, RD_CNT_OVF = 5, RD_CNT_SLOTS = 8 };
+enum { RD_CNT_FIX = 0, RD_CNT_MATCH = 1, RD_CNT_REC = 2, RD_CNT_TASKS = 3, RD_CNT_PARSED = 4, RD_CNT_OVF = 5, RD_CNT_DMATCH = 6,
+       RD_CNT_SLOTS = 8 };
 #define RD_DEMOD_FIX_BUCKETS 4u
+#define RD_DEMOD_FUSED_SEARCH 8u
+struct rd_fs_out {
+    uint32_t *list = nullptr, *cnt = nullptr;
+    uint32_t cap = 0;
+    int p_hi = -1;
+};
 #define RD_FT_GSH 2
 #define RD_FT_STREAMS (1 << RD_FT_GSH)
 struct rd_ft_bufs {
@@ -15,7 +22,11 @@
     uint32_t fix_bcap = 0;
     uint32_t bcap = 0;
     uint32_t *gstate = nullptr;
+    const uint32_t *fsl = nullptr;
+    const uint32_t *fscnt = nullptr;
+    uint32_t fs_cap = 0;
 };
+#define RD_FT_GSTATE_ROWS 4
 #define RD_NQUEUE 32
 #define RD_QUEUE_STRIDE 64
 #define RD_CNT_QUEUE0 RD_QUEUE_STRIDE
@@ -46,10 +57,11 @@
 
 uint32_t rd_launch_demod(const rd_layout &lay, uint32_t *fix_list, uint32_t fix_cap, uint32_t *counters, hipStream_t st,
                          hipEvent_t ev_start = nullptr, hipEvent_t ev_stop = nullptr, uint32_t flags = 0,
-                         uint32_t *chunk_out = nullptr, uint32_t *bucket_cnt = nullptr);
-bool rd_launch_demod_mfma(const rd_layout &lay, uint32_t *fix_list, uint32_t fix_cap, uint32_t *counters, hipStream_t st,
+                         uint32_t *chunk_out = nullptr, uint32_t *bucket_cnt = nullptr, const rd_fs_out *fs = nullptr);
+uint32_t rd_launch_demod_mfma(const rd_layout &lay, uint32_t *fix_list, uint32_t fix_cap, uint32_t *counters, hipStream_t st,
                           hipEvent_t ev_start = nullptr, hipEvent_t ev_stop = nullptr, float *dbg_g = nullptr,
-                          uint32_t flags = 0, uint32_t *chunk_out = nullptr, uint32_t *bucket_cnt = nullptr);
+                          uint32_t flags = 0, uint32_t *chunk_out = nullptr, uint32_t *bucket_cnt = nullptr,
+                          const rd_fs_out *fs = nullptr);
 void rd_launch_fixup(const rd_layout &lay, const uint32_t *fix_list, uint32_t fix_cap, uint32_t *counters, int all,
                      uint32_t *zero_next, hipStream_t st, uint32_t zero_words = RD_CNT_TOTAL, uint64_t expect = 0);
 void rd_launch_search(const uint32_t *bits, size_t bits_stride, int n_streams, long n_bits, long p_lo, long p_hi,
@@ -58,6 +70,7 @@
 int rd_launch_tail_fused(const rd_layout &lay, const rd_devcfg &cfg, int n_calls, long p_lo, long p_hi, const rd_ft_bufs &fb,
                          uint32_t bucket_limit, uint32_t seq, int skip_fix, rd_packet *recs, uint32_t rec_cap, uint32_t *counters,
                          hipStream_t st, hipEvent_t ev_stop = nullptr, uint32_t *zero_next = nullptr, uint32_t zero_words = 0);
+int rd_tail_fused_search_fits(uint32_t bcap, uint32_t n_samples);
 int rd_launch_slice(const rd_layout &lay, const uint32_t *bits, size_t bits_stride, long n_bits, const rd_devcfg &cfg,
                      const rd_match *matches, uint32_t match_cap, int batch_mode, int n_calls, int call,
                      rd_packet *recs, rd_packet *recs_host, uint32_t *counters, hipStream_t st,
diff --git a/rtldavis_amd/csrc/rd_kernels.hip b/rtldavis_amd/csrc/rd_kernels.hip
--- a/rtldavis_amd/csrc/rd_kernels.hip
+++ b/rtldavis_amd/csrc/rd_kernels.hip
@@ -6,12 +6,13 @@
 #include "rd_internal.h"
 #include "rd_math.h"
 #include "rd_mfma.h"
+#include "rd_search.h"
 
 uint32_t rd_launch_demod(const rd_layout &lay, uint32_t *fix_list, uint32_t fix_cap, uint32_t *counters, hipStream_t st,
-                         hipEvent_t ev_start, hipEvent_t ev_stop, uint32_t flags, uint32_t *chunk_out, uint32_t *bucket_cnt) {
-    if (!bucket_cnt) flags &= ~RD_DEMOD_FIX_BUCKETS;
-    const bool bucketed = rd_launch_demod_mfma(lay, fix_list, fix_cap, counters, st, ev_start, ev_stop, nullptr, flags, chunk_out, bucket_cnt);
-    return bucketed ? RD_DEMOD_FIX_BUCKETS : 0u;
+                         hipEvent_t ev_start, hipEvent_t ev_stop, uint32_t flags, uint32_t *chunk_out, uint32_t *bucket_cnt,
+                         const rd_fs_out *fs) {
+    if (!bucket_cnt) flags &= ~(RD_DEMOD_FIX_BUCKETS | RD_DEMOD_FUSED_SEARCH);
+    return rd_launch_demod_mfma(lay, fix_list, fix_cap, counters, st, ev_start, ev_stop, nullptr, flags, chunk_out, bucket_cnt, fs);
 }
 
 __global__ __launch_bounds__(256) void k_fixup(rd_layout lay, uint32_t runs_per_stream, const uint32_t *fix_list,
@@ -813,6 +814,11 @@
     uint32_t bcap;
     uint32_t bucket_limit;
     uint32_t *gstate;
+    const uint32_t *fsl;
+    const uint32_t *fscnt;
+    uint32_t fs_cap;
+    uint32_t bm_off, bm_words;
+    uint32_t tps;
     uint32_t seq;
     rd_packet *recs;
     uint32_t rec_cap;
@@ -829,32 +835,6 @@
 #define RD_FT_STAMP(k) do { } while (0)
 #endif
 
-template <int S_, int T>
-__device__ __forceinline__ uint32_t rd_tap(const uint32_t *r, int o) {
-    constexpr int wj = (T * S_) >> 5, sh = (T * S_) & 31;
-    return sh ? __builtin_amdgcn_alignbit(r[o + wj + 1], r[o + wj], sh) : r[o + wj];
-}
-constexpr int rd_tt3(bool pa, bool pb, bool pc) { return (pa ? 0xF0 : 0x0F) & (pb ? 0xCC : 0x33) & (pc ? 0xAA : 0x55); }
-template <int S_, int P_, uint64_t PRE_, int T>
-__device__ __forceinline__ uint32_t rd_match_from(uint32_t m, const uint32_t *r, int o) {
-    if constexpr (T >= P_) {
-        return m;
-    } else if constexpr (T + 1 == P_) {
-        const uint32_t v = rd_tap<S_, T>(r, o);
-        return __builtin_amdgcn_bitop3_b32(m, v, v, rd_tt3(true, (PRE_ >> T) & 1, (PRE_ >> T) & 1));
-    } else {
-        const uint32_t n = __builtin_amdgcn_bitop3_b32(m, rd_tap<S_, T>(r, o), rd_tap<S_, T + 1>(r, o),
-                                                       rd_tt3(true, (PRE_ >> T) & 1, (PRE_ >> (T + 1)) & 1));
-        return rd_match_from<S_, P_, PRE_, T + 2>(n, r, o);
-    }
-}
-template <int S_, int P_, uint64_t PRE_>
-__device__ __forceinline__ uint32_t rd_match_word(const uint32_t *r, int o) {
-    static_assert(P_ >= 3, "three taps in the first instruction");
-    const uint32_t m = __builtin_amdgcn_bitop3_b32(rd_tap<S_, 0>(r, o), rd_tap<S_, 1>(r, o), rd_tap<S_, 2>(r, o),
-                                                   rd_tt3(PRE_ & 1, (PRE_ >> 1) & 1, (PRE_ >> 2) & 1));
-    return rd_match_from<S_, P_, PRE_, 3>(m, r, o);
-}
 
 __device__ __forceinline__ void rd_barrier_lds() { asm volatile("s_waitcnt lgkmcnt(0)\n\ts_barrier" ::: "memory"); }
 
@@ -878,6 +858,12 @@
         for (uint32_t i = tid; i < a.zero_words; i += RD_FT_WG) a.zero_next[i] = 0;
     if (tid < G) { s_cnt[tid] = 0; s_kept[tid] = 0; }
     if (tid == 0) s_ready = 0;
+    uint32_t *s_bm = s_dyn + a.bm_off;
+    uint32_t n_dm_raw = 0;
+    if (a.fsl) {
+        for (uint32_t i = tid; i < (uint32_t)G * a.bm_words; i += RD_FT_WG) s_bm[i] = 0;
+        n_dm_raw = a.fscnt[grp];
+    }
     const int prio_q = (int)(((unsigned)grp * 4u) / (unsigned)n_groups);
     if (wave == 0) RD_FT_STAMP(0);
 
@@ -931,7 +917,47 @@
     __syncthreads();
     if (wave == 0) RD_FT_STAMP(1);
 
-    {
+    if (a.fsl) {
+        const uint32_t n_dm = n_dm_raw < a.fs_cap ? n_dm_raw : a.fs_cap;
+        const uint32_t *ml = a.fsl + (size_t)grp * a.fs_cap;
+        for (uint32_t i = tid; i < n_dm; i += RD_FT_WG) {
+            const uint32_t e = ml[i];
+            const uint32_t g = e >> 30;
+            const uint32_t slot = atomicAdd(&s_cnt[g], 1u);
+            if (slot < a.bcap) s_pos[(size_t)g * a.bcap + slot] = (int32_t)(e & 0x3FFFFFFFu);
+        }
+        auto test_word = [&](uint32_t g, long u) {
+            const uint32_t bit = 1u << (u & 31);
+            if (atomicOr(&s_bm[(size_t)g * a.bm_words + (uint32_t)(u >> 5)], bit) & bit) return;
+            const uint32_t *w = a.lay.bits + (size_t)(stream0 + (int)g) * a.lay.bits_stride + u;
+            uint32_t r[RD_FS_SPAN];
+#pragma unroll
+            for (int k = 0; k < RD_FS_SPAN; k++) r[k] = w[k];
+            uint32_t m = rd_match_word<S_, P_, PRE_>(r, 0) & rd_fs_range_mask(u, a.p_hi);
+            while (m) {
+                const int bpos = __builtin_ctz(m);
+                m &= m - 1;
+                const uint32_t slot = atomicAdd(&s_cnt[g], 1u);
+                if (slot < a.bcap) s_pos[(size_t)g * a.bcap + slot] = (int32_t)(32 * u + bpos);
+            }
+        };
+        const uint32_t *bk = a.fixb + (size_t)grp * a.fix_bcap;
+        const uint32_t n_fix = n_fix_raw < a.fix_bcap ? n_fix_raw : a.fix_bcap;
+        for (uint32_t it = tid; it < n_fix * RD_FS_SPAN; it += RD_FT_WG) {
+            const uint32_t widx = bk[it / RD_FS_SPAN] >> 4;
+            const int k = (int)(it % RD_FS_SPAN);
+            const uint32_t s = widx / (uint32_t)a.lay.bits_stride;
+            const uint32_t d = widx - s * (uint32_t)a.lay.bits_stride;
+            const long u = rd_fs_tail_candidate(d, k);
+            const uint32_t g = s - (uint32_t)stream0;
+            if (g < (uint32_t)n_here && rd_fs_tail_takes(u, k, a.p_hi)) test_word(g, u);
+        }
+        for (uint32_t it = tid; it < (uint32_t)n_here * (RD_FS_SPAN - 1); it += RD_FT_WG) {
+            const long u = rd_fs_tail_end_first(a.tps) + (long)(it % (RD_FS_SPAN - 1));
+            if (u >= 0 && 32 * u <= (long)a.p_hi) test_word(it / (RD_FS_SPAN - 1), u);
+        }
+        if (n_dm_raw > a.fs_cap && tid == 0) atomicOr(&a.counters[RD_CNT_OVF], 8u);
+    } else {
         constexpr int NW = ((RD_SEARCH_OUT + ((P_ - 1) * S_ + 31) / 32 + 1 + 3) / 4) * 4;
         const int gps = a.p_hi / (32 * RD_SEARCH_OUT) + 1;
         const int wgps = (gps + 63) / 64;
@@ -1158,6 +1184,8 @@
         __hip_atomic_store(&a.gstate[n_groups + grp], tag | (mtotal < 0xFFFFFu ? mtotal : 0xFFFFFu), __ATOMIC_RELAXED, __HIP_MEMORY_SCOPE_AGENT);
         __hip_atomic_store(&a.gstate[2 * n_groups + grp], tag | (n_fix_raw < 0xFFFFFu ? n_fix_raw : 0xFFFFFu), __ATOMIC_RELAXED,
                            __HIP_MEMORY_SCOPE_AGENT);
+        __hip_atomic_store(&a.gstate[3 * n_groups + grp], tag | (n_dm_raw < 0xFFFFFu ? n_dm_raw : 0xFFFFFu), __ATOMIC_RELAXED,
+                           __HIP_MEMORY_SCOPE_AGENT);
         __hip_atomic_store(&a.gstate[grp], tag | total, __ATOMIC_RELAXED, __HIP_MEMORY_SCOPE_AGENT);
         if (n_fix_raw > a.fix_bcap) atomicOr(&a.counters[RD_CNT_OVF], 8u);
     }
@@ -1193,33 +1221,38 @@
         for (int o = 32; o > 0; o >>= 1) sum += (uint32_t)__shfl_xor((int)sum, o, 64);
         if (lane == 0) __hip_atomic_store(&s_ready, sum + 1u, __ATOMIC_RELAXED, __HIP_MEMORY_SCOPE_WORKGROUP);
         if (grp == n_groups - 1) {
-            uint32_t mt = 0, ft = 0;
+            uint32_t mt = 0, ft = 0, dt = 0;
             for (int i0 = 0; i0 < n_groups; i0 += 512) {
-                uint32_t vm[8], vf[8];
+                uint32_t vm[8], vf[8], vd[8];
 #pragma unroll
                 for (int k = 0; k < 8; k++) {
                     const int i = i0 + lane + 64 * k;
                     vm[k] = i < n_groups ? __hip_atomic_load(&a.gstate[n_groups + i], __ATOMIC_RELAXED, __HIP_MEMORY_SCOPE_AGENT) : tag;
                     vf[k] = i < n_groups ? __hip_atomic_load(&a.gstate[2 * n_groups + i], __ATOMIC_RELAXED, __HIP_MEMORY_SCOPE_AGENT) : tag;
+                    vd[k] = i < n_groups ? __hip_atomic_load(&a.gstate[3 * n_groups + i], __ATOMIC_RELAXED, __HIP_MEMORY_SCOPE_AGENT) : tag;
                 }
 #pragma unroll
                 for (int k = 0; k < 8; k++) {
                     const int i = i0 + lane + 64 * k;
                     if ((vm[k] & 0xFFF00000u) != tag) vm[k] = tagged(&a.gstate[n_groups + i]);
                     if ((vf[k] & 0xFFF00000u) != tag) vf[k] = tagged(&a.gstate[2 * n_groups + i]);
+                    if ((vd[k] & 0xFFF00000u) != tag) vd[k] = tagged(&a.gstate[3 * n_groups + i]);
                     mt += vm[k] & 0xFFFFFu;
                     ft += vf[k] & 0xFFFFFu;
+                    dt += vd[k] & 0xFFFFFu;
                 }
             }
 #pragma unroll
             for (int o = 32; o > 0; o >>= 1) {
                 mt += (uint32_t)__shfl_xor((int)mt, o, 64);
                 ft += (uint32_t)__shfl_xor((int)ft, o, 64);
+                dt += (uint32_t)__shfl_xor((int)dt, o, 64);
             }
             if (lane == 0) {
                 a.counters[RD_CNT_TASKS] = sum + total;
                 a.counters[RD_CNT_MATCH] = mt;
                 a.counters[RD_CNT_FIX] = ft;
+                a.counters[RD_CNT_DMATCH] = dt;
                 if (sum + total > a.rec_cap) atomicOr(&a.counters[RD_CNT_OVF], 2u);
             }
         }
@@ -1320,6 +1353,10 @@
 #endif
 
 size_t rd_tail_fused_lds(uint32_t bcap) { return (size_t)RD_FT_STREAMS * bcap * (8 + 1 + 2 + 4) * sizeof(uint32_t); }
+static uint32_t rd_tail_bm_words(uint32_t n_samples) { return ((n_samples + 31) / 32 + 31) / 32; }
+int rd_tail_fused_search_fits(uint32_t bcap, uint32_t n_samples) {
+    return rd_tail_fused_lds(bcap) + (size_t)RD_FT_STREAMS * rd_tail_bm_words(n_samples) * sizeof(uint32_t) <= 150 * 1024;
+}
 
 int rd_launch_tail_fused(const rd_layout &lay, const rd_devcfg &cfg, int n_calls, long p_lo, long p_hi, const rd_ft_bufs &fb,
                          uint32_t bucket_limit, uint32_t seq, int skip_fix, rd_packet *recs, uint32_t rec_cap, uint32_t *counters,
@@ -1338,6 +1375,11 @@
     a.recs = recs; a.rec_cap = rec_cap; a.counters = counters; a.zero_next = zero_next; a.zero_words = zero_words;
     a.stamps = nullptr;
     a.abl = 0;
+    const bool fused = fb.fsl && fb.fscnt && fb.fs_cap && !skip_fix && rd_tail_fused_search_fits(fb.bcap, lay.n_samples);
+    a.fsl = fused ? fb.fsl : nullptr; a.fscnt = fb.fscnt; a.fs_cap = fb.fs_cap;
+    a.bm_off = (uint32_t)(rd_tail_fused_lds(fb.bcap) / sizeof(uint32_t));
+    a.bm_words = rd_tail_bm_words(lay.n_samples);
+    a.tps = (lay.n_samples + RD_TILE_SAMPLES - 1) / RD_TILE_SAMPLES;
     const uint32_t groups = (uint32_t)(lay.n_streams + RD_FT_STREAMS - 1) / RD_FT_STREAMS;
 #ifdef RD_DIAG
     if (const char *e = getenv("RD_FT_ABL")) a.abl = atoi(e);
@@ -1347,7 +1389,7 @@
         a.stamps = g_ft_stamps;
     }
 #endif
-    const size_t lds = std::max<size_t>(rd_tail_fused_lds(fb.bcap), 33 * 1024);
+    const size_t lds = std::max<size_t>(rd_tail_fused_lds(fb.bcap) + (fused ? (size_t)RD_FT_STREAMS * a.bm_words * sizeof(uint32_t) : 0), 33 * 1024);
     static bool attr_set = false;
     if (lds > 48 * 1024 && !attr_set) {
         hipFuncSetAttribute((const void *)k_tail<14, 16, 0x91D3ull, 80>, hipFuncAttributeMaxDynamicSharedMemorySize, 150 * 1024);
diff --git a/rtldavis_amd/csrc/rd_search.h b/rtldavis_amd/csrc/rd_search.h
--- /dev/null
+++ b/rtldavis_amd/csrc/rd_search.h
@@ -0,0 +1,59 @@
+#pragma once
+#include <stdint.h>
+
+#if defined(__HIPCC__)
+#define RD_FS_HD __host__ __device__
+#else
+#define RD_FS_HD
+#endif
+
+#define RD_FS_SPAN 8
+#define RD_FS_TILE_WORDS 64
+
+RD_FS_HD inline bool rd_fs_demod_owns(uint32_t dirty8, bool one_wave) { return one_wave && (dirty8 & 0xFFu) == 0; }
+
+RD_FS_HD inline uint32_t rd_fs_range_mask(long v, long p_hi) {
+    const long q0 = 32 * v;
+    if (v < 0 || q0 > p_hi) return 0u;
+    return q0 + 31 <= p_hi ? 0xFFFFFFFFu : (0xFFFFFFFFu >> (31 - (int)(p_hi - q0)));
+}
+
+RD_FS_HD inline long rd_fs_demod_word(uint32_t ti, uint32_t wi) { return (long)ti * RD_FS_TILE_WORDS + (long)wi - (RD_FS_SPAN - 1); }
+RD_FS_HD inline bool rd_fs_demod_one_wave(uint32_t wi, bool carry) { return carry || wi >= RD_FS_SPAN - 1; }
+
+RD_FS_HD inline long rd_fs_tail_candidate(uint32_t d, int k) { return (long)d - k; }
+RD_FS_HD inline bool rd_fs_tail_takes(long u, int k, long p_hi) {
+    return u >= 0 && 32 * u <= p_hi && !rd_fs_demod_owns(1u << k, true);
+}
+RD_FS_HD inline long rd_fs_tail_end_first(uint32_t tiles_per_stream) {
+    return (long)tiles_per_stream * RD_FS_TILE_WORDS - (RD_FS_SPAN - 1);
+}
+
+#if defined(__HIPCC__)
+template <int S_, int T>
+__device__ __forceinline__ uint32_t rd_tap(const uint32_t *r, int o) {
+    constexpr int wj = (T * S_) >> 5, sh = (T * S_) & 31;
+    return sh ? __builtin_amdgcn_alignbit(r[o + wj + 1], r[o + wj], sh) : r[o + wj];
+}
+constexpr int rd_tt3(bool pa, bool pb, bool pc) { return (pa ? 0xF0 : 0x0F) & (pb ? 0xCC : 0x33) & (pc ? 0xAA : 0x55); }
+template <int S_, int P_, uint64_t PRE_, int T>
+__device__ __forceinline__ uint32_t rd_match_from(uint32_t m, const uint32_t *r, int o) {
+    if constexpr (T >= P_) {
+        return m;
+    } else if constexpr (T + 1 == P_) {
+        const uint32_t v = rd_tap<S_, T>(r, o);
+        return __builtin_amdgcn_bitop3_b32(m, v, v, rd_tt3(true, (PRE_ >> T) & 1, (PRE_ >> T) & 1));
+    } else {
+        const uint32_t n = __builtin_amdgcn_bitop3_b32(m, rd_tap<S_, T>(r, o), rd_tap<S_, T + 1>(r, o),
+                                                       rd_tt3(true, (PRE_ >> T) & 1, (PRE_ >> (T + 1)) & 1));
+        return rd_match_from<S_, P_, PRE_, T + 2>(n, r, o);
+    }
+}
+template <int S_, int P_, uint64_t PRE_>
+__device__ __forceinline__ uint32_t rd_match_word(const uint32_t *r, int o) {
+    static_assert(P_ >= 3, "three taps in the first instruction");
+    const uint32_t m = __builtin_amdgcn_bitop3_b32(rd_tap<S_, 0>(r, o), rd_tap<S_, 1>(r, o), rd_tap<S_, 2>(r, o),
+                                                   rd_tt3(PRE_ & 1, (PRE_ >> 1) & 1, (PRE_ >> 2) & 1));
+    return rd_match_from<S_, P_, PRE_, 3>(m, r, o);
+}
+#endif
```

Measured after the change: 2.060 million MS/s. About the same (-0.2%).
